# mythos-bio/mythos

Hardware: AMD Instinct MI355X
Metric: MD steps/sec (and ns/day) per GPU, oxDNA2 12 kbp duplex (higher is better)
Workload: dtype f32; 1 GPU; oxDNA2 12000 bp duplex (24000 nt), Debye-Hueckel salt 0.5, Langevin dt 0.005, free space, 1 replica/GPU; half_charged_ends=True, replicas=1, repeats=1, warmup_steps_done=10205, precision=headline f32 (north_star: fp32 at 1e-3); the other precision: --full, full=False

## Files before the change

include/mythos_hip.h:

```cpp
#ifndef MYTHOS_HIP_H
#define MYTHOS_HIP_H

#include <stdint.h>

#ifdef __cplusplus
extern "C" {
#endif

typedef struct mythos_system mythos_system_t;
typedef struct mythos_sim mythos_sim_t;
typedef struct mythos_martini mythos_martini_t;
typedef struct mythos_martini_sim mythos_martini_sim_t;
typedef struct mythos_obs mythos_obs_t;
typedef void* mythos_stream_t;

enum mythos_status {
  MYTHOS_OK = 0,
  MYTHOS_ERR_INVALID_ARGUMENT = -1,
  MYTHOS_ERR_HIP = -2,
  MYTHOS_ERR_NO_DEVICE = -3,
  MYTHOS_ERR_NOT_READY = -4,
  MYTHOS_ERR_OVERFLOW = -5,
  MYTHOS_ERR_NUMERIC = -6
};

enum mythos_dtype { MYTHOS_F32 = 0, MYTHOS_F64 = 1 };

#define MYTHOS_OXDNA_N_TERMS 8

const char* mythos_version(void);
const char* mythos_last_error(void);
int mythos_device_count(void);

int mythos_oxdna_param_count(void);
const char* mythos_oxdna_param_name(int index);

mythos_system_t* mythos_oxdna_create(int model, int n, const int32_t* seq, const uint8_t* is_end, int n_bonded,
                                     const int32_t* bonded, const double* box, int dtype, int device);
void mythos_oxdna_destroy(mythos_system_t* sys);

int mythos_oxdna_set_params(mythos_system_t* sys, const double* flat_params, int n_params);

int mythos_oxdna_set_nucleotide_types(mythos_system_t* sys, const uint8_t* is_rna);

int mythos_oxdna_set_pseq(mythos_system_t* sys, const double* marginals, const int32_t* unit, int n_bp,
                          const double* bp_probs, int terms);

int mythos_oxdna_energy_dpseq(mythos_system_t* sys, const void* center, const void* quat, int n_frames, double* e_terms,
                              void* dU_dcenter, void* dU_dquat, double* dU_dparams, double* dU_dmarginals, double* dU_dbp,
                              mythos_stream_t stream);

int mythos_oxdna_set_neighbors(mythos_system_t* sys, const int32_t* pairs, int n_pairs);

int mythos_oxdna_build_neighbors(mythos_system_t* sys, const void* center, double r_cut, double skin,
                                 mythos_stream_t stream);
int mythos_oxdna_neighbor_stats(mythos_system_t* sys, int* max_row, double* mean_row);

int mythos_oxdna_energy(mythos_system_t* sys, const void* center, const void* quat, int n_frames, double* e_terms,
                        void* dU_dcenter, void* dU_dquat, double* dU_dparams, mythos_stream_t stream);

#define MYTHOS_DEBYE_SWEEP_CONSTS 5
int mythos_oxdna_debye_sweep(mythos_system_t* sys, const void* center, const void* quat, int n_frames, int n_kt,
                             const double* dh_consts, double* e_dh, double* de_dconsts, mythos_stream_t stream);

#define MYTHOS_OP_BOND 0
#define MYTHOS_OP_MINDISTANCE 1
int mythos_oxdna_order_params(mythos_system_t* sys, const void* center, const void* quat, int n_frames, int n_ops,
                              const int32_t* op_kind, const int32_t* op_first, const int32_t* pairs, int n_pairs,
                              double hb_cutoff, double* op_out, double* hb_out, double* dist_out, mythos_stream_t stream);

mythos_obs_t* mythos_observables_create(int model, int n, const double* geometry, const double* box, int n_bp,
                                        const int32_t* base_pairs, int n_quartets, const int32_t* quartets, int skip_ends,
                                        int dtype, int device);
void mythos_observables_destroy(mythos_obs_t* obs);
int mythos_observables_width(const mythos_obs_t* obs);
int mythos_observables_eval(mythos_obs_t* obs, const void* center, const void* quat, int n_frames, double* out,
                            mythos_stream_t stream);
int mythos_oxdna_energy_obs(mythos_system_t* sys, const void* center, const void* quat, int n_frames, double* e_terms,
                            void* dU_dcenter, void* dU_dquat, double* dU_dparams, mythos_obs_t* obs, double* obs_out,
                            mythos_stream_t stream);

mythos_sim_t* mythos_langevin_create(mythos_system_t* sys, double dt, double kT, double gamma_t, double gamma_r,
                                     double mass, const double* inertia, uint64_t seed);
void mythos_langevin_destroy(mythos_sim_t* sim);

int mythos_langevin_set_neighbor_policy(mythos_sim_t* sim, double r_cut, double skin, int every);

int mythos_langevin_init_momenta(mythos_sim_t* sim, void* p_lin, void* p_ang, mythos_stream_t stream);

int mythos_langevin_run(mythos_sim_t* sim, void* center, void* quat, void* p_lin, void* p_ang, int n_steps,
                        int save_every, void* traj_center, void* traj_quat, double* e_trace,
                        mythos_stream_t stream);
int mythos_langevin_load(mythos_sim_t* sim, const void* center, const void* quat, const void* p_lin, const void* p_ang,
                         mythos_stream_t stream);
int mythos_langevin_advance(mythos_sim_t* sim, int n_steps, int save_every, void* traj_center, void* traj_quat,
                            double* e_trace, mythos_stream_t stream);
int mythos_langevin_store(mythos_sim_t* sim, void* center, void* quat, void* p_lin, void* p_ang, mythos_stream_t stream);

int64_t mythos_langevin_get_step(const mythos_sim_t* sim);
int mythos_langevin_set_step(mythos_sim_t* sim, int64_t step);
int mythos_langevin_set_seed(mythos_sim_t* sim, uint64_t seed);

int mythos_langevin_set_external_forces(mythos_sim_t* sim, int count, const int32_t* index, const double* force);

enum mythos_langevin_option { MYTHOS_LANGEVIN_UNFUSED = 0 };
int mythos_langevin_set_option(mythos_sim_t* sim, int option, int64_t value);

int mythos_langevin_set_timing(mythos_sim_t* sim, int samples);
int mythos_langevin_last_kernel_ms(const mythos_sim_t* sim, double* kernel_ms, double* loop_ms_per_launch,
                                   int* launches, int* samples);

int mythos_langevin_last_recoveries(const mythos_sim_t* sim, int* recoveries);
int mythos_langevin_last_rebuilds(const mythos_sim_t* sim, int* scheduled);

int mythos_oxdna_read_trajectory(const char* path, int n, int max_frames, double* times, double* box, double* energies,
                                 double* frames, int* n_frames);

int mythos_oxdna_write_trajectory(const char* path, int n, int n_frames, const double* times, const double* box,
                                  const double* energies, const double* frames, int append);

enum mythos_debug_key {
  MYTHOS_DEBUG_CELL_BUCKET_CAP = 0,
  MYTHOS_DEBUG_ENERGY_LIST_CAP = 1,
  MYTHOS_DEBUG_MD_SEGMENT = 2,
  MYTHOS_DEBUG_MD_OVERFLOW_AT = 3,
  MYTHOS_DEBUG_MD_DENSE = 4,
  MYTHOS_DEBUG_MD_ITEMS_BIG = 5,
  MYTHOS_DEBUG_MD_LANES = 6,
  MYTHOS_DEBUG_KEYS = 7
};
int mythos_debug_set(int key, int64_t value);
int64_t mythos_debug_get(int key);

#define MYTHOS_MARTINI_N_TERMS 3
mythos_martini_t* mythos_martini_create(int n, const int32_t* types, int n_types, const double* sigma,
                                        const double* eps, int n_bonds, const int32_t* bonds, const double* bond_k,
                                        const double* bond_r0, int n_angles, const int32_t* angles,
                                        const double* angle_k, const double* angle_t0, int angle_kind, double r_cut,
                                        int dtype, int device);
void mythos_martini_destroy(mythos_martini_t* m);
int mythos_martini_energy(mythos_martini_t* m, const void* pos, const void* box, int n_frames, double* e_terms,
                          void* dU_dpos, mythos_stream_t stream);

int mythos_martini_param_grads(mythos_martini_t* m, const void* pos, const void* box, int n_frames, double* d_sigma,
                               double* d_eps, double* d_bond_k, double* d_bond_r0, double* d_angle_k,
                               double* d_angle_t0, mythos_stream_t stream);

mythos_martini_sim_t* mythos_martini_langevin_create(mythos_martini_t* sys, double dt, double kT, double gamma,
                                                     const double* mass, uint64_t seed);
void mythos_martini_langevin_destroy(mythos_martini_sim_t* sim);
int mythos_martini_langevin_set_neighbor_policy(mythos_martini_sim_t* sim, double skin, int rebuild_every);
int mythos_martini_langevin_set_inner_list(mythos_martini_sim_t* sim, double margin, int every);
int mythos_martini_langevin_init_velocities(mythos_martini_sim_t* sim, void* vel, mythos_stream_t stream);
int mythos_martini_langevin_run(mythos_martini_sim_t* sim, void* pos, void* vel, const double* box, int n_steps,
                                int save_every, void* traj_pos, double* e_trace, mythos_stream_t stream);
int mythos_martini_langevin_load(mythos_martini_sim_t* sim, const void* pos, const void* vel, const double* box,
                                 mythos_stream_t stream);
int mythos_martini_langevin_advance(mythos_martini_sim_t* sim, int n_steps, int save_every, void* traj_pos, double* e_trace,
                                    mythos_stream_t stream);
int mythos_martini_langevin_store(mythos_martini_sim_t* sim, void* pos, void* vel, mythos_stream_t stream);
int64_t mythos_martini_langevin_get_step(const mythos_martini_sim_t* sim);
int mythos_martini_langevin_last_rebuilds(const mythos_martini_sim_t* sim, int* scheduled);
int mythos_martini_langevin_last_kernel_ms(const mythos_martini_sim_t* sim, double* kernel_ms,
                                           double* loop_ms_per_launch, int* launches, int* samples);
int mythos_martini_langevin_set_timing(mythos_martini_sim_t* sim, int samples);
int mythos_martini_langevin_last_recoveries(const mythos_martini_sim_t* sim, int* recoveries);
int mythos_martini_langevin_neighbor_stats(const mythos_martini_sim_t* sim, int* max_row, double* mean_row);
int mythos_martini_langevin_get_rows(const mythos_martini_sim_t* sim, int which, int32_t* rows, int32_t* row_len, int* stride);

int mythos_martini_langevin_set_barostat(mythos_martini_sim_t* sim, int kind, int coupling, const double ref_p[2],
                                         const double compressibility[2], double tau_p, int every);
int mythos_martini_langevin_pressure(mythos_martini_sim_t* sim, double out[10], mythos_stream_t stream);
int mythos_martini_langevin_get_box(const mythos_martini_sim_t* sim, double box[3]);
int mythos_martini_langevin_last_boxes(const mythos_martini_sim_t* sim, double* boxes, int* n_rows);

typedef struct mythos_martini_obs mythos_martini_obs_t;
mythos_martini_obs_t* mythos_martini_obs_create(int n, int n_groups, const int32_t* beads_per_item, const int32_t* members,
                                                const int32_t* index, int device);
void mythos_martini_obs_destroy(mythos_martini_obs_t* obs);
int64_t mythos_martini_obs_count(const mythos_martini_obs_t* obs);
int mythos_martini_obs_eval(mythos_martini_obs_t* obs, const void* pos, const void* box, int dtype, int n_frames, double* out,
                            mythos_stream_t stream);

typedef struct mythos_w1_plan mythos_w1_plan_t;
mythos_w1_plan_t* mythos_w1_plan_create(int n_groups, const int32_t* n_frames, const int32_t* members, const double* samples,
                                        const int64_t* n_ref, const double* ref, const double* ref_weights,
                                        const uint8_t* has_ref_weights, const int64_t* order, int device,
                                        mythos_stream_t stream);
void mythos_w1_plan_destroy(mythos_w1_plan_t* plan);
int mythos_w1_eval(mythos_w1_plan_t* plan, const double* weights, double* w1, double* dw1_dweights, mythos_stream_t stream);

#define MYTHOS_MEMBRANE_ROW 7
typedef struct mythos_membrane mythos_membrane_t;
mythos_membrane_t* mythos_membrane_create(int n, int n_lipids, const int32_t* lipid_start, const int32_t* lipid_beads, int n_thick,
                                          const int32_t* thick_beads, const int32_t* thick_lipid, int device);
void mythos_membrane_destroy(mythos_membrane_t* mem);
int mythos_membrane_n_lipids(const mythos_membrane_t* mem);
int mythos_membrane_eval(mythos_membrane_t* mem, const void* pos, const void* box, int dtype, int n_frames, double* out,
                         int8_t* leaflets, mythos_stream_t stream);

#define MYTHOS_DUPLEX_ROW 4
typedef struct mythos_duplex_obs mythos_duplex_obs_t;
mythos_duplex_obs_t* mythos_duplex_obs_create(int model, int n, const double* geometry, const double* box, int n_bp,
                                              const int32_t* base_pairs, int n_quartets, const int32_t* quartets,
                                              const int32_t* end_pairs, const double* target_center, int device);
void mythos_duplex_obs_destroy(mythos_duplex_obs_t* obs);
int mythos_duplex_obs_eval(mythos_duplex_obs_t* obs, const void* center, const void* quat, int dtype, int n_frames, double* out,
                           mythos_stream_t stream);

#ifdef __cplusplus
}
#endif
#endif
```

mythos_amd/_lib.py:

```python

from __future__ import annotations

import ctypes as C
import os
from pathlib import Path

import torch

_LIB_PATH = Path(__file__).resolve().parent / "lib" / "libmythos_hip.so"

c_int_p = C.POINTER(C.c_int32)
c_double_p = C.POINTER(C.c_double)
c_uint8_p = C.POINTER(C.c_uint8)


class MythosHipError(RuntimeError):
    """An error reported by libmythos_hip.so."""


_lib = None

V = C.c_void_p
_SIGS = {
    "mythos_version": (C.c_char_p, []),
    "mythos_last_error": (C.c_char_p, []),
    "mythos_device_count": (C.c_int, []),
    "mythos_debug_set": (C.c_int, [C.c_int, C.c_int64]),
    "mythos_debug_get": (C.c_int64, [C.c_int]),
    "mythos_oxdna_param_count": (C.c_int, []),
    "mythos_oxdna_param_name": (C.c_char_p, [C.c_int]),
    "mythos_oxdna_create": (V, [C.c_int, C.c_int, c_int_p, c_uint8_p, C.c_int, c_int_p, c_double_p, C.c_int, C.c_int]),
    "mythos_oxdna_destroy": (None, [V]),
    "mythos_oxdna_set_params": (C.c_int, [V, c_double_p, C.c_int]),
    "mythos_oxdna_set_pseq": (C.c_int, [V, c_double_p, c_int_p, C.c_int, c_double_p, C.c_int]),
    "mythos_oxdna_set_nucleotide_types": (C.c_int, [V, c_uint8_p]),
    "mythos_oxdna_set_neighbors": (C.c_int, [V, c_int_p, C.c_int]),
    "mythos_oxdna_build_neighbors": (C.c_int, [V, V, C.c_double, C.c_double, V]),
    "mythos_oxdna_neighbor_stats": (C.c_int, [V, C.POINTER(C.c_int), c_double_p]),
    "mythos_oxdna_energy": (C.c_int, [V, V, V, C.c_int, V, V, V, V, V]),
    "mythos_oxdna_energy_obs": (C.c_int, [V, V, V, C.c_int, V, V, V, V, V, V, V]),
    "mythos_oxdna_energy_dpseq": (C.c_int, [V, V, V, C.c_int, V, V, V, V, V, V, V]),
    "mythos_oxdna_debye_sweep": (C.c_int, [V, V, V, C.c_int, C.c_int, c_double_p, V, V, V]),
    "mythos_oxdna_order_params": (C.c_int, [V, V, V, C.c_int, C.c_int, c_int_p, c_int_p, c_int_p, C.c_int, C.c_double, V, V, V, V]),
    "mythos_observables_create": (V, [C.c_int, C.c_int, c_double_p, c_double_p, C.c_int, c_int_p, C.c_int, c_int_p, C.c_int, C.c_int, C.c_int]),
    "mythos_observables_destroy": (None, [V]),
    "mythos_observables_width": (C.c_int, [V]),
    "mythos_observables_eval": (C.c_int, [V, V, V, C.c_int, V, V]),
    "mythos_langevin_create": (V, [V, C.c_double, C.c_double, C.c_double, C.c_double, C.c_double, c_double_p, C.c_uint64]),
    "mythos_langevin_destroy": (None, [V]),
    "mythos_langevin_set_neighbor_policy": (C.c_int, [V, C.c_double, C.c_double, C.c_int]),
    "mythos_langevin_init_momenta": (C.c_int, [V, V, V, V]),
    "mythos_langevin_run": (C.c_int, [V, V, V, V, V, C.c_int, C.c_int, V, V, V, V]),
    "mythos_langevin_load": (C.c_int, [V, V, V, V, V, V]),
    "mythos_langevin_advance": (C.c_int, [V, C.c_int, C.c_int, V, V, V, V]),
    "mythos_langevin_store": (C.c_int, [V, V, V, V, V, V]),
    "mythos_langevin_get_step": (C.c_int64, [V]),
    "mythos_langevin_set_step": (C.c_int, [V, C.c_int64]),
    "mythos_langevin_set_seed": (C.c_int, [V, C.c_uint64]),
    "mythos_langevin_set_external_forces": (C.c_int, [V, C.c_int, c_int_p, c_double_p]),
    "mythos_langevin_last_kernel_ms": (C.c_int, [V, c_double_p, c_double_p, C.POINTER(C.c_int), C.POINTER(C.c_int)]),
    "mythos_langevin_set_option": (C.c_int, [V, C.c_int, C.c_int64]),
    "mythos_langevin_set_timing": (C.c_int, [V, C.c_int]),
    "mythos_martini_langevin_set_timing": (C.c_int, [V, C.c_int]),
    "mythos_langevin_last_recoveries": (C.c_int, [V, C.POINTER(C.c_int)]),
    "mythos_langevin_last_rebuilds": (C.c_int, [V, C.POINTER(C.c_int)]),
    "mythos_oxdna_read_trajectory": (C.c_int, [C.c_char_p, C.c_int, C.c_int, c_double_p, c_double_p, c_double_p, c_double_p, C.POINTER(C.c_int)]),
    "mythos_oxdna_write_trajectory": (C.c_int, [C.c_char_p, C.c_int, C.c_int, c_double_p, c_double_p, c_double_p, c_double_p, C.c_int]),
    "mythos_martini_create": (
        V,
        [C.c_int, c_int_p, C.c_int, c_double_p, c_double_p, C.c_int, c_int_p, c_double_p, c_double_p, C.c_int,
         c_int_p, c_double_p, c_double_p, C.c_int, C.c_double, C.c_int, C.c_int],
    ),
    "mythos_martini_destroy": (None, [V]),
    "mythos_martini_energy": (C.c_int, [V, V, V, C.c_int, V, V, V]),
    "mythos_martini_param_grads": (C.c_int, [V, V, V, C.c_int, V, V, V, V, V, V, V]),
    "mythos_martini_langevin_create": (V, [V, C.c_double, C.c_double, C.c_double, c_double_p, C.c_uint64]),
    "mythos_martini_langevin_destroy": (None, [V]),
    "mythos_martini_langevin_set_neighbor_policy": (C.c_int, [V, C.c_double, C.c_int]),
    "mythos_martini_langevin_set_inner_list": (C.c_int, [V, C.c_double, C.c_int]),
    "mythos_martini_langevin_init_velocities": (C.c_int, [V, V, V]),
    "mythos_martini_langevin_run": (C.c_int, [V, V, V, c_double_p, C.c_int, C.c_int, V, V, V]),
    "mythos_martini_langevin_load": (C.c_int, [V, V, V, c_double_p, V]),
    "mythos_martini_langevin_advance": (C.c_int, [V, C.c_int, C.c_int, V, V, V]),
    "mythos_martini_langevin_store": (C.c_int, [V, V, V, V]),
    "mythos_martini_langevin_get_step": (C.c_int64, [V]),
    "mythos_martini_langevin_last_rebuilds": (C.c_int, [V, C.POINTER(C.c_int)]),
    "mythos_martini_langevin_last_kernel_ms": (C.c_int, [V, c_double_p, c_double_p, C.POINTER(C.c_int), C.POINTER(C.c_int)]),
    "mythos_martini_langevin_last_recoveries": (C.c_int, [V, C.POINTER(C.c_int)]),
    "mythos_martini_langevin_neighbor_stats": (C.c_int, [V, C.POINTER(C.c_int), c_double_p]),
    "mythos_martini_langevin_get_rows": (C.c_int, [V, C.c_int, C.POINTER(C.c_int32), C.POINTER(C.c_int32), C.POINTER(C.c_int)]),
    "mythos_martini_langevin_set_barostat": (C.c_int, [V, C.c_int, C.c_int, c_double_p, c_double_p, C.c_double, C.c_int]),
    "mythos_martini_langevin_pressure": (C.c_int, [V, c_double_p, V]),
    "mythos_martini_langevin_get_box": (C.c_int, [V, c_double_p]),
    "mythos_martini_langevin_last_boxes": (C.c_int, [V, c_double_p, C.POINTER(C.c_int)]),
    "mythos_martini_obs_create": (V, [C.c_int, C.c_int, c_int_p, c_int_p, c_int_p, C.c_int]),
    "mythos_martini_obs_destroy": (None, [V]),
    "mythos_martini_obs_count": (C.c_int64, [V]),
    "mythos_martini_obs_eval": (C.c_int, [V, V, V, C.c_int, C.c_int, V, V]),
    "mythos_w1_plan_create": (V, [C.c_int, c_int_p, c_int_p, V, C.POINTER(C.c_int64), V, V, c_uint8_p, V, C.c_int, V]),
    "mythos_w1_plan_destroy": (None, [V]),
    "mythos_w1_eval": (C.c_int, [V, V, V, V, V]),
    "mythos_membrane_create": (V, [C.c_int, C.c_int, c_int_p, c_int_p, C.c_int, c_int_p, c_int_p, C.c_int]),
    "mythos_membrane_destroy": (None, [V]),
    "mythos_membrane_n_lipids": (C.c_int, [V]),
    "mythos_membrane_eval": (C.c_int, [V, V, V, C.c_int, C.c_int, V, V, V]),
    "mythos_duplex_obs_create": (V, [C.c_int, C.c_int, c_double_p, c_double_p, C.c_int, c_int_p, C.c_int, c_int_p, c_int_p, c_double_p, C.c_int]),
    "mythos_duplex_obs_destroy": (None, [V]),
    "mythos_duplex_obs_eval": (C.c_int, [V, V, V, C.c_int, C.c_int, V, V]),
}


def lib_path() -> Path:
    return Path(os.environ.get("MYTHOS_HIP_LIB", _LIB_PATH))


def load() -> C.CDLL:
    global _lib
    if _lib is not None:
        return _lib
    path = lib_path()
    if not path.exists():
        raise MythosHipError(
            f"{path} not found: the HIP extension is not built (run __graft_entry__.build()). "
            "mythos_amd has no CPU fallback."
        )
    lib = C.CDLL(str(path))
    for name, (res, args) in _SIGS.items():
        fn = getattr(lib, name)
        fn.restype = res
        fn.argtypes = args
    _lib = lib
    return lib


DECLARED_SYMBOLS = tuple(_SIGS)


MEMBRANE_ROW = 7


def last_error() -> str:
    return load().mythos_last_error().decode()


def check(rc: int, what: str = "") -> None:
    if rc == 0:
        return
    msg = f"{what}: {last_error()} (status {rc})"
    if rc == -1:
        raise ValueError(msg)
    if rc == -6:
        raise FloatingPointError(msg)
    raise MythosHipError(msg)


DEBUG_KEYS = {"cell_bucket_cap": 0, "energy_list_cap": 1, "md_segment": 2, "md_overflow_at": 3, "md_dense": 4, "md_items_big": 5, "md_lanes": 6}


def debug_set(key: str, value: int) -> None:
    check(load().mythos_debug_set(DEBUG_KEYS[key], int(value)), f"debug_set({key})")


def debug_get(key: str) -> int:
    return int(load().mythos_debug_get(DEBUG_KEYS[key]))


_PARAM_NAMES: list[str] = []


def param_names() -> list[str]:
    if not _PARAM_NAMES:
        lib = load()
        _PARAM_NAMES.extend(lib.mythos_oxdna_param_name(i).decode() for i in range(lib.mythos_oxdna_param_count()))
    return list(_PARAM_NAMES)


def device_count() -> int:
    return int(load().mythos_device_count())


def ptr(t):
    if t is None:
        return None
    if hasattr(t, "data_ptr"):
        return C.c_void_p(t.data_ptr())
    return C.c_void_p(t.ctypes.data)


def stream(device) -> C.c_void_p:
    return C.c_void_p(torch.cuda.current_stream(device).cuda_stream)


def dtype_code(dtype: torch.dtype) -> int:
    if dtype == torch.float32:
        return 0
    if dtype == torch.float64:
        return 1
    raise ValueError(f"unsupported dtype {dtype}: use torch.float32 or torch.float64")


class Handle:

    _destroy = ""
    _h = None

    def __init__(self, create: str, *args):
        self._lib = load()
        self._h = getattr(self._lib, create)(*args)
        if not self._h:
            raise MythosHipError(f"{create}: {last_error()}")

    def close(self) -> None:
        h, self._h = self._h, None
        if h:
            getattr(self._lib, self._destroy)(h)

    def __del__(self):
        try:
            self.close()
        except Exception:
            pass


def per_device(owner, key, make):
    sets = owner.__dict__.setdefault("_sets", {})
    key = str(key)
    if key not in sets:
        sets[key] = make()
    return sets[key]
```

mythos_amd/csrc/langevin.hip:

```cpp
#include <memory>
#include <vector>

#include "langevin_core.inc"

namespace {
MdEntries md_entries_of(const mythos_sim* s) { return s->sys->dtype == MYTHOS_F32 ? md_entries<float>() : md_entries_f64(); }
}

extern "C" {

mythos_sim_t* mythos_langevin_create(mythos_system_t* sys, double dt, double kT, double gamma_t, double gamma_r,
                                     double mass, const double* inertia, uint64_t seed) {
  if (!sys || !(dt > 0) || !(kT >= 0) || gamma_t < 0 || gamma_r < 0 || !(mass > 0)) {
    set_error("mythos_langevin_create: invalid argument");
    return nullptr;
  }
  if (select_device(sys->device, "mythos_langevin_create")) return nullptr;
  auto s = std::make_unique<mythos_sim>();
  s->sys = sys;
  s->device = sys->device;
  s->dt = dt;
  s->kT = kT;
  s->gamma_t = gamma_t;
  s->gamma_r = gamma_r;
  s->mass = mass;
  for (int k = 0; k < 3; ++k) s->inertia[k] = inertia ? inertia[k] : 1.0;
  s->seed = seed;
  const size_t v4 = (sys->dtype == MYTHOS_F32 ? sizeof(float4) : sizeof(double4)) * (size_t)sys->n;
  bool ok = md_run_create(*s);
  for (int k = 0; k < 2; ++k)
    for (int a = 0; a < mythos_sim::kFrameArrays; ++a) ok = ok && s->frame[k][a].alloc(v4) == 0;
  ok = ok && s->keep_hi.alloc(v4) == 0 && s->keep_lo.alloc(v4) == 0 &&
       s->d_epart.alloc((size_t)((sys->n + 15) / 16) * kTraceWidth) == 0 && sys->reserve_refs() == 0;
  if (!ok) {
    set_error("mythos_langevin_create: device allocation failed");
    return nullptr;
  }
  return s.release();
}

void mythos_langevin_destroy(mythos_sim_t* s) { delete s; }

int mythos_langevin_set_neighbor_policy(mythos_sim_t* s, double r_cut, double skin, int every) {
  if (!s || (every > 0 && (!(r_cut > 0) || !(skin > 0)))) {
    set_error("mythos_langevin_set_neighbor_policy: invalid argument");
    return MYTHOS_ERR_INVALID_ARGUMENT;
  }
  s->r_cut = r_cut;
  s->skin = skin;
  s->rebuild_every = every;
  s->list_fitted = false;
  s->list_valid = false;
  return MYTHOS_OK;
}

int mythos_langevin_init_momenta(mythos_sim_t* s, void* p_lin, void* p_ang, mythos_stream_t stream) {
  if (!s || !p_lin || !p_ang) {
    set_error("mythos_langevin_init_momenta: invalid argument");
    return MYTHOS_ERR_INVALID_ARGUMENT;
  }
  MYTHOS_HIP_TRY(hipSetDevice(s->device));
  return md_entries_of(s).init_momenta(s, p_lin, p_ang, (hipStream_t)stream);
}

namespace {

int md_ready_state(mythos_sim_t* s, const char* who) {
  mythos_system* sys = s->sys;
  if (!sys->params_set) {
    set_error(std::string(who) + ": parameters must be set first");
    return MYTHOS_ERR_NOT_READY;
  }
  if (sys->model == 4 && !sys->types_set) {
    set_error(std::string(who) + ": an oxNA system needs its nucleotide types (mythos_oxdna_set_nucleotide_types)");
    return MYTHOS_ERR_NOT_READY;
  }
  MYTHOS_HIP_TRY(hipSetDevice(sys->device));
  return MYTHOS_OK;
}

int md_ready(mythos_sim_t* s, const char* who) {
  mythos_system* sys = s->sys;
  if (int rc = md_ready_state(s, who)) return rc;
  if (!sys->nbrs_set && s->rebuild_every <= 0) {
    set_error(std::string(who) + ": parameters and neighbours (or a neighbour policy) must be set first");
    return MYTHOS_ERR_NOT_READY;
  }
  if (s->rebuild_every > 0 && sys->list.stride == 0)
    if (int rc = rows_reserve(sys->list, sys->n, 64)) return rc;
  if (s->list_epoch != sys->list_epoch) {
    s->list_valid = false;
    s->list_epoch = sys->list_epoch;
  }
  return MYTHOS_OK;
}


int md_load(mythos_sim_t* s, void* c, void* q, void* p, void* l, hipStream_t st) {
  s->unfused.active = s->unfused.want && s->sys->model == 4;
  return md_entries_of(s).load(s, c, q, p, l, st);
}

int md_advance(mythos_sim_t* s, int n_steps, int save_every, bool close, void* tc, void* tq, double* e_trace, hipStream_t st) {
  if (s->ext_count > 0 && s->unfused.active) {
    set_error("mythos_langevin_run / advance: external forces are not applied on the unfused oxNA path "
              "(MYTHOS_LANGEVIN_UNFUSED); clear them or step through the fused kernel");
    return MYTHOS_ERR_INVALID_ARGUMENT;
  }
  const size_t q_align = s->sys->dtype == MYTHOS_F32 ? sizeof(float4) : sizeof(double4);
  if (save_every > 0 && tq && (reinterpret_cast<uintptr_t>(tq) % q_align) != 0) {
    set_error("mythos_langevin_run / advance: traj_quat must be aligned to 4 elements (" + std::to_string(q_align) + " bytes)");
    return MYTHOS_ERR_INVALID_ARGUMENT;
  }
  return md_entries_of(s).advance(s, n_steps, save_every, close, tc, tq, e_trace, st);
}

int md_store(mythos_sim_t* s, void* c, void* q, void* p, void* l, hipStream_t st) {
  return md_entries_of(s).store(s, c, q, p, l, st);
}

}

int mythos_langevin_run(mythos_sim_t* s, void* center, void* quat, void* p_lin, void* p_ang, int n_steps,
                        int save_every, void* traj_center, void* traj_quat, double* e_trace,
                        mythos_stream_t stream) {
  if (!s || !center || !quat || !p_lin || !p_ang || n_steps < 0 || save_every < 0) {
    set_error("mythos_langevin_run: invalid argument");
    return MYTHOS_ERR_INVALID_ARGUMENT;
  }
  if (int rc = md_ready(s, "mythos_langevin_run")) return rc;
  hipStream_t st = (hipStream_t)stream;
  if (int rc = md_load(s, center, quat, p_lin, p_ang, st)) return rc;
  const int rc = md_advance(s, n_steps, save_every, true, traj_center, traj_quat, e_trace, st);
  if (int rs = md_store(s, center, quat, p_lin, p_ang, st)) return rc ? rc : rs;
  return rc;
}

int mythos_langevin_load(mythos_sim_t* s, const void* center, const void* quat, const void* p_lin, const void* p_ang,
                         mythos_stream_t stream) {
  if (!s || !center || !quat || !p_lin || !p_ang) {
    set_error("mythos_langevin_load: invalid argument");
    return MYTHOS_ERR_INVALID_ARGUMENT;
  }
  if (int rc = md_ready_state(s, "mythos_langevin_load")) return rc;
  return md_load(s, (void*)center, (void*)quat, (void*)p_lin, (void*)p_ang, (hipStream_t)stream);
}

int mythos_langevin_advance(mythos_sim_t* s, int n_steps, int save_every, void* traj_center, void* traj_quat,
                            double* e_trace, mythos_stream_t stream) {
  if (!s || n_steps < 0 || save_every < 0) {
    set_error("mythos_langevin_advance: invalid argument");
    return MYTHOS_ERR_INVALID_ARGUMENT;
  }
  if (!s->resident) {
    set_error("mythos_langevin_advance: no resident state (call mythos_langevin_load first; a run that ended in a numeric "
              "error drops its state)");
    return MYTHOS_ERR_NOT_READY;
  }
  if (int rc = md_ready(s, "mythos_langevin_advance")) return rc;
  return md_advance(s, n_steps, save_every, false, traj_center, traj_quat, e_trace, (hipStream_t)stream);
}

int mythos_langevin_store(mythos_sim_t* s, void* center, void* quat, void* p_lin, void* p_ang, mythos_stream_t stream) {
  if (!s || !center || !quat || !p_lin || !p_ang) {
    set_error("mythos_langevin_store: invalid argument");
    return MYTHOS_ERR_INVALID_ARGUMENT;
  }
  if (!s->resident) {
    set_error("mythos_langevin_store: no resident state");
    return MYTHOS_ERR_NOT_READY;
  }
  if (s->open) {
    if (int rc = md_ready(s, "mythos_langevin_store")) return rc;
  } else {
    MYTHOS_HIP_TRY(hipSetDevice(s->device));
  }
  return md_store(s, center, quat, p_lin, p_ang, (hipStream_t)stream);
}

int64_t mythos_langevin_get_step(const mythos_sim_t* s) { return md_get_step(s); }

int mythos_langevin_set_step(mythos_sim_t* s, int64_t step) {
  if (!s || step < 0) {
    set_error("mythos_langevin_set_step: invalid argument");
    return MYTHOS_ERR_INVALID_ARGUMENT;
  }
  s->step = step;
  s->ext_stamp_stale = true;
  return MYTHOS_OK;
}

int mythos_langevin_set_external_forces(mythos_sim_t* s, int count, const int32_t* index, const double* force) {
  const char* who = "mythos_langevin_set_external_forces";
  if (!s || count < 0 || (count > 0 && (!index || !force))) {
    set_error(std::string(who) + ": invalid argument");
    return MYTHOS_ERR_INVALID_ARGUMENT;
  }
  if (s->resident && s->open) {
    set_error(std::string(who) + ": the resident frame is open (its pending closing half kick would mix two forces); call "
              "mythos_langevin_store first");
    return MYTHOS_ERR_INVALID_ARGUMENT;
  }
  const int n = s->sys->n;
  std::vector<char> seen((size_t)n, 0);
  for (int e = 0; e < count; ++e) {
    if (index[e] < 0 || index[e] >= n) {
      set_error(std::string(who) + ": nucleotide index " + std::to_string(index[e]) + " out of range [0, " + std::to_string(n) + ")");
      return MYTHOS_ERR_INVALID_ARGUMENT;
    }
    if (seen[index[e]]) {
      set_error(std::string(who) + ": nucleotide " + std::to_string(index[e]) + " is listed twice (sum its forces first)");
      return MYTHOS_ERR_INVALID_ARGUMENT;
    }
    seen[index[e]] = 1;
    for (int k = 0; k < 3; ++k)
      if (!std::isfinite(force[3 * (size_t)e + k])) {
        set_error(std::string(who) + ": a force component is not finite");
        return MYTHOS_ERR_INVALID_ARGUMENT;
      }
  }
  MYTHOS_HIP_TRY(hipSetDevice(s->device));
  s->ext_stamp_stale = true;
  if (count == 0) {
    s->ext_count = 0;
    return MYTHOS_OK;
  }
  MYTHOS_HIP_TRY(hipDeviceSynchronize());
  std::vector<double> f4((size_t)count * 4, 0.0);
  for (int e = 0; e < count; ++e)
    for (int k = 0; k < 3; ++k) f4[4 * (size_t)e + k] = force[3 * (size_t)e + k];
  s->ext_count = 0;
  if (int rc = s->d_ext_index.upload(index, (size_t)count)) return rc;
  if (int rc = s->d_ext_force.upload_real(s->sys->dtype, f4.data(), f4.size())) return rc;
  if (!s->d_ext_stamp)
    if (int rc = s->d_ext_stamp.alloc(1)) return rc;
  s->ext_count = count;
  return MYTHOS_OK;
}

int mythos_langevin_set_seed(mythos_sim_t* s, uint64_t seed) {
  if (!s) {
    set_error("mythos_langevin_set_seed: invalid argument");
    return MYTHOS_ERR_INVALID_ARGUMENT;
  }
  s->seed = seed;
  return MYTHOS_OK;
}

int mythos_langevin_last_kernel_ms(const mythos_sim_t* s, double* kernel_ms, double* loop_ms_per_launch,
                                   int* launches, int* samples) {
  return md_last_kernel_ms(s, kernel_ms, loop_ms_per_launch, launches, samples, "mythos_langevin_last_kernel_ms");
}

int mythos_langevin_last_recoveries(const mythos_sim_t* s, int* recoveries) {
  return md_last_count(s, &MdRun::last_recoveries, recoveries, "mythos_langevin_last_recoveries");
}

int mythos_langevin_last_rebuilds(const mythos_sim_t* s, int* scheduled) {
  return md_last_count(s, &MdRun::last_rebuilds, scheduled, "mythos_langevin_last_rebuilds");
}

int mythos_langevin_set_option(mythos_sim_t* s, int option, int64_t value) {
  if (!s || option != MYTHOS_LANGEVIN_UNFUSED || (value != 0 && value != 1)) {
    set_error("mythos_langevin_set_option: invalid argument");
    return MYTHOS_ERR_INVALID_ARGUMENT;
  }
  if (value == 1 && s->sys->model != 4) {
    set_error("mythos_langevin_set_option: the unfused path exists for oxNA systems (model 4) only");
    return MYTHOS_ERR_INVALID_ARGUMENT;
  }
  s->unfused.want = value == 1;
  return MYTHOS_OK;
}

int mythos_langevin_set_timing(mythos_sim_t* s, int samples) { return md_set_timing(s, samples, "mythos_langevin_set_timing"); }

}
```

mythos_amd/csrc/langevin_core.inc:

```
#include <algorithm>
#include <cmath>
#include <type_traits>

#include <hip/hip_ext.h>

#ifndef MYTHOS_LEAN_MATH
#define MYTHOS_LEAN_MATH 1
#endif

#include "cell_list.h"
#include "chunk_order.h"
#include "md_driver.h"
#include "md_plan.h"
#include "oxdna_gather.h"
#include "philox.h"

#include "langevin_step.h"
#include "langevin_frame.h"
#include "langevin_unfused.inc"

using namespace mythos;

namespace mythos {

static_assert(kMdPlanBlock == kMdBlock, "md_plan.h plans for the step kernel's workgroup");

inline int device_cus(const mythos_system* sys) {
  int cus = 256;
  (void)hipDeviceGetAttribute(&cus, hipDeviceAttributeMultiprocessorCount, sys->device);
  return cus;
}

template <typename R>
static int update_chunk_order(mythos_sim* sim, const typename Vec4T<R>::type* p0, int blocks, hipStream_t st) {
  if (blocks < 64) {
    sim->d_chunk_order.reset(), sim->d_chunk_keys.reset();
    return 0;
  }
  if (int rc = sim->d_chunk_keys.grow((size_t)blocks)) return rc;
  if (int rc = sim->d_chunk_order.grow((size_t)blocks)) return rc;
  MYTHOS_HIP_TRY(chunk_order_device(p0, blocks, kMdBlock / sim->lanes, std::max(1.0, sim->r_cut > 0 ? sim->r_cut : 4.0), sim->d_chunk_keys.get(),
                                    sim->d_chunk_order.get(), st));
  return 0;
}

template <typename R, int MODEL>
static int load_typed(mythos_sim* sim, const R* center, const R* quat, const R* p_lin, const R* p_ang, hipStream_t st) {
  mythos_system* sys = sim->sys;
  const int n = sys->n;
  const int tb = (n + 255) / 256;
  const OxParams<R>& P = params_of<R>(sys);
  const R g_k1 = P[GEO_BACK_A1], g_k2 = (MODEL >= 2) ? P[GEO_BACK_A2] : R(0);
  sim->cur = 0;
  const Frame<R> f0 = frame_of<R>(sim, 0);
  const double* Prna = oxdna_param_set(sys, sys->param_sets() == 1 ? 0 : 1);
  hipLaunchKernelGGL((pack_state_kernel<R, (MODEL == 4 ? 0 : back_axis<MODEL>())>), dim3(tb), dim3(256), 0, st, n, g_k1, g_k2,
                     R(Prna[GEO_BACK_A1]), R(Prna[GEO_BACK_A2]), center, quat, p_lin, p_ang,
                     sys->d_meta.get(), f0, sim->keep_valid ? (const R*)sim->keep_hi.get() : nullptr,
                     (const R*)sim->keep_lo.get());
  MYTHOS_HIP_TRY(hipGetLastError());
  sim->resident = true;
  sim->list_valid = false;
  sim->since_build = 0;
  sim->items_big = false;
  sim->open = false;
  sim->ext_stamp_stale = true;
  sim->param_epoch = sys->param_epoch;
  const int cus = device_cus(sys);
  sim->lanes = md_lanes_for(n, cus, debug_value(MYTHOS_DEBUG_MD_LANES));
  return update_chunk_order<R>(sim, f0.p0, md_plan_for(n, sim->lanes, cus, sizeof(R), 0).blocks, st);
}

template <typename R>
static int unpack_typed(mythos_sim* sim, R* center, R* quat, R* p_lin, R* p_ang, hipStream_t st) {
  const int n = sim->sys->n;
  hipLaunchKernelGGL(unpack_state_kernel<R>, dim3((n + 255) / 256), dim3(256), 0, st, n, frame_of<R>(sim, sim->cur),
                     center, quat, p_lin, p_ang, (R*)sim->keep_hi.get(), (R*)sim->keep_lo.get());
  MYTHOS_HIP_TRY(hipGetLastError());
  sim->keep_valid = true;
  return 0;
}

template <typename R, int MODEL>
static int advance_typed(mythos_sim* sim, int n_steps, int save_every, bool close, R* traj_center, R* traj_quat, double* e_trace,
                         hipStream_t st) {
  using V4 = typename Vec4T<R>::type;
  mythos_system* sys = sim->sys;
  const int n = sys->n;
  const MdPlan plan = md_plan_for(n, sim->lanes, device_cus(sys), sizeof(R), debug_value(MYTHOS_DEBUG_MD_DENSE));
  const int blocks = plan.blocks;
  const R* Pdev = device_params_of<R>(sys);
  const BoxT<R> box = make_box<R>(sys);
  const LangevinConst<R> K = make_const<R>(sim);
  const MdCut<R> cut = make_cut<R>(sys);
  const Frame<R> fr[2] = {frame_of<R>(sim, 0), frame_of<R>(sim, 1)};
  if (sim->param_epoch != sys->param_epoch) {
    const OxParams<R>& Ph = params_of<R>(sys);
    const double* Prna = oxdna_param_set(sys, sys->param_sets() == 1 ? 0 : 1);
    hipLaunchKernelGGL((rederive_frame_kernel<R, (MODEL == 4 ? 0 : back_axis<MODEL>())>), dim3((n + 255) / 256), dim3(256), 0, st, n,
                       Ph[GEO_BACK_A1], (MODEL >= 2) ? Ph[GEO_BACK_A2] : R(0), R(Prna[GEO_BACK_A1]), R(Prna[GEO_BACK_A2]),
                       (const int*)sys->d_meta.get(), fr[sim->cur]);
    MYTHOS_HIP_TRY(hipGetLastError());
    sim->param_epoch = sys->param_epoch;
  }
  const bool dynamic_list = sim->rebuild_every > 0;
  PseqView<R> pseq;
  const bool use_pseq = sys->pseq_terms != 0;
  if (debug_value(MYTHOS_DEBUG_MD_ITEMS_BIG) == 1) sim->items_big = true;
  if (use_pseq) pseq.marg = (const R*)sys->d_ps_marg.get(), pseq.unit = sys->d_ps_unit.get(), pseq.bp = (const R*)sys->d_ps_bp.get(), pseq.terms = sys->pseq_terms;
  int* halt_words = dynamic_list ? sys->list.d_overflow.get() : nullptr;
  auto launch_step = [&](int k, const LaunchRow& row) {
    const int cur = row.cur;
    const bool save = row.save;
    const R kick_close = R(row.kick_close);
    R* tc = ((save || row.save_next) && traj_center) ? traj_center + (size_t)row.sidx * n * 3 : nullptr;
    R* tq = ((save || row.save_next) && traj_quat) ? traj_quat + (size_t)row.sidx * n * 4 : nullptr;
    const V4* ref = (const V4*)sys->d_ref_pos.get();
    const V4* ref_off = (const V4*)sys->d_ref_off.get();
    const V4* ref_a1 = (const V4*)sys->d_ref_a1.get();
    if (sim->ext_count > 0) {
      if (sim->ext_stamp_stale) {
        (void)hipMemsetAsync(sim->d_ext_stamp.get(), 0, sizeof(unsigned long long), st);
        sim->ext_stamp_stale = false;
      }
      const double c = double(row.kick_close) + 0.5 * row.do_step;
      const unsigned long long stamp = 2ull * (unsigned long long)(sim->step + k) + (row.kick_close != 0.0f ? 1ull : 0ull) + 1ull;
      hipLaunchKernelGGL(ext_kick_kernel<R>, dim3(1), dim3(256), 0, st, sim->ext_count, (const int*)sim->d_ext_index.get(),
                         (const V4*)sim->d_ext_force.get(), R(c * sim->dt), fr[cur].mom, (const int*)sim->d_flags.get(),
                         (const int*)halt_words, k, stamp, sim->d_ext_stamp.get());
    }
    auto launch = [&](auto save_tag, auto items_tag, auto pseq_tag, auto dense_tag, auto lanes_tag) {
      hipExtLaunchKernelGGL((md_step_kernel<R, MODEL, decltype(save_tag)::value, decltype(items_tag)::value, decltype(pseq_tag)::value,
                                            decltype(dense_tag)::value, decltype(lanes_tag)::value>),
                            dim3(plan.grid), dim3(kMdBlock), 0, st, row.ea, row.eb, 0,
                            Pdev, box, K, cut, n, fr[cur], fr[cur ^ 1], sys->list.d_rows.get(), sys->d_row_len.get(), row_close_of(sys),
                            sys->list.stride, sys->extra_bonds ? 1 : 0, kick_close, row.do_step, sim->seed, (uint64_t)(sim->step + k), ref,
                            ref_off, ref_a1, sim->d_flags.get(), tc, tq, sim->d_epart.get(), sim->d_chunk_order.get(), halt_words, k, 0,
                            plan.prio_on, pseq);
    };
    with_bool(save, [&](auto save_tag) {
      with_bool(sim->items_big, [&](auto big_tag) {
        constexpr bool SV = decltype(save_tag)::value;
        using Items = std::integral_constant<int, decltype(big_tag)::value ? md_items_big<R, SV>() : kMdItems>;
        with_bool(use_pseq, [&](auto pseq_tag) {
          using L8 = std::integral_constant<int, 8>;
          using L16 = std::integral_constant<int, 16>;
          constexpr bool dense_exists = sizeof(R) == 4 && !SV && !decltype(pseq_tag)::value && Items::value == kMdItems && MODEL <= 2;
          if (sim->lanes == 16) {
            launch(save_tag, Items{}, pseq_tag, std::false_type{}, L16{});
          } else if constexpr (dense_exists) {
            with_bool(plan.dense_grid, [&](auto dense_tag) { launch(save_tag, Items{}, pseq_tag, dense_tag, L8{}); });
          } else {
            launch(save_tag, Items{}, pseq_tag, std::false_type{}, L8{});
          }
        });
      });
    });
    if (save)
      hipLaunchKernelGGL(reduce_trace_kernel<kTraceWidth>, dim3(1), dim3(256), 0, st, sim->d_epart.get(), blocks,
                         e_trace + (size_t)row.sidx * kTraceWidth);
  };
  auto rebuild = [&](int buf) -> int {
    if ((++sim->builds & 63) == 0)
      if (int rc = update_chunk_order<R>(sim, fr[buf].p0, blocks, st)) return rc;
    return rows_build_device(sys, fr[buf].p0, true, sim->r_cut, sim->skin, fr[buf].p3, fr[buf].p1, true, st);
  };
  auto rebuild_until_fit = [&](int buf) -> int {
    return rows_build_until_fit(sys, fr[buf].p0, true, sim->r_cut, sim->skin, fr[buf].p3, fr[buf].p1, true, true, st);
  };
  auto on_abort = [&]() -> int {
    if (!sim->items_big) {
      sim->items_big = true;
      return 0;
    }
    set_error("mythos_langevin_run: more than " + std::to_string(md_items_big<R, false>()) + " (" + std::to_string(md_items_big<R, true>()) +
              " on steps that save energies)"
              " neighbours of one nucleotide are inside the range of an angular term (overlapping bases?)");
    return MYTHOS_ERR_OVERFLOW;
  };
  MdDrive d;
  d.who = "mythos_langevin_run";
  d.n_steps = n_steps, d.save_every = save_every, d.close = close;
  d.energy_rows = save_every > 0 && e_trace != nullptr;
  d.plain_rows = save_every > 0 && e_trace == nullptr && (traj_center != nullptr || traj_quat != nullptr);
  d.dynamic_list = dynamic_list;
  d.halt_words = halt_words;
  d.row_stride = &sys->list.stride;
  d.skin = sim->skin;
  d.st = st;
  return md_drive(*sim, d, launch_step, rebuild, rebuild_until_fit, on_abort);
}

template <typename R>
static int entry_load(mythos_sim* s, void* c, void* q, void* p, void* l, hipStream_t st) {
  if (s->unfused.active) return unfused_load<R>(s, (R*)c, (R*)q, (R*)p, (R*)l, st);
  return with_model(s->sys->model, [&](auto m) { return load_typed<R, decltype(m)::value>(s, (R*)c, (R*)q, (R*)p, (R*)l, st); });
}

template <typename R>
static int entry_advance(mythos_sim* s, int n_steps, int save_every, bool close, void* tc, void* tq, double* e_trace, hipStream_t st) {
  if (s->unfused.active) return unfused_advance<R>(s, n_steps, save_every, (R*)tc, (R*)tq, e_trace, st);
  return with_model(s->sys->model, [&](auto m) {
    return advance_typed<R, decltype(m)::value>(s, n_steps, save_every, close, (R*)tc, (R*)tq, e_trace, st);
  });
}

template <typename R>
static int entry_store(mythos_sim* s, void* c, void* q, void* p, void* l, hipStream_t st) {
  if (s->unfused.active) return unfused_store<R>(s, (R*)c, (R*)q, (R*)p, (R*)l, st);
  const int rc = s->open ? entry_advance<R>(s, 0, 0, true, nullptr, nullptr, nullptr, st) : MYTHOS_OK;
  const int ru = unpack_typed<R>(s, (R*)c, (R*)q, (R*)p, (R*)l, st);
  return rc ? rc : ru;
}

template <typename R>
static int entry_init_momenta(mythos_sim* s, void* p_lin, void* p_ang, hipStream_t st) {
  const double sd_t = std::sqrt(s->mass * s->kT);
  double sd_r[3];
  for (int k = 0; k < 3; ++k) sd_r[k] = std::sqrt(s->inertia[k] * s->kT);
  hipLaunchKernelGGL(init_momenta_kernel<R>, dim3(1), dim3(256), 0, st, s->sys->n, R(sd_t), R(sd_r[0]), R(sd_r[1]), R(sd_r[2]), s->seed,
                     (R*)p_lin, (R*)p_ang);
  MYTHOS_HIP_TRY(hipGetLastError());
  return MYTHOS_OK;
}

struct MdEntries {
  int (*load)(mythos_sim*, void*, void*, void*, void*, hipStream_t);
  int (*advance)(mythos_sim*, int, int, bool, void*, void*, double*, hipStream_t);
  int (*store)(mythos_sim*, void*, void*, void*, void*, hipStream_t);
  int (*init_momenta)(mythos_sim*, void*, void*, hipStream_t);
};
template <typename R>
constexpr MdEntries md_entries() {
  return {entry_load<R>, entry_advance<R>, entry_store<R>, entry_init_momenta<R>};
}
MdEntries md_entries_f64();

}
```

mythos_amd/csrc/langevin_sim.h:

```cpp
#pragma once
#ifndef MYTHOS_UNFUSED_STATE_DEFINED
#error "langevin_sim.h needs UnfusedState: include langevin_unfused.inc (or langevin_core.inc), which defines it and then includes this file"
#endif
#include <cmath>

#include "langevin_step.h"
#include "md_driver.h"

struct mythos_sim : mythos::MdRun {
  mythos_system* sys = nullptr;
  int device = 0;
  double dt = 0, kT = 0, gamma_t = 0, gamma_r = 0, mass = 1, inertia[3] = {1, 1, 1};
  double r_cut = 0, skin = 0;
  static constexpr int kFrameArrays = 8;
  mythos::DeviceBytes frame[2][kFrameArrays];
  int builds = 0;
  int list_epoch = 0;
  mythos::DeviceBytes keep_hi, keep_lo;
  bool keep_valid = false;
  bool items_big = false;
  int param_epoch = 0;
  int lanes = mythos::kMdG;
  mythos::DeviceBuf<int> d_chunk_order;
  mythos::DeviceBuf<unsigned long long> d_chunk_keys;
  mythos::DeviceBuf<double> d_epart;
  mythos::UnfusedState unfused;
  int ext_count = 0;
  mythos::DeviceBuf<int> d_ext_index;
  mythos::DeviceBytes d_ext_force;
  mythos::DeviceBuf<unsigned long long> d_ext_stamp;
  bool ext_stamp_stale = true;
  ~mythos_sim() { (void)hipSetDevice(device); }
};

namespace mythos {

template <typename R>
static LangevinConst<R> make_const(const mythos_sim* s) {
  LangevinConst<R> K;
  K.dt = R(s->dt);
  K.half_dt = R(0.5 * s->dt);
  K.inv_mass = R(1.0 / s->mass);
  const double c1t = std::exp(-s->gamma_t * s->dt), c1r = std::exp(-s->gamma_r * s->dt);
  K.c1_t = R(c1t);
  K.c2_t = R(std::sqrt(s->kT * (1.0 - c1t * c1t) * s->mass));
  K.c1_r = R(c1r);
  for (int k = 0; k < 3; ++k) {
    K.inv_inertia[k] = R(1.0 / s->inertia[k]);
    K.c2_r[k] = R(std::sqrt(s->kT * (1.0 - c1r * c1r) * s->inertia[k]));
  }
  K.skin_half_sq = R(s->rebuild_every > 0 ? 0.25 * s->skin * s->skin : -1.0);
  return K;
}

template <typename R>
static MdCut<R> make_cut(const mythos_system* sys) {
  const OxParams<double>& P = sys->pd;
  double rbb = oxdna_param_max(sys, NEXC_BACKBONE_RC);
  if (sys->model >= 2) rbb = std::max(rbb, oxdna_param_max(sys, DH_RCUT));
  const double rcom = oxdna_close_range(sys);
  MdCut<R> c;
  c.rbb2 = R(rbb * rbb);
  c.rcom2 = R(rcom * rcom);
  auto sq = [](double v) { return R(v * v); };
  c.hb_lo2 = sq(P[HYDR_RCLOW]), c.hb_hi2 = sq(P[HYDR_RCHIGH]);
  c.cr_lo2 = sq(P[CRST_RCLOW]), c.cr_hi2 = sq(P[CRST_RCHIGH]);
  c.cx_lo2 = sq(P[CXST_RCLOW]), c.cx_hi2 = sq(P[CXST_RCHIGH]);
  c.hb_mask = 0;
  for (int k = 0; k < 16; ++k)
    if (P[HYDR_EPS_00 + k] != 0.0) c.hb_mask |= 1u << k;
  return c;
}

template <typename R>
static Frame<R> frame_of(const mythos_sim* sim, int k) {
  using V4 = typename Vec4T<R>::type;
  auto a = [&](int i) { return (V4*)sim->frame[k][i].get(); };
  return Frame<R>{a(0), a(1), a(2), a(3), a(4), a(5), a(6), a(7)};
}

}
```

mythos_amd/csrc/langevin_step.h:

```cpp
#pragma once
#include <hip/hip_runtime.h>

#include <cstdint>

#include "oxdna_gather.h"
#include "philox.h"

namespace mythos {

template <typename R>
struct LangevinConst {
  R dt, half_dt;
  R inv_mass;
  R inv_inertia[3];
  R c1_t, c2_t;
  R c1_r, c2_r[3];
  R skin_half_sq;
};

template <int K, typename R>
__device__ __forceinline__ void free_rotor(R* q, R* L, R h, const R* inv_I) {
  const R phi = h * L[K] * inv_I[K];
  R s, c;
  if constexpr (sizeof(R) == 4) {
    s = __sinf(R(0.5) * phi);
    c = __cosf(R(0.5) * phi);
  } else {
    R x = R(0.5) * phi;
    int halvings = 0;
    const bool large = __ballot(fabs(x) >= R(0.03125)) != 0ull;
    if (large)
      while (fabs(x) >= R(0.03125) && halvings < 64) x *= R(0.5), ++halvings;
    const R x2 = x * x;
    s = x * (R(1) + x2 * (R(-1.0 / 6) + x2 * (R(1.0 / 120) + x2 * R(-1.0 / 5040))));
    c = R(1) + x2 * (R(-0.5) + x2 * (R(1.0 / 24) + x2 * R(-1.0 / 720)));
    if (large)
      for (; halvings > 0; --halvings) {
        const R s2 = R(2) * s * c;
        c = c * c - s * s;
        s = s2;
      }
  }
  const R q0 = q[0], q1 = q[1], q2 = q[2], q3 = q[3];
  if constexpr (K == 0) {
    q[0] = c * q0 - s * q1;
    q[1] = c * q1 + s * q0;
    q[2] = c * q2 + s * q3;
    q[3] = c * q3 - s * q2;
  } else if constexpr (K == 1) {
    q[0] = c * q0 - s * q2;
    q[1] = c * q1 - s * q3;
    q[2] = c * q2 + s * q0;
    q[3] = c * q3 + s * q1;
  } else {
    q[0] = c * q0 - s * q3;
    q[1] = c * q1 + s * q2;
    q[2] = c * q2 - s * q1;
    q[3] = c * q3 + s * q0;
  }
  const R cf = c * c - s * s, sf = R(2) * s * c;
  constexpr int A = (K + 1) % 3, B = (K + 2) % 3;
  const R la = L[A], lb = L[B];
  L[A] = cf * la + sf * lb;
  L[B] = -sf * la + cf * lb;
}

template <typename R>
__device__ __forceinline__ void drift(R* x, R* q, const R* p, R* L, R h, const LangevinConst<R>& K) {
  x[0] += h * p[0] * K.inv_mass;
  x[1] += h * p[1] * K.inv_mass;
  x[2] += h * p[2] * K.inv_mass;
  free_rotor<2>(q, L, R(0.5) * h, K.inv_inertia);
  free_rotor<1>(q, L, R(0.5) * h, K.inv_inertia);
  free_rotor<0>(q, L, h, K.inv_inertia);
  free_rotor<1>(q, L, R(0.5) * h, K.inv_inertia);
  free_rotor<2>(q, L, R(0.5) * h, K.inv_inertia);
}

constexpr int kMdBlock = 256;
constexpr int kMdG = 8;
constexpr int kMdPPB = kMdBlock / kMdG;
#ifndef MYTHOS_MD_ITEMS
#define MYTHOS_MD_ITEMS 16
#endif
#ifndef MYTHOS_MD_F64_BLOCKS
#define MYTHOS_MD_F64_BLOCKS 3
#endif
#ifndef MYTHOS_MD_F64S_BLOCKS
#define MYTHOS_MD_F64S_BLOCKS 2
#endif
#ifndef MYTHOS_MD_F32_BLOCKS
#define MYTHOS_MD_F32_BLOCKS 3
#endif
#ifndef MYTHOS_MD_F32S_BLOCKS
#define MYTHOS_MD_F32S_BLOCKS 2
#endif
constexpr int kMdItems = MYTHOS_MD_ITEMS;
template <typename R, bool SAVE>
constexpr int md_items_big() {
  return (sizeof(R) == 8 && SAVE) ? 22 : 32;
}
#ifndef MYTHOS_MD_POOL
#define MYTHOS_MD_POOL 320
#endif
constexpr int kMdPool = MYTHOS_MD_POOL;
constexpr int kTraceWidth = T_COUNT + 2;

template <typename R>
struct Frame {
  typename Vec4T<R>::type *p0, *p1, *p2, *p3, *q, *pl, *mom, *ang;
};

template <typename R>
constexpr bool kHiLo = sizeof(R) == 4;

template <typename R>
__device__ __forceinline__ V3<R> centre_diff(const typename Vec4T<R>::type& o_hi, const typename Vec4T<R>::type& o_lo,
                                             const V3<R>& s_hi, const V3<R>& s_lo) {
  V3<R> d{o_hi.x - s_hi.x, o_hi.y - s_hi.y, o_hi.z - s_hi.z};
  if constexpr (kHiLo<R>) {
    d.x += o_lo.x - s_lo.x;
    d.y += o_lo.y - s_lo.y;
    d.z += o_lo.z - s_lo.z;
  }
  return d;
}

template <typename R>
struct MdCut {
  R rbb2;
  R rcom2;
  R hb_lo2, hb_hi2, cr_lo2, cr_hi2, cx_lo2, cx_hi2;
  unsigned int hb_mask;
};

template <typename R>
__device__ __forceinline__ V3<R> xyz(const typename Vec4T<R>::type& v) {
  return V3<R>{v.x, v.y, v.z};
}

template <typename R>
__device__ __forceinline__ R f3_coef(R eps, R tw, const F3P<R>& fp, R r2, R& coef) {
  coef = R(0);
  if (r2 >= fp.rc * fp.rc) return R(0);
  const R r = m_sqrt(r2);
  const FD<R> v = f3_eval(r, eps, fp);
  coef = tw * v.d / r;
  return v.f;
}

template <typename R>
__device__ __forceinline__ R f3_radial(R eps, R tw, const F3P<R>& fp, V3<R> d, R r2, V3<R>& g) {
  if (r2 >= fp.rc * fp.rc) return R(0);
  const R r = m_sqrt(r2);
  const FD<R> v = f3_eval(r, eps, fp);
  axpy(g, tw * v.d / r, d);
  return v.f;
}

#ifndef MYTHOS_MD_PRIO_MAP
#define MYTHOS_MD_PRIO_MAP 33210
#endif
#if MYTHOS_MD_PRIO_MAP != 0
constexpr int md_prio_digit(int phase) {
  int v = MYTHOS_MD_PRIO_MAP;
  for (int k = 4; k > phase; --k) v /= 10;
  return v % 10;
}
#define MD_PRIO(phase)                                                     \
  do {                                                                     \
    if (prio_on) __builtin_amdgcn_s_setprio(md_prio_digit(phase));        \
  } while (0)
#else
#define MD_PRIO(phase) do { } while (0)
#endif

template <typename R, bool SAVE, int ITEMS, bool DENSE = false, int MODEL = 2, bool PSEQ = false>
constexpr int md_blocks_per_cu() {
  if (DENSE) return 5;
  if (ITEMS > kMdItems) return sizeof(R) == 4 ? (SAVE ? 1 : 2) : 1;
  return sizeof(R) == 4 ? (SAVE ? MYTHOS_MD_F32S_BLOCKS : MYTHOS_MD_F32_BLOCKS) : (SAVE ? MYTHOS_MD_F64S_BLOCKS : MYTHOS_MD_F64_BLOCKS);
}

template <typename R>
struct RadSet {
  F3P<R> f_bb, f_base, f_bkba, f_babk;
  R eps_n, tw_n, tw_dh;
  DebyeP<R> dhp;
  bool half_ends;
  R rbb2, hb_lo2, hb_hi2, cr_lo2, cr_hi2, cx_lo2, cx_hi2;
  unsigned int hb_mask;
};
template <typename R, int MODEL, class PT>
__device__ __forceinline__ RadSet<R> radset_from(const PT& P, const MdCut<R>& cut) {
  RadSet<R> s;
  s.f_bb = f3_params<R>(P, NEXC_BACKBONE_RSTAR), s.f_base = f3_params<R>(P, NEXC_BASE_RSTAR);
  s.f_bkba = f3_params<R>(P, NEXC_BACK_BASE_RSTAR), s.f_babk = f3_params<R>(P, NEXC_BASE_BACK_RSTAR);
  s.eps_n = P[NEXC_EPS];
  s.tw_n = P[TW_NEXC], s.tw_dh = (MODEL >= 2) ? P[TW_DH] : R(0);
  s.half_ends = (MODEL >= 2) && (P[DH_HALF_CHARGED_ENDS] != R(0));
  s.dhp = (MODEL >= 2) ? debye_params<R>(P) : DebyeP<R>{};
  s.rbb2 = cut.rbb2, s.hb_lo2 = cut.hb_lo2, s.hb_hi2 = cut.hb_hi2, s.cr_lo2 = cut.cr_lo2, s.cr_hi2 = cut.cr_hi2;
  s.cx_lo2 = cut.cx_lo2, s.cx_hi2 = cut.cx_hi2, s.hb_mask = cut.hb_mask;
  return s;
}
template <typename R, class PT>
__device__ __forceinline__ MdCut<R> cut_from(const PT& P, R rcom2) {
  MdCut<R> c;
  const R rbb = fmax(P[NEXC_BACKBONE_RC], P[DH_RCUT]);
  c.rbb2 = rbb * rbb, c.rcom2 = rcom2;
  c.hb_lo2 = P[HYDR_RCLOW] * P[HYDR_RCLOW], c.hb_hi2 = P[HYDR_RCHIGH] * P[HYDR_RCHIGH];
  c.cr_lo2 = P[CRST_RCLOW] * P[CRST_RCLOW], c.cr_hi2 = P[CRST_RCHIGH] * P[CRST_RCHIGH];
  c.cx_lo2 = P[CXST_RCLOW] * P[CXST_RCLOW], c.cx_hi2 = P[CXST_RCHIGH] * P[CXST_RCHIGH];
  c.hb_mask = 0u;
#pragma unroll
  for (int k = 0; k < 16; ++k) c.hb_mask |= (P[HYDR_EPS_00 + k] != R(0)) ? (1u << k) : 0u;
  return c;
}
template <typename R>
__device__ __forceinline__ F3P<R> pick3(const F3P<R>& a, const F3P<R>& b, const F3P<R>& c, int k) {
  return {k == 0 ? a.rstar : (k == 1 ? b.rstar : c.rstar), k == 0 ? a.sigma : (k == 1 ? b.sigma : c.sigma),
          k == 0 ? a.b : (k == 1 ? b.b : c.b), k == 0 ? a.rc : (k == 1 ? b.rc : c.rc), a.base};
}
#define MD_PICK3(f) (k == 0 ? a.f : (k == 1 ? b.f : c.f))
template <typename R>
__device__ __forceinline__ RadSet<R> pick3(const RadSet<R>& a, const RadSet<R>& b, const RadSet<R>& c, int k) {
  RadSet<R> s;
  s.f_bb = pick3(a.f_bb, b.f_bb, c.f_bb, k), s.f_base = pick3(a.f_base, b.f_base, c.f_base, k);
  s.f_bkba = pick3(a.f_bkba, b.f_bkba, c.f_bkba, k), s.f_babk = pick3(a.f_babk, b.f_babk, c.f_babk, k);
  s.eps_n = MD_PICK3(eps_n), s.tw_n = MD_PICK3(tw_n), s.tw_dh = MD_PICK3(tw_dh);
  s.dhp = {MD_PICK3(dhp.rcut), MD_PICK3(dhp.rhigh), MD_PICK3(dhp.kappa), MD_PICK3(dhp.prefactor), MD_PICK3(dhp.bsmooth)};
  s.half_ends = a.half_ends;
  s.rbb2 = MD_PICK3(rbb2), s.hb_lo2 = MD_PICK3(hb_lo2), s.hb_hi2 = MD_PICK3(hb_hi2), s.cr_lo2 = MD_PICK3(cr_lo2);
  s.cr_hi2 = MD_PICK3(cr_hi2), s.cx_lo2 = MD_PICK3(cx_lo2), s.cx_hi2 = MD_PICK3(cx_hi2), s.hb_mask = MD_PICK3(hb_mask);
  return s;
}
#undef MD_PICK3

#define MD_RADSET_OF_ENTRY                                                                                         \
  const int md_kind = (MODEL == 4) ? na1_kind(self.rna, ((int)o0.w >> 3) & 1) : 0;                                 \
  const RadSet<R> rs_picked = (MODEL == 4) ? pick3(rs0, rs1, rs2, md_kind) : rs0;                                  \
  const RadSet<R>& rs = (MODEL == 4) ? rs_picked : rs0;
__device__ __forceinline__ int na1_kind(int self_rna, int other_rna) { return (self_rna && other_rna) ? 1 : ((self_rna || other_rna) ? 2 : 0); }

template <typename R, int MODEL, bool SAVE, int ITEMS, bool PSEQ = false, bool DENSE = false, int GL = kMdG>
__global__ __launch_bounds__(kMdBlock, (md_blocks_per_cu<R, SAVE, ITEMS, DENSE, MODEL, PSEQ>())) void md_step_kernel(
    const R* __restrict__ Pg, const BoxT<R> box, const LangevinConst<R> K, const MdCut<R> cut, int n, const Frame<R> in,
    const Frame<R> out,
    const int* __restrict__ rows, const int* __restrict__ row_len, const int* __restrict__ row_close, int row_stride,
    int extra_bonds, R kick_close, int do_step, uint64_t seed, uint64_t step, const typename Vec4T<R>::type* __restrict__ ref_pos,
    const typename Vec4T<R>::type* __restrict__ ref_off, const typename Vec4T<R>::type* __restrict__ ref_a1,
    int* __restrict__ flags,
    R* __restrict__ traj_c, R* __restrict__ traj_q, double* __restrict__ e_part, const int* __restrict__ chunk_order,
    const int* __restrict__ list_overflow, int k_index, int , int prio_on, const PseqView<R> pseq) {
  using V4 = typename Vec4T<R>::type;
  constexpr int G = GL, PPB = kMdBlock / GL;
  static_assert(GL == 8 || GL == 16, "lanes per nucleotide");
  static_assert(!DENSE || GL == kMdG, "DENSE serves large grids");
  constexpr int RW = (SAVE ? 12 + T_COUNT : 12) + 1;
  constexpr int kSlots = 2 + ITEMS;
  __shared__ int items[2][PPB][ITEMS];
  __shared__ int item_cnt[2][PPB];
  __shared__ int item_pre[4][PPB + 1];
  __shared__ R self_lds[PPB][13];
  __shared__ R rad_lds[PPB][7];
  static_assert(!DENSE || (sizeof(R) == 4 && !SAVE && !PSEQ && ITEMS == kMdItems && MODEL <= 2), "DENSE: see md_blocks_per_cu");
  constexpr bool kPooled = sizeof(R) == 8 || DENSE;
  constexpr int kPool = (ITEMS > kMdItems || !kPooled) ? PPB * kSlots : kMdPool * PPB / kMdPPB;
  static_assert(kPool >= PPB * ROW_BONDED_SLOTS, "the pool holds at least the bonded rows");
  static_assert(ITEMS > ROW_BONDED_SLOTS, "room for the second-bond slots of circular strands");
  __shared__ R res_flat[kPool * RW + (kPooled ? 0 : PPB)];
  __shared__ int row_base[kPooled ? 4 : 1][PPB + 1];
  constexpr int kFixedStride = (kSlots * RW) | 1;
  auto pool_row = [&](int row) -> R* { return res_flat + row * RW; };
  auto fixed_row = [&](int pp, int slot) -> R* { return res_flat + pp * kFixedStride + slot * RW; };
  __shared__ double e_lds[SAVE ? PPB : 1][kTraceWidth];
  using CP = ConstParams<R, PSEQ>;
  const auto make_cp = [&](const R* g) {
    if constexpr (PSEQ) return CP(g, pseq); else return CP(g);
  };
  const CP P = make_cp(Pg);
  const int grp = threadIdx.x / G;
  const int lane = threadIdx.x % G;
  const int n_blocks = (n + PPB - 1) / PPB;
  const int vb = (int)(blockIdx.x & 7) * ((n_blocks + 7) >> 3) + (int)(blockIdx.x >> 3);
  if (vb >= n_blocks) return;
  __shared__ int s_halt;
  int halt_word = 0;
  if (threadIdx.x == 0) {
    const int hw = flags[1], aw = flags[3];
    halt_word = ((hw != 0 && hw <= k_index) ? 1 : 0) | ((aw != 0 && aw <= k_index) ? 1 : 0) |
                (list_overflow ? (list_overflow[0] | list_overflow[1]) : 0);
  }
  const int bid = chunk_order ? chunk_order[vb] : vb;
  const int i = bid * PPB + grp;
  const bool valid = i < n;
  const int ii = valid ? i : n - 1;

  const R g_ba = P[GEO_BASE], g_st = P[GEO_STACK];
  const CP Prna = make_cp(Pg + ((MODEL == 4) ? OXP_COUNT : 0)), Pdrh = make_cp(Pg + ((MODEL == 4) ? 2 * OXP_COUNT : 0));
  const Na1Params<CP> P4{P, Prna, Pdrh};

  Nuc<R> self;
  V3<R> offb_s, self_lo{R(0), R(0), R(0)};
  {
    const V4 s0 = in.p0[ii], s1 = in.p1[ii], s2 = in.p2[ii], s3 = in.p3[ii];
    if constexpr (kHiLo<R>) self_lo = xyz<R>(in.pl[ii]);
    self.c = xyz<R>(s0);
    self.a1 = xyz<R>(s1);
    self.a3 = xyz<R>(s2);
    self.a2 = cross(self.a3, self.a1);
    offb_s = xyz<R>(s3);
    const int m = (int)s0.w;
    self.seq = m & 3;
    self.is_end = (m >> 2) & 1;
    self.rna = (m >> 3) & 1;
    if (lane == 0) {
      R* sl = self_lds[grp];
      sl[0] = s0.x, sl[1] = s0.y, sl[2] = s0.z, sl[3] = s1.x, sl[4] = s1.y, sl[5] = s1.z;
      sl[6] = s2.x, sl[7] = s2.y, sl[8] = s2.z, sl[9] = s0.w;
      sl[10] = self_lo.x, sl[11] = self_lo.y, sl[12] = self_lo.z;
    }
  }
  const int* __restrict__ row = rows + (size_t)ii * row_stride;
  const int len = valid ? row_len[ii] : 0;
  const int close_end = min(len, row_close[ii]);

  R e[T_COUNT];
#pragma unroll
  for (int k = 0; k < T_COUNT; ++k) e[k] = R(0);
  V3<R> gbk{R(0), R(0), R(0)}, gba{R(0), R(0), R(0)};

  MD_PRIO(0);
  const RadSet<R> rs0 = (MODEL == 4) ? radset_from<R, 2>(P, cut_from<R>(P, cut.rcom2)) : radset_from<R, MODEL>(P, cut);
  const RadSet<R> rs1 = (MODEL == 4) ? radset_from<R, 2>(Prna, cut_from<R>(Prna, cut.rcom2)) : rs0;
  const RadSet<R> rs2 = (MODEL == 4) ? radset_from<R, 2>(Pdrh, cut_from<R>(Pdrh, cut.rcom2)) : rs0;
  int n_items[2] = {0, 0};
  const int row_room = ITEMS - (extra_bonds ? ROW_BONDED_SLOTS - 2 : 0);
  const int lane64 = threadIdx.x & 63;
  const int gshift = lane64 & ~(G - 1);
  auto row_at = [&](int s, int end) -> int {
    const int v = row[max(min(s, end - 1), 0)];
    return s < end ? v : -1;
  };
  auto slot_of_entry = [&](int e) -> int { return e >= 0 ? (e & ROW_INDEX_MASK) : ii; };
  {
    int e_cur = -1, e_nxt = -1;
    V4 n0{}, n3{}, n1{}, nl{};
    {
      const int s = ROW_BONDED_SLOTS + lane;
      e_cur = row_at(s, close_end);
      e_nxt = row_at(s + G, close_end);
      const int j = slot_of_entry(e_cur);
      n0 = in.p0[j];
      n3 = in.p3[j];
      n1 = in.p1[j];
      if constexpr (kHiLo<R>) nl = in.pl[j];
    }
#pragma unroll 1
    for (int s0 = ROW_BONDED_SLOTS; s0 < close_end; s0 += G) {
      const int s = s0 + lane;
      const int entry = e_cur;
      const V4 o0 = n0, o3 = n3, o1 = n1, ol = nl;
      e_cur = e_nxt;
      e_nxt = row_at(s + 2 * G, close_end);
      {
        const int jn = slot_of_entry(e_cur);
        n0 = in.p0[jn];
        n3 = in.p3[jn];
        n1 = in.p1[jn];
        if constexpr (kHiLo<R>) nl = in.pl[jn];
      }
      bool flag[2] = {false, false};
      if (entry >= 0) {
        const bool role_p = (entry & ROW_ROLE_Q) == 0;
        MD_RADSET_OF_ENTRY
        const bool o_rna = (MODEL == 4) && ((((int)o0.w) >> 3) & 1);
        const R gba_s = (MODEL == 4 && self.rna) ? Prna[GEO_BASE] : g_ba, gba_o = o_rna ? Prna[GEO_BASE] : g_ba;
        const R gst_s = (MODEL == 4 && self.rna) ? Prna[GEO_STACK] : g_st, gst_o = o_rna ? Prna[GEO_STACK] : g_st;
        (void)gst_s, (void)gst_o;
        const V3<R> dco = min_image(centre_diff<R>(o0, ol, self.c, self_lo), box);
        const V3<R> offb_o = xyz<R>(o3);
        const bool close = dot(dco, dco) < cut.rcom2;
        {
          const V3<R> d = dco + offb_o - offb_s;
          const R r2 = dot(d, d);
          if (r2 < rs.rbb2) {
            const R r = m_sqrt(r2);
            const FD<R> v = f3_eval(r, rs.eps_n, rs.f_bb);
            R dVdr = rs.tw_n * v.d;
            R en = v.f;
            if constexpr (MODEL >= 2) {
              const FD<R> dh = debye_eval(r, rs.dhp);
              R mult = R(1);
              if (rs.half_ends) {
                const int mo = (int)o0.w;
                mult = (self.is_end ? R(0.5) : R(1)) * (((mo >> 2) & 1) ? R(0.5) : R(1));
              }
              dVdr += rs.tw_dh * mult * dh.d;
              if constexpr (SAVE) e[T_DH] += R(0.5) * mult * dh.f;
            }
            if constexpr (SAVE) e[T_NEXC] += R(0.5) * en;
            axpy(gbk, dVdr / r, d);
          }
        }
        if (close) {
          const V3<R> a1o = xyz<R>(o1);
          R en = R(0);
          {
            V3<R> dA = dco - offb_s;
            axpy(dA, gba_o, a1o);
            V3<R> dB = dco + offb_o;
            axpy(dB, -gba_s, self.a1);
            const R ra2 = dot(dA, dA), rb2 = dot(dB, dB);
            R c1, c2;
            en += f3_coef(rs.eps_n, rs.tw_n, rs.f_bkba, role_p ? ra2 : rb2, c1);
            en += f3_coef(rs.eps_n, rs.tw_n, rs.f_babk, role_p ? rb2 : ra2, c2);
            axpy(gbk, role_p ? c1 : c2, dA);
            axpy(gba, role_p ? c2 : c1, dB);
          }
          const V3<R> da = a1o - self.a1;
          {
            V3<R> d = dco;
            if constexpr (MODEL == 4) {
              axpy(d, gba_o, a1o);
              axpy(d, -gba_s, self.a1);
            } else {
              axpy(d, g_ba, da);
            }
            const R r2 = dot(d, d);
            en += f3_radial(rs.eps_n, rs.tw_n, rs.f_base, d, r2, gba);
            flag[0] = rs.cr_lo2 < r2 && r2 < rs.cr_hi2;
            if (!flag[0] && rs.hb_lo2 < r2 && r2 < rs.hb_hi2) {
              const int so = (int)o0.w & 3;
              if (PSEQ && (pseq.terms & 2) != 0)
                flag[0] = rs.hb_mask != 0u;
              else
                flag[0] = (rs.hb_mask >> (role_p ? (self.seq * 4 + so) : (so * 4 + self.seq))) & 1u;
            }
          }
          {
            V3<R> d = dco;
            if constexpr (MODEL == 4) {
              axpy(d, gst_o, a1o);
              axpy(d, -gst_s, self.a1);
            } else {
              axpy(d, g_st, da);
            }
            const R r2 = dot(d, d);
            flag[1] = rs.cx_lo2 < r2 && r2 < rs.cx_hi2;
          }
          if constexpr (SAVE) e[T_NEXC] += R(0.5) * en;
        }
      }
#pragma unroll
      for (int t = 0; t < 2; ++t) {
        const unsigned long long bal = __ballot(flag[t]);
        const unsigned int gm = (unsigned int)(bal >> gshift) & ((1u << G) - 1u);
        if (flag[t]) {
          const int pos = n_items[t] + __popc(gm & ((1u << lane) - 1u));
          if (pos < ITEMS) items[t][grp][pos] = entry;
        }
        n_items[t] += __popc(gm);
      }
    }
  }
  MD_PRIO(1);
  {
    int e_cur = -1, e_nxt = -1;
    V4 n0{}, n3{}, nl{};
    {
      const int s = close_end + lane;
      e_cur = row_at(s, len);
      e_nxt = row_at(s + G, len);
      const int j = slot_of_entry(e_cur);
      n0 = in.p0[j];
      n3 = in.p3[j];
      if constexpr (kHiLo<R>) nl = in.pl[j];
    }
#pragma unroll 1
    for (int s0 = close_end; s0 < len; s0 += G) {
      const int s = s0 + lane;
      const int entry = e_cur;
      const V4 o0 = n0, o3 = n3, ol = nl;
      e_cur = e_nxt;
      e_nxt = row_at(s + 2 * G, len);
      {
        const int jn = slot_of_entry(e_cur);
        n0 = in.p0[jn];
        n3 = in.p3[jn];
        if constexpr (kHiLo<R>) nl = in.pl[jn];
      }
      if (entry >= 0) {
        MD_RADSET_OF_ENTRY
        const V3<R> dco = min_image(centre_diff<R>(o0, ol, self.c, self_lo), box);
        const V3<R> d = dco + xyz<R>(o3) - offb_s;
        const R r2 = dot(d, d);
        if (r2 < rs.rbb2) {
          const R r = m_sqrt(r2);
          const FD<R> v = f3_eval(r, rs.eps_n, rs.f_bb);
          R dVdr = rs.tw_n * v.d;
          if constexpr (MODEL >= 2) {
            const FD<R> dh = debye_eval(r, rs.dhp);
            R mult = R(1);
            if (rs.half_ends) {
              const int mo = (int)o0.w;
              mult = (self.is_end ? R(0.5) : R(1)) * (((mo >> 2) & 1) ? R(0.5) : R(1));
            }
            dVdr += rs.tw_dh * mult * dh.d;
            if constexpr (SAVE) e[T_DH] += R(0.5) * mult * dh.f;
          }
          if constexpr (SAVE) e[T_NEXC] += R(0.5) * v.f;
          axpy(gbk, dVdr / r, d);
        }
      }
    }
  }
  if (n_items[0] + n_items[1] > row_room) {
    if (lane == 0) atomicMax(flags + 3, k_index + 1);
    n_items[0] = n_items[1] = 0;
  }
  group_reduce_v3<G>(gbk);
  group_reduce_v3<G>(gba);
  if (lane == 0) {
    R* rl = rad_lds[grp];
    rl[0] = gbk.x, rl[1] = gbk.y, rl[2] = gbk.z, rl[3] = gba.x, rl[4] = gba.y, rl[5] = gba.z;
#pragma unroll
    for (int t = 0; t < 2; ++t) item_cnt[t][grp] = valid ? n_items[t] : 0;
  }
  if (threadIdx.x == 0) s_halt = halt_word;
  __syncthreads();
  MD_PRIO(2);
  if (s_halt != 0) return;
  if (vb == 0 && threadIdx.x == 0) flags[2] = k_index + 1;

  {
    NoPG pg;
    const int wave = ((threadIdx.x >> 6) + bid) & 3;
    const bool bonded_wave = wave == 0;
    const int lst = wave == 3 ? 1 : 0;
    const int pw = threadIdx.x >> 6;
    const int n_bonded_rows = extra_bonds ? ROW_BONDED_SLOTS : 2;
    {
      const int l = threadIdx.x & 63;
      int inc = (l < PPB) ? item_cnt[lst][l] : 0;
      int rows_inc = (kPooled && l < PPB) ? n_bonded_rows + item_cnt[0][l] + item_cnt[1][l] : 0;
#pragma unroll
      for (int o = 1; o < PPB; o <<= 1) {
        const int u = __shfl_up(inc, o, 64);
        if (l >= o) inc += u;
        if constexpr (kPooled) {
          const int v = __shfl_up(rows_inc, o, 64);
          if (l >= o) rows_inc += v;
        }
      }
      if (l < PPB) item_pre[pw][l + 1] = inc;
      if (l == 0) item_pre[pw][0] = 0;
      if constexpr (kPooled) {
        if (l < PPB) row_base[pw][l + 1] = rows_inc;
        if (l == 0) row_base[pw][0] = 0;
      }
      __builtin_amdgcn_wave_barrier();
      __builtin_amdgcn_fence(__ATOMIC_ACQ_REL, "wavefront");
    }
    const bool pool_over = kPooled && row_base[kPooled ? pw : 0][PPB] > kPool;
    if (pool_over && threadIdx.x == 0) atomicMax(flags + 3, k_index + 1);
    const int n_list = pool_over ? 0 : item_pre[pw][PPB];
    const int half = (n_list + 1) >> 1;
    const int q_lo = wave == 2 ? half : 0;
    const int q_hi = wave == 1 ? half : n_list;
    const int n_total = q_hi - q_lo;
    const int n_sweeps = (n_total + 63) / 64;
    const int my_sweeps = bonded_wave ? (pool_over ? 0 : (extra_bonds ? 2 : 1)) : n_sweeps;
    for (int sweep = 0; sweep < my_sweeps; ++sweep) {
      int p, idx, sl;
      bool active;
      if (bonded_wave) {
        p = (threadIdx.x & 63) >> 1;
        idx = (threadIdx.x & 1) + 2 * sweep;
        sl = idx;
        active = p < PPB;
      } else {
        const int q = q_lo + sweep * 64 + (threadIdx.x & 63);
        active = q < q_hi;
        int lo = 0, hi = PPB;
        while (hi - lo > 1) {
          const int mid = (lo + hi) >> 1;
          if (item_pre[pw][mid] <= q) lo = mid; else hi = mid;
        }
        p = lo;
        const int k = q - item_pre[pw][lo];
        sl = active ? items[lst][p][k] : -1;
        idx = n_bonded_rows + k + (lst >= 1 ? item_cnt[0][p] : 0);
      }
      const int ip = bid * PPB + p;
      if (!active || ip >= n) continue;
      const int entry = bonded_wave ? rows[(size_t)ip * row_stride + sl] : sl;
      R* out_r = kPooled ? pool_row(row_base[kPooled ? pw : 0][p] + idx) : fixed_row(p, idx);
      SelfGrad<R> g;
      g.dc = g.g1 = g.g2 = g.g3 = V3<R>{R(0), R(0), R(0)};
      R ee[T_COUNT];
#pragma unroll
      for (int k = 0; k < T_COUNT; ++k) ee[k] = R(0);
      if (entry >= 0) {
        const int j = entry & ROW_INDEX_MASK;
        const bool role_p = bonded_wave ? ((sl & 1) == 1) : ((entry & ROW_ROLE_Q) == 0);
        Nuc<R> me, o;
        const R* ms = self_lds[p];
        me.c = V3<R>{ms[0], ms[1], ms[2]};
        me.a1 = V3<R>{ms[3], ms[4], ms[5]};
        me.a3 = V3<R>{ms[6], ms[7], ms[8]};
        me.a2 = cross(me.a3, me.a1);
        const int mm = (int)ms[9];
        me.seq = mm & 3;
        me.is_end = (mm >> 2) & 1;
        me.rna = (mm >> 3) & 1;
        me.idx = ip, o.idx = j;
        const V4 o0 = in.p0[j], o1 = in.p1[j], o2 = in.p2[j];
        V4 ol{};
        if constexpr (kHiLo<R>) ol = in.pl[j];
        o.c = xyz<R>(o0);
        o.a1 = xyz<R>(o1);
        o.a3 = xyz<R>(o2);
        o.a2 = cross(o.a3, o.a1);
        const int mo = (int)o0.w;
        o.seq = mo & 3;
        o.is_end = (mo >> 2) & 1;
        o.rna = (mo >> 3) & 1;
        const V3<R> dco = min_image(centre_diff<R>(o0, ol, me.c, V3<R>{ms[10], ms[11], ms[12]}), box);
        const auto& PP = [&]() -> const auto& {
          if constexpr (MODEL == 4) return P4; else return P;
        }();
        if (wave == 0) {
          bonded_pair<R, MODEL, true, NoPG>(PP, me, o, dco, role_p, R(0.5), ee, g, pg);
        } else if (wave != 3) {
          unbonded_angular<R, MODEL, true, NoPG, 3>(PP, me, o, dco, role_p, R(0.5), ee, g, pg);
        } else {
          unbonded_angular<R, MODEL, true, NoPG, 4>(PP, me, o, dco, role_p, R(0.5), ee, g, pg);
        }
      }
      out_r[0] = g.dc.x, out_r[1] = g.dc.y, out_r[2] = g.dc.z;
      out_r[3] = g.g1.x, out_r[4] = g.g1.y, out_r[5] = g.g1.z;
      out_r[6] = g.g2.x, out_r[7] = g.g2.y, out_r[8] = g.g2.z;
      out_r[9] = g.g3.x, out_r[10] = g.g3.y, out_r[11] = g.g3.z;
      if constexpr (SAVE) {
#pragma unroll
        for (int k = 0; k < T_COUNT; ++k) out_r[12 + k] = ee[k];
      }
    }
  }
  const int int_wave = (3 - bid) & 3;
  const int il = threadIdx.x & 63;
  const int i_int = bid * PPB + il;
  const bool integrates = (int)(threadIdx.x >> 6) == int_wave && il < PPB && i_int < n;
  R z[6] = {R(0), R(0), R(0), R(0), R(0), R(0)};
  V4 pm{}, lm{}, qv{}, r0{}, f0{}, a0{};
  if (integrates) {
    pm = in.mom[i_int], lm = in.ang[i_int], qv = in.q[i_int];
    if (do_step && K.skin_half_sq > R(0)) r0 = ref_pos[i_int], f0 = ref_off[i_int], a0 = ref_a1[i_int];
    if (do_step) normals6(seed, (uint32_t)i_int, step, 0u, z);
#pragma unroll
    for (int k = 0; k < 6; ++k) pin_vgpr(z[k]);
    pin_vgpr(pm.x), pin_vgpr(pm.y), pin_vgpr(pm.z);
    pin_vgpr(lm.x), pin_vgpr(lm.y), pin_vgpr(lm.z);
    pin_vgpr(qv.x), pin_vgpr(qv.y), pin_vgpr(qv.z), pin_vgpr(qv.w);
  }
  __syncthreads();
  MD_PRIO(3);

  SelfGrad<R> sg;
  sg.dc = sg.g1 = sg.g2 = sg.g3 = V3<R>{R(0), R(0), R(0)};
  const int fw = kPooled ? (int)(threadIdx.x >> 6) : 0;
  const int rb = kPooled ? row_base[fw][grp] : 0;
  const bool pool_ok = !kPooled || row_base[fw][PPB] <= kPool;
  const int n_bonded_fold = extra_bonds ? ROW_BONDED_SLOTS : 2;
  if (valid && pool_ok) {
    const int total = kPooled ? row_base[fw][grp + 1] - rb : n_bonded_fold + item_cnt[0][grp] + item_cnt[1][grp];
    for (int u = lane; u < total; u += G) {
      const R* rr = kPooled ? pool_row(rb + u) : fixed_row(grp, u);
      sg.dc = sg.dc + V3<R>{rr[0], rr[1], rr[2]};
      sg.g1 = sg.g1 + V3<R>{rr[3], rr[4], rr[5]};
      sg.g2 = sg.g2 + V3<R>{rr[6], rr[7], rr[8]};
      sg.g3 = sg.g3 + V3<R>{rr[9], rr[10], rr[11]};
      if constexpr (SAVE) {
#pragma unroll
        for (int k = 0; k < T_COUNT; ++k) e[k] += rr[12 + k];
      }
    }
  }
  if (lane == 0) {
    const R* rl = rad_lds[grp];
    const V3<R> rbk{rl[0], rl[1], rl[2]}, rba{rl[3], rl[4], rl[5]};
    sg.dc = sg.dc - (rbk + rba);
    if constexpr (MODEL == 4) {
      const bool r = self.rna != 0;
      axpy(sg.g1, -(r ? Prna[GEO_BACK_A1] : P[GEO_BACK_A1]), rbk);
      axpy(sg.g1, -(r ? Prna[GEO_BASE] : P[GEO_BASE]), rba);
      axpy(sg.g2, r ? R(0) : -P[GEO_BACK_A2], rbk);
      axpy(sg.g3, r ? -Prna[GEO_BACK_A2] : R(0), rbk);
    } else {
    axpy(sg.g1, -P[GEO_BACK_A1], rbk);
    axpy(sg.g1, -P[GEO_BASE], rba);
    if constexpr (MODEL == 2) axpy(sg.g2, -P[GEO_BACK_A2], rbk);
    if constexpr (MODEL == 3) axpy(sg.g3, -P[GEO_BACK_A2], rbk);
    }
  }
  if constexpr (SAVE) {
    group_reduce<G, R, true>(e, sg);
  } else {
    group_reduce_v3<G>(sg.dc);
    group_reduce_v3<G>(sg.g1);
    group_reduce_v3<G>(sg.g2);
    group_reduce_v3<G>(sg.g3);
  }

  if (lane == 0) {
    Nuc<R> own;
    const R* ms = self_lds[grp];
    own.a1 = V3<R>{ms[3], ms[4], ms[5]};
    own.a3 = V3<R>{ms[6], ms[7], ms[8]};
    own.a2 = cross(own.a3, own.a1);
    const V3<R> tl = axes_grad_to_torque(own, sg);
    R* fr = kPooled ? pool_row(pool_ok ? rb : grp * 2) : fixed_row(grp, 0);
    fr[0] = -sg.dc.x, fr[1] = -sg.dc.y, fr[2] = -sg.dc.z;
    fr[3] = dot(own.a1, tl), fr[4] = dot(own.a2, tl), fr[5] = dot(own.a3, tl);
  }
  __syncthreads();
  MD_PRIO(4);
  double ke_t = 0.0, ke_r = 0.0;
  if (integrates) {
    const int i = i_int;
    Nuc<R> self;
    {
      const R* ms = self_lds[il];
      self.c = V3<R>{ms[0], ms[1], ms[2]};
      self.a1 = V3<R>{ms[3], ms[4], ms[5]};
      self.a3 = V3<R>{ms[6], ms[7], ms[8]};
      self.a2 = cross(self.a3, self.a1);
    }
    const R* fr = kPooled ? pool_row(row_base[fw][PPB] <= kPool ? row_base[fw][il] : il * 2) : fixed_row(il, 0);
    const V3<R> F{fr[0], fr[1], fr[2]};
    const R tb[3] = {fr[3], fr[4], fr[5]};
    const bool int_rna = (MODEL == 4) && ((((int)self_lds[il][9]) >> 3) & 1);
    const R g_k1 = int_rna ? Prna[GEO_BACK_A1] : P[GEO_BACK_A1];
    const R g_k2 = (MODEL >= 2) ? (int_rna ? Prna[GEO_BACK_A2] : P[GEO_BACK_A2]) : R(0);
    R p[3] = {pm.x, pm.y, pm.z}, L[3] = {lm.x, lm.y, lm.z};
    R qs[4] = {qv.x, qv.y, qv.z, qv.w};
    const R kc = kick_close * K.dt;
    p[0] += kc * F.x;
    p[1] += kc * F.y;
    p[2] += kc * F.z;
    L[0] += kc * tb[0];
    L[1] += kc * tb[1];
    L[2] += kc * tb[2];
    if constexpr (SAVE) {
      ke_t = 0.5 * double(K.inv_mass) * (double(p[0]) * p[0] + double(p[1]) * p[1] + double(p[2]) * p[2]);
      ke_r = 0.5 * (double(K.inv_inertia[0]) * L[0] * L[0] + double(K.inv_inertia[1]) * L[1] * L[1] +
                    double(K.inv_inertia[2]) * L[2] * L[2]);
      if (traj_c) {
        traj_c[3 * i + 0] = self.c.x;
        traj_c[3 * i + 1] = self.c.y;
        traj_c[3 * i + 2] = self.c.z;
      }
      if (traj_q) {
        traj_q[4 * i + 0] = qs[0];
        traj_q[4 * i + 1] = qs[1];
        traj_q[4 * i + 2] = qs[2];
        traj_q[4 * i + 3] = qs[3];
      }
    }
    R x[3] = {self.c.x, self.c.y, self.c.z};
    R xl[3] = {self_lds[il][10], self_lds[il][11], self_lds[il][12]};
    R dxa[3] = {R(0), R(0), R(0)};
    R* const xd = kHiLo<R> ? dxa : x;
    V3<R> n1 = self.a1, n2 = self.a2, n3 = self.a3;
    const bool bk3 = MODEL == 3 || int_rna;
    V3<R> nbk{bk3 ? n3.x : n2.x, bk3 ? n3.y : n2.y, bk3 ? n3.z : n2.z};
    if (do_step) {
      p[0] += K.half_dt * F.x;
      p[1] += K.half_dt * F.y;
      p[2] += K.half_dt * F.z;
      L[0] += K.half_dt * tb[0];
      L[1] += K.half_dt * tb[1];
      L[2] += K.half_dt * tb[2];
      drift(xd, qs, p, L, K.half_dt, K);
      p[0] = K.c1_t * p[0] + K.c2_t * z[0];
      p[1] = K.c1_t * p[1] + K.c2_t * z[1];
      p[2] = K.c1_t * p[2] + K.c2_t * z[2];
      L[0] = K.c1_r * L[0] + K.c2_r[0] * z[3];
      L[1] = K.c1_r * L[1] + K.c2_r[1] * z[4];
      L[2] = K.c1_r * L[2] + K.c2_r[2] * z[5];
      drift(xd, qs, p, L, K.half_dt, K);
      if constexpr (kHiLo<R>) {
#pragma unroll
        for (int k = 0; k < 3; ++k) {
          const R sdl = xl[k] + dxa[k];
          const R t = x[k] + sdl;
          xl[k] = sdl - (t - x[k]);
          x[k] = t;
        }
      }
      const R inv = m_rsqrt(qs[0] * qs[0] + qs[1] * qs[1] + qs[2] * qs[2] + qs[3] * qs[3]);
      qs[0] *= inv;
      qs[1] *= inv;
      qs[2] *= inv;
      qs[3] *= inv;
      if (!(x[0] == x[0]) || !(qs[0] == qs[0])) atomicOr(flags, 2);
      quat_axes(qs[0], qs[1], qs[2], qs[3], n1, n2, n3);
      nbk = V3<R>{bk3 ? n3.x : n2.x, bk3 ? n3.y : n2.y, bk3 ? n3.z : n2.z};
      if (K.skin_half_sq > R(0)) {
        const R dx = x[0] - r0.x, dy = x[1] - r0.y, dz = x[2] - r0.z;
        const R bx = dx + (g_k1 * n1.x + g_k2 * nbk.x - f0.x), by = dy + (g_k1 * n1.y + g_k2 * nbk.y - f0.y),
                bz = dz + (g_k1 * n1.z + g_k2 * nbk.z - f0.z);
        const R gb = int_rna ? Prna[GEO_BASE] : P[GEO_BASE];
        const R sx = dx + gb * (n1.x - a0.x), sy = dy + gb * (n1.y - a0.y), sz = dz + gb * (n1.z - a0.z);
        if (dx * dx + dy * dy + dz * dz > K.skin_half_sq || bx * bx + by * by + bz * bz > K.skin_half_sq ||
            sx * sx + sy * sy + sz * sz > K.skin_half_sq)
          atomicMax(flags + 1, k_index + 1);
      }
    }
    if constexpr (!SAVE) {
      if (traj_c) {
        traj_c[3 * i + 0] = x[0];
        traj_c[3 * i + 1] = x[1];
        traj_c[3 * i + 2] = x[2];
      }
      if (traj_q) reinterpret_cast<V4*>(traj_q)[i] = V4{qs[0], qs[1], qs[2], qs[3]};
    }
    out.p0[i] = V4{x[0], x[1], x[2], self_lds[il][9]};
    if constexpr (kHiLo<R>) out.pl[i] = V4{xl[0], xl[1], xl[2], R(0)};
    out.p1[i] = V4{n1.x, n1.y, n1.z, R(0)};
    out.p2[i] = V4{n3.x, n3.y, n3.z, R(0)};
    out.p3[i] = do_step ? V4{g_k1 * n1.x + g_k2 * nbk.x, g_k1 * n1.y + g_k2 * nbk.y, g_k1 * n1.z + g_k2 * nbk.z, R(0)} : in.p3[i];
    out.q[i] = V4{qs[0], qs[1], qs[2], qs[3]};
    out.mom[i] = V4{p[0], p[1], p[2], R(0)};
    out.ang[i] = V4{L[0], L[1], L[2], R(0)};
  }
  if constexpr (SAVE) {
    if (lane == 0) {
#pragma unroll
      for (int k = 0; k < T_COUNT; ++k) e_lds[grp][k] = valid ? double(e[k]) : 0.0;
    }
    if ((int)(threadIdx.x >> 6) == int_wave && il < PPB) {
      e_lds[il][T_COUNT] = ke_t;
      e_lds[il][T_COUNT + 1] = ke_r;
    }
    __syncthreads();
    if (threadIdx.x < kTraceWidth) {
      double s = 0.0;
      for (int g = 0; g < PPB; ++g) s += e_lds[g][threadIdx.x];
      e_part[(size_t)bid * kTraceWidth + threadIdx.x] = s;
    }
  }
}

}
```

mythos_amd/csrc/md_driver.h:

```cpp
#ifndef MYTHOS_MD_DRIVER_H
#define MYTHOS_MD_DRIVER_H

#include <algorithm>
#include <string>

#include "mythos_internal.h"

namespace mythos {

struct MdRun {
  static constexpr int kCtlWords = 4;
  static constexpr int kMaxSamples = 16;
  uint64_t seed = 0;
  int64_t step = 0;
  int cur = 0;
  bool open = false;
  bool resident = false;
  bool list_valid = false;
  bool list_fitted = false;
  int since_build = 0;
  int rebuild_every = 0;
  int timing_samples = 0;
  hipEvent_t ev0 = nullptr, ev1 = nullptr;
  hipEvent_t sa[kMaxSamples] = {}, sb[kMaxSamples] = {};
  DeviceBuf<int> d_flags;
  int* h_ctl = nullptr;
  int* d_ctl = nullptr;
  double last_avg_ms = 0;
  double last_kernel_ms = 0;
  int last_launches = 0, last_samples = 0;
  int last_recoveries = 0;
  int last_rebuilds = 0;

  MdRun() = default;
  MdRun(const MdRun&) = delete;
  MdRun& operator=(const MdRun&) = delete;
  ~MdRun() {
    if (h_ctl) (void)hipHostFree(h_ctl);
    for (hipEvent_t e : {ev0, ev1})
      if (e) (void)hipEventDestroy(e);
    for (int k = 0; k < kMaxSamples; ++k) {
      if (sa[k]) (void)hipEventDestroy(sa[k]);
      if (sb[k]) (void)hipEventDestroy(sb[k]);
    }
  }
};

inline bool md_run_create(MdRun& r) {
  bool ok = r.d_flags.alloc(MdRun::kCtlWords) == 0 && hipMemset(r.d_flags.get(), 0, MdRun::kCtlWords * sizeof(int)) == hipSuccess &&
            hipHostMalloc((void**)&r.h_ctl, 8 * sizeof(int), hipHostMallocDefault) == hipSuccess &&
            hipHostGetDevicePointer((void**)&r.d_ctl, r.h_ctl, 0) == hipSuccess &&
            hipEventCreate(&r.ev0) == hipSuccess && hipEventCreate(&r.ev1) == hipSuccess;
  if (ok) std::fill(r.h_ctl, r.h_ctl + 8, 0);
  for (int k = 0; ok && k < MdRun::kMaxSamples; ++k)
    ok = hipEventCreate(&r.sa[k]) == hipSuccess && hipEventCreate(&r.sb[k]) == hipSuccess;
  return ok;
}

static __global__ void publish_ctl_kernel(int* __restrict__ flags, const int* __restrict__ overflow, int* __restrict__ out) {
  if (threadIdx.x != 0 || blockIdx.x != 0) return;
  out[0] = flags[0], out[1] = flags[1], out[2] = flags[2], out[3] = flags[3];
  out[4] = overflow ? overflow[0] : 0, out[5] = overflow ? overflow[1] : 0, out[6] = overflow ? overflow[2] : 0;
  flags[0] = 0, flags[2] = 0;
}

template <int WIDTH>
static __global__ __launch_bounds__(256) void reduce_trace_kernel(const double* __restrict__ part, int n_blocks, double* __restrict__ out) {
  static_assert(WIDTH <= 16, "one column per trace entry");
  __shared__ double acc[16][17];
  const int k = threadIdx.x & 15, g = threadIdx.x >> 4;
  double s = 0.0;
  if (k < WIDTH)
    for (int b = g; b < n_blocks; b += 16) s += part[(size_t)b * WIDTH + k];
  acc[g][k] = s;
  __syncthreads();
  if (g == 0 && k < WIDTH && out) {
    double t = 0.0;
#pragma unroll
    for (int j = 0; j < 16; ++j) t += acc[j][k];
    out[k] = t;
  }
}

struct MdDrive {
  const char* who;
  int n_steps, save_every;
  bool close;
  bool energy_rows;
  bool plain_rows;
  bool dynamic_list;
  int* halt_words;
  const int* row_stride;
  double skin;
  std::string give_up_hint;
  hipStream_t st;
};

struct LaunchRow {
  int cur;
  bool save;
  bool save_next;
  int sidx;
  float kick_close;
  int do_step;
  int built_at;
  hipEvent_t ea, eb;
};

template <class Launch, class Rebuild, class RebuildUntilFit, class OnAbort>
static int md_drive(MdRun& run, const MdDrive& d, Launch&& launch, Rebuild&& rebuild, RebuildUntilFit&& rebuild_until_fit,
                    OnAbort&& on_abort) {
  const bool closes = d.close || (d.energy_rows && d.n_steps > 0 && d.n_steps % d.save_every == 0);
  const int n_launch = closes ? d.n_steps + 1 : d.n_steps;
  if (n_launch == 0) return MYTHOS_OK;
  const hipStream_t st = d.st;
  const bool was_open = run.open;
  const int cur0 = run.cur;
  int built_at = 0;
  if (d.dynamic_list) {
    if (!run.list_fitted) {
      if (int rc = rebuild_until_fit(cur0)) return rc;
      run.list_fitted = true;
    } else if (!run.list_valid) {
      if (int rc = rebuild(cur0)) return rc;
    } else {
      built_at = -run.since_build;
    }
    run.list_valid = true;
  }
  const bool timing = run.timing_samples > 0;
  if (timing) MYTHOS_HIP_TRY(hipEventRecord(run.ev0, st));
  int launches = 0, samples = 0, recoveries = 0, scheduled = 0;
  const int max_samples = std::min(run.timing_samples, MdRun::kMaxSamples);
  const int sample_stride = std::max(1, n_launch / std::max(1, max_samples));
  auto drop_list = [&]() {
    run.list_valid = false;
    run.since_build = 0;
    run.last_recoveries = recoveries;
    run.last_rebuilds = scheduled;
    (void)hipMemsetAsync(run.d_flags.get() + 1, 0, 3 * sizeof(int), st);
    if (d.halt_words) (void)hipMemsetAsync(d.halt_words, 0, kOverflowWords * sizeof(int), st);
  };
  auto fail = [&](int ran, int rc) -> int {
    run.cur = cur0 ^ (ran & 1);
    run.step += ran;
    run.open = was_open || ran > 0;
    drop_list();
    return rc;
  };
  constexpr int kMaxRecoveries = 64;
  const long long dbg_seg = debug_value(MYTHOS_DEBUG_MD_SEGMENT);
  const int kSegment = dbg_seg > 0 ? (int)std::min<long long>(dbg_seg, 1 << 20) : 8192;
  int k = 0, seg_len = kSegment;
  int cur = cur0;
  while (k < n_launch) {
    const int seg_start = k, seg_end = std::min(n_launch - 1, k + seg_len - 1);
    for (; k <= seg_end; ++k) {
      const bool last = (k == d.n_steps);
      LaunchRow row;
      row.cur = cur;
      row.save = d.energy_rows && k > 0 && (k % d.save_every == 0);
      row.save_next = d.plain_rows && !last && ((k + 1) % d.save_every == 0);
      row.sidx = row.save ? (k / d.save_every - 1) : (row.save_next ? ((k + 1) / d.save_every - 1) : 0);
      if (d.dynamic_list && k - built_at >= run.rebuild_every) {
        if (int rc = rebuild(cur)) return fail(k, rc);
        built_at = k;
        ++scheduled;
        if (debug_value(MYTHOS_DEBUG_MD_OVERFLOW_AT) == k + 1) {
          debug_clear(MYTHOS_DEBUG_MD_OVERFLOW_AT);
          MYTHOS_HIP_TRY(hipMemsetD32Async((hipDeviceptr_t)d.halt_words, *d.row_stride + 1, 1, st));
        }
      }
      row.kick_close = (k == 0 && !was_open) ? 0.0f : 0.5f;
      row.do_step = last ? 0 : 1;
      row.built_at = built_at;
      row.ea = row.eb = nullptr;
      if (!row.save && (k % sample_stride == sample_stride / 2) && samples < max_samples)
        row.ea = run.sa[samples], row.eb = run.sb[samples], ++samples;
      launch(k, row);
      ++launches;
      cur ^= 1;
    }
    if (timing && k >= n_launch) MYTHOS_HIP_TRY(hipEventRecord(run.ev1, st));
    hipLaunchKernelGGL(publish_ctl_kernel, dim3(1), dim3(1), 0, st, run.d_flags.get(), (const int*)d.halt_words, run.d_ctl);
    MYTHOS_HIP_TRY(hipGetLastError());
    MYTHOS_HIP_TRY(hipStreamSynchronize(st));
    const int* ctl = run.h_ctl;
    if (ctl[0] & 2) {
      drop_list();
      run.resident = false;
      run.step += d.n_steps;
      run.last_avg_ms = run.last_kernel_ms = 0.0;
      run.last_launches = launches;
      run.last_samples = samples;
      set_error(std::string(d.who) + ": NaN in the state (time step too large or overlapping start configuration)");
      return MYTHOS_ERR_NUMERIC;
    }
    const int aborted = ctl[3];
    if (ctl[1] == 0 && ctl[4] == 0 && ctl[5] == 0 && aborted == 0) continue;
    if (aborted != 0) {
      if (int rc = on_abort()) return fail(aborted - 1, rc);
    } else if (!d.dynamic_list) {
      break;
    }
    const int progressed = std::max(ctl[2], seg_start);
    const int ran = aborted != 0 ? std::min(progressed, aborted - 1) : progressed;
    if (++recoveries > kMaxRecoveries) {
      set_error(std::string(d.who) + ": the neighbour list had to be rebuilt out of turn more than " + std::to_string(kMaxRecoveries) +
                " times in one run: the skin (" + std::to_string(d.skin) + ") is too small for a rebuild every " +
                std::to_string(run.rebuild_every) + " steps" + d.give_up_hint);
      return fail(ran, MYTHOS_ERR_OVERFLOW);
    }
    cur = cur0 ^ (ran & 1);
    k = ran;
    seg_len = std::max(std::min(256, kSegment), seg_len / 4);
    MYTHOS_HIP_TRY(hipMemsetAsync(run.d_flags.get() + 1, 0, 3 * sizeof(int), st));
    if (d.dynamic_list) {
      if (int rc = rebuild_until_fit(cur)) return fail(ran, rc);
      built_at = k;
    }
  }
  run.last_recoveries = recoveries;
  run.last_rebuilds = scheduled;
  run.cur = cur;
  run.open = !closes;
  run.since_build = d.n_steps - built_at;
  if (timing) {
    float ms = 0;
    MYTHOS_HIP_TRY(hipEventElapsedTime(&ms, run.ev0, run.ev1));
    run.last_avg_ms = launches ? double(ms) / launches : 0.0;
    double acc = 0;
    for (int s = 0; s < samples; ++s) {
      float t = 0;
      MYTHOS_HIP_TRY(hipEventElapsedTime(&t, run.sa[s], run.sb[s]));
      acc += t;
    }
    run.last_kernel_ms = samples ? acc / samples : 0.0;
  } else {
    run.last_avg_ms = run.last_kernel_ms = 0.0;
  }
  run.last_launches = launches;
  run.last_samples = samples;
  run.step += d.n_steps;
  return MYTHOS_OK;
}

inline int md_set_timing(MdRun* r, int samples, const char* who) {
  if (!r || samples < 0) {
    set_error(std::string(who) + ": invalid argument");
    return MYTHOS_ERR_INVALID_ARGUMENT;
  }
  r->timing_samples = std::min(samples, MdRun::kMaxSamples);
  return MYTHOS_OK;
}

inline int md_last_kernel_ms(const MdRun* r, double* kernel_ms, double* loop_ms_per_launch, int* launches, int* samples,
                             const char* who) {
  if (!r) {
    set_error(std::string(who) + ": invalid argument");
    return MYTHOS_ERR_INVALID_ARGUMENT;
  }
  if (kernel_ms) *kernel_ms = r->last_kernel_ms;
  if (loop_ms_per_launch) *loop_ms_per_launch = r->last_avg_ms;
  if (launches) *launches = r->last_launches;
  if (samples) *samples = r->last_samples;
  return MYTHOS_OK;
}

inline int md_last_count(const MdRun* r, int MdRun::*field, int* out, const char* who) {
  if (!r || !out) {
    set_error(std::string(who) + ": invalid argument");
    return MYTHOS_ERR_INVALID_ARGUMENT;
  }
  *out = r->*field;
  return MYTHOS_OK;
}

inline int64_t md_get_step(const MdRun* r) { return r ? r->step : -1; }

}

#endif
```

mythos_amd/csrc/md_plan.h:

```cpp
#pragma once
#include <cstddef>

namespace mythos {

constexpr int kMdPlanBlock = 256;

inline int md_lanes_for(int n, int cus, long long debug_lanes) {
  if (debug_lanes == 8 || debug_lanes == 16) return (int)debug_lanes;
  const int grid16 = (n + 15) / 16;
  return 2 * grid16 <= 3 * cus ? 16 : 8;
}

struct MdPlan {
  int ppb;
  int blocks;
  int grid;
  bool dense_grid;
  int prio_on;
};

inline MdPlan md_plan_for(int n, int lanes, int cus, std::size_t real_bytes, long long debug_dense) {
  MdPlan p;
  p.ppb = kMdPlanBlock / lanes;
  p.blocks = (n + p.ppb - 1) / p.ppb;
  p.grid = 8 * ((p.blocks + 7) / 8);
  p.dense_grid = real_bytes == 4 && lanes == 8 && (debug_dense == 1 || (debug_dense != 2 && p.grid > 4 * cus));
  p.prio_on = (real_bytes == 8 && p.grid > 3 * cus) ? 0 : 1;
  return p;
}

}
```

mythos_amd/csrc/neighbors.hip:

```cpp
#include <algorithm>
#include <cmath>

#include "cell_list.h"
#include "oxdna_gather.h"

namespace mythos {

int rows_from_pairs(mythos_system* sys, const int32_t* pairs, int n_pairs) {
  const int n = sys->n;
  std::vector<int> count(n, 0);
  for (int k = 0; k < n_pairs; ++k) {
    const int i = pairs[2 * k], j = pairs[2 * k + 1];
    if (i < 0 || j < 0 || i >= n || j >= n || i == j) {
      set_error("set_neighbors: pair index out of range or i == j");
      return MYTHOS_ERR_INVALID_ARGUMENT;
    }
    ++count[i];
    ++count[j];
  }
  int mx = 0;
  for (int c : count) mx = std::max(mx, c);
  const int stride = ((mx + ROW_BONDED_SLOTS + 15) / 16) * 16;
  std::vector<int> rows((size_t)n * stride, -1), len(n, ROW_BONDED_SLOTS);
  for (int i = 0; i < n; ++i) {
    for (int k = 0; k < ROW_BONDED_SLOTS; ++k) rows[(size_t)i * stride + k] = sys->h_partners[(size_t)ROW_BONDED_SLOTS * i + k];
  }
  for (int k = 0; k < n_pairs; ++k) {
    const int i = pairs[2 * k], j = pairs[2 * k + 1];
    rows[(size_t)i * stride + len[i]++] = j;
    rows[(size_t)j * stride + len[j]++] = i | ROW_ROLE_Q;
  }
  if (int rc = rows_reserve(sys->list, n, stride)) return rc;
  MYTHOS_HIP_TRY(hipMemcpy(sys->list.d_rows.get(), rows.data(), rows.size() * sizeof(int), hipMemcpyHostToDevice));
  MYTHOS_HIP_TRY(hipMemcpy(sys->d_row_len.get(), len.data(), n * sizeof(int), hipMemcpyHostToDevice));
  MYTHOS_HIP_TRY(hipMemcpy(row_close_of(sys), len.data(), n * sizeof(int), hipMemcpyHostToDevice));
  sys->nbrs_set = true;
  return 0;
}

template <typename R>
struct SiteCrit {
  const R* off;
  const R* a1;
  R rbb2;
  R rbase2, rstack2, rkb2;
  R g_ba, g_st;
};

template <typename R, class A>
__device__ __forceinline__ bool far_in_range_v(const SiteCrit<R>& sc, const A& oi, const A& oj, const V3<R>& d) {
  const V3<R> e{d.x + oj[0] - oi[0], d.y + oj[1] - oi[1], d.z + oj[2] - oi[2]};
  return dot(e, e) < sc.rbb2;
}
template <typename R>
__device__ __forceinline__ bool far_in_range(const SiteCrit<R>& sc, int i, int j, const V3<R>& d) {
  if (!sc.off) return true;
  return far_in_range_v(sc, sc.off + 4 * i, sc.off + 4 * j, d);
}

template <typename R, class A>
__device__ __forceinline__ bool site_close_v(const SiteCrit<R>& sc, const A& ai, const A& oi, const A& aj, const A& oj, const V3<R>& d) {
  const V3<R> da{aj[0] - ai[0], aj[1] - ai[1], aj[2] - ai[2]};
  V3<R> e = d;
  axpy(e, sc.g_ba, da);
  if (dot(e, e) < sc.rbase2) return true;
  e = d;
  axpy(e, sc.g_st, da);
  if (dot(e, e) < sc.rstack2) return true;
  e = V3<R>{d.x + sc.g_ba * aj[0] - oi[0], d.y + sc.g_ba * aj[1] - oi[1], d.z + sc.g_ba * aj[2] - oi[2]};
  if (dot(e, e) < sc.rkb2) return true;
  e = V3<R>{d.x + oj[0] - sc.g_ba * ai[0], d.y + oj[1] - sc.g_ba * ai[1], d.z + oj[2] - sc.g_ba * ai[2]};
  return dot(e, e) < sc.rkb2;
}
template <typename R>
__device__ __forceinline__ bool site_close(const SiteCrit<R>& sc, int i, int j, const V3<R>& d) {
  if (!sc.off) return true;
  return site_close_v(sc, sc.a1 + 4 * i, sc.off + 4 * i, sc.a1 + 4 * j, sc.off + 4 * j, d);
}

template <typename R, bool VEC4>
__global__ __launch_bounds__(256) void build_rows_allpairs_kernel(int n, const R* __restrict__ pos,
                                                                   const BoxT<R> box, R rc2, R rcl2,
                                                                   const SiteCrit<R> sc,
                                                                   const int* __restrict__ partners_rows_in,
                                                                   int* __restrict__ rows, int* __restrict__ row_len,
                                                                   int* __restrict__ row_close, int row_stride,
                                                                   int* __restrict__ overflow) {
  const int wave = (blockIdx.x * blockDim.x + threadIdx.x) >> 6;
  const int lane = threadIdx.x & 63;
  if (wave >= n) return;
  const int i = wave;
  constexpr int S = VEC4 ? 4 : 3;
  const V3<R> ci{pos[S * i], pos[S * i + 1], pos[S * i + 2]};
  int* row = rows + (size_t)i * row_stride;
  const int* bq = partners_rows_in + (size_t)ROW_BONDED_SLOTS * i;
  const int4 bp = make_int4(bq[0], bq[1], bq[2], bq[3]);
  int cnt = ROW_BONDED_SLOTS, n_close = 0;
  for (int pass = 0; pass < 2; ++pass) {
    for (int j0 = 0; j0 < n; j0 += 64) {
      const int j = j0 + lane;
      bool hit = false;
      if (j < n && j != i && j != bp.x && j != bp.y && j != bp.z && j != bp.w) {
        V3<R> d{pos[S * j] - ci.x, pos[S * j + 1] - ci.y, pos[S * j + 2] - ci.z};
        d = min_image(d, box);
        const R r2 = dot(d, d);
        if (r2 < rc2) {
          const bool cl = r2 < rcl2 && site_close(sc, i, j, d);
          hit = (pass == 0) ? cl : (!cl && far_in_range(sc, i, j, d));
        }
      }
      const unsigned long long m = __ballot(hit);
      if (hit) {
        const int slot = cnt + __popcll(m & ((1ull << lane) - 1ull));
        if (slot < row_stride) row[slot] = (j < i) ? (j | ROW_ROLE_Q) : j;
      }
      cnt += __popcll(m);
    }
    if (pass == 0) n_close = cnt;
  }
  if (lane == 0) {
    row[0] = bp.x, row[1] = bp.y, row[2] = bp.z, row[3] = bp.w;
    if (cnt > row_stride) {
      atomicMax(overflow, cnt);
      cnt = row_stride;
    }
    row_len[i] = cnt;
    row_close[i] = min(n_close, cnt);
  }
}

template <int G>
__device__ __forceinline__ void group_sort_to_row(const int* buf, int cnt, int* __restrict__ dst, int room, int l) {
  for (int b = 0; b < cnt; b += G) {
    const int k = b + l;
    const int e = (k < cnt) ? buf[k] : 0;
    const int key = e & ROW_INDEX_MASK;
    int rank = 0;
    for (int q = 0; q < cnt; ++q) rank += ((buf[q] & ROW_INDEX_MASK) < key) ? 1 : 0;
    if (k < cnt && rank < room) dst[rank] = e;
  }
}

#ifndef MYTHOS_ROW_G
#define MYTHOS_ROW_G 16
#endif
constexpr int kRowG = MYTHOS_ROW_G;

template <typename R, bool VEC4, int G>
__global__ __launch_bounds__(256) void build_rows_cells_kernel(int n, const R* __restrict__ pos, const BoxT<R> box,
                                                                const CellGrid<R> g, R rc2, R rcl2,
                                                                const SiteCrit<R> sc,
                                                                const int* __restrict__ partners,
                                                                const int* __restrict__ cell_cnt,
                                                                const typename CellPlace<R>::type* __restrict__ place,
                                                                int cell_cap, const int* __restrict__ spill, int cell_H,
                                                                size_t site_stride,
                                                                int* __restrict__ rows,
                                                                int* __restrict__ row_len, int* __restrict__ row_close,
                                                                int row_stride, int* __restrict__ overflow,
                                                                R* __restrict__ ref_pos, R* __restrict__ ref_off,
                                                                R* __restrict__ ref_a1) {
  constexpr int NG = 256 / G;
  __shared__ int s_pre[NG][29], s_st[NG][28], s_c[NG][28][3];
  extern __shared__ int s_seg_all[];
  const int kSegCap = row_stride;
  const int grp = threadIdx.x / G, l = threadIdx.x % G;
  const int gshift = (threadIdx.x & 63) & ~(G - 1);
  const int i = blockIdx.x * NG + grp;
  if (i >= n) return;
  int* s_close = s_seg_all + (size_t)grp * 2 * row_stride;
  int* s_far = s_close + row_stride;
  constexpr int S = VEC4 ? 4 : 3;
  const V3<R> ci{pos[S * i], pos[S * i + 1], pos[S * i + 2]};
  using PL = typename CellPlace<R>::type;
  R oi[3] = {R(0), R(0), R(0)}, ai[3] = {R(0), R(0), R(0)};
  if (sc.off) {
#pragma unroll
    for (int a = 0; a < 3; ++a) oi[a] = sc.off[4 * (size_t)i + a], ai[a] = sc.a1[4 * (size_t)i + a];
  }
  const int total = cell_candidates<R, G>(g, ci.x, ci.y, ci.z, cell_cnt, cell_cap, cell_H, s_pre[grp], s_st[grp], s_c[grp], l);
  int* row = rows + (size_t)i * row_stride;
  const int* bq = partners + (size_t)ROW_BONDED_SLOTS * i;
  const int4 bp = make_int4(bq[0], bq[1], bq[2], bq[3]);
  int out_c = 0, out_f = 0;
  int lo = 0;
  constexpr unsigned int kGroupMask = (G == 32) ? 0xffffffffu : ((1u << G) - 1u);
  for (int t0 = 0; t0 < total; t0 += G) {
    const int t = t0 + l;
    bool hit_c = false, hit_f = false;
    int j = -1;
    if (t < total) {
      while (s_pre[grp][lo + 1] <= t) ++lo;
      R xj, yj, zj;
      R oj[3] = {R(0), R(0), R(0)}, aj[3] = {R(0), R(0), R(0)};
      if (lo < 27) {
        const size_t at = (size_t)s_st[grp][lo] + (t - s_pre[grp][lo]);
        const PL pl = place[at];
        if (site_stride) {
          const PL po = place[site_stride + at], pa = place[2 * site_stride + at];
          oj[0] = po.x, oj[1] = po.y, oj[2] = po.z, aj[0] = pa.x, aj[1] = pa.y, aj[2] = pa.z;
        }
        xj = pl.x, yj = pl.y, zj = pl.z;
        j = cell_index_of(pl.w);
      } else {
        j = spill[t - s_pre[grp][27]];
        xj = pos[S * j], yj = pos[S * j + 1], zj = pos[S * j + 2];
        if (site_stride) {
#pragma unroll
          for (int a = 0; a < 3; ++a) oj[a] = sc.off[4 * (size_t)j + a], aj[a] = sc.a1[4 * (size_t)j + a];
        }
      }
      if (j != i && j != bp.x && j != bp.y && j != bp.z && j != bp.w) {
        bool mine = true;
        if (!g.direct && lo < 27) {
          int jx, jy, jz;
          cell_of(g, xj, yj, zj, jx, jy, jz);
          mine = jx == s_c[grp][lo][0] && jy == s_c[grp][lo][1] && jz == s_c[grp][lo][2];
        }
        if (mine) {
          V3<R> d{xj - ci.x, yj - ci.y, zj - ci.z};
          d = min_image(d, box);
          const R r2 = dot(d, d);
          if (r2 < rc2) {
            if (site_stride) {
              hit_c = r2 < rcl2 && site_close_v(sc, ai, oi, aj, oj, d);
              hit_f = !hit_c && far_in_range_v(sc, oi, oj, d);
            } else {
              hit_c = r2 < rcl2 && site_close(sc, i, j, d);
              hit_f = !hit_c && far_in_range(sc, i, j, d);
            }
          }
        }
      }
    }
    const int e = (j < i) ? (j | ROW_ROLE_Q) : j;
    const unsigned int mc = (unsigned int)(__ballot(hit_c) >> gshift) & kGroupMask;
    const unsigned int mf = (unsigned int)(__ballot(hit_f) >> gshift) & kGroupMask;
    const unsigned int below = (1u << l) - 1u;
    if (hit_c) {
      const int k = out_c + __popc(mc & below);
      if (k < kSegCap) s_close[k] = e;
    }
    if (hit_f) {
      const int k = out_f + __popc(mf & below);
      if (k < kSegCap) s_far[k] = e;
    }
    out_c += __popc(mc);
    out_f += __popc(mf);
  }
  __builtin_amdgcn_wave_barrier();
  __builtin_amdgcn_fence(__ATOMIC_ACQ_REL, "wavefront");
  const int n_close = ROW_BONDED_SLOTS + out_c;
  int out = n_close + out_f;
  group_sort_to_row<G>(s_close, min(out_c, kSegCap), row + ROW_BONDED_SLOTS, row_stride - ROW_BONDED_SLOTS, l);
  if (n_close < row_stride) group_sort_to_row<G>(s_far, min(out_f, kSegCap), row + n_close, row_stride - n_close, l);
  if (l == 0) {
    row[0] = bp.x, row[1] = bp.y, row[2] = bp.z, row[3] = bp.w;
    if (out > row_stride) {
      atomicMax(overflow, out);
      out = row_stride;
    }
    row_len[i] = out;
    row_close[i] = min(n_close, out);
    if (ref_pos) {
      R* rp = ref_pos + 4 * (size_t)i;
      rp[0] = ci.x, rp[1] = ci.y, rp[2] = ci.z, rp[3] = VEC4 ? pos[S * i + 3] : R(0);
      if (sc.off) {
        R* ro = ref_off + 4 * (size_t)i;
        R* ra = ref_a1 + 4 * (size_t)i;
#pragma unroll
        for (int k = 0; k < 4; ++k) ro[k] = sc.off[4 * (size_t)i + k], ra[k] = sc.a1[4 * (size_t)i + k];
      }
    }
  }
}

template <typename R>
static int build_cells_typed(mythos_system* sys, const R* pos, bool vec4, double rl, double skin, const R* off,
                             const R* a1, bool write_refs, hipStream_t st) {
  R* ref_pos = write_refs ? (R*)sys->d_ref_pos.get() : nullptr;
  R* ref_off = write_refs ? (R*)sys->d_ref_off.get() : nullptr;
  R* ref_a1 = write_refs ? (R*)sys->d_ref_a1.get() : nullptr;
  const int n = sys->n;
  const double rcl = sys->params_set ? std::min(rl, oxdna_close_range(sys) + skin) : rl;
  int* d_close = row_close_of(sys);
  double rbb = rl;
  if (off && sys->params_set) {
    rbb = oxdna_param_max(sys, NEXC_BACKBONE_RC);
    if (sys->model >= 2) rbb = std::max(rbb, oxdna_param_max(sys, DH_RCUT));
    rbb = std::min(rl, rbb + skin);
  }
  if (!sys->params_set || !a1) off = nullptr;
  SiteCrit<R> sc{off, a1, R(rbb * rbb), R(0), R(0), R(0), R(0), R(0)};
  if (off) {
    auto mx = [&](int idx) { return oxdna_param_max(sys, idx); };
    const double* Pd = oxdna_param_set(sys, 0);
    const double* Pr = oxdna_param_set(sys, sys->param_sets() == 1 ? 0 : 1);
    const double slack_ba = std::fabs(Pd[GEO_BASE] - Pr[GEO_BASE]), slack_st = std::fabs(Pd[GEO_STACK] - Pr[GEO_STACK]);
    auto sq = [&](double r) { return R((r + skin) * (r + skin)); };
    sc.rbase2 = sq(std::max({mx(HYDR_RCHIGH), mx(CRST_RCHIGH), mx(NEXC_BASE_RC)}) + slack_ba);
    sc.rstack2 = sq(mx(CXST_RCHIGH) + slack_st);
    sc.rkb2 = sq(std::max(mx(NEXC_BACK_BASE_RC), mx(NEXC_BASE_BACK_RC)) + 0.5 * slack_ba);
    sc.g_ba = R(0.5 * (Pd[GEO_BASE] + Pr[GEO_BASE]));
    sc.g_st = R(0.5 * (Pd[GEO_STACK] + Pr[GEO_STACK]));
  }
  VerletRows& L = sys->list;
  CellGrid<R> g;
  const bool cells = cell_grid(g, n, rl, sys->has_box ? sys->box : nullptr);
  const int blocks_ap = (n * 64 + 255) / 256;
  int* d_partners = sys->d_row_len.get() + n;
  const BoxT<R> box = make_box<R>(sys);
  if (!cells) {
    if (vec4)
      hipLaunchKernelGGL((build_rows_allpairs_kernel<R, true>), dim3(blocks_ap), dim3(256), 0, st, n, pos, box,
                         R(rl * rl), R(rcl * rcl), sc, d_partners, L.d_rows.get(), sys->d_row_len.get(), d_close, L.stride, L.d_overflow.get());
    else
      hipLaunchKernelGGL((build_rows_allpairs_kernel<R, false>), dim3(blocks_ap), dim3(256), 0, st, n, pos, box,
                         R(rl * rl), R(rcl * rcl), sc, d_partners, L.d_rows.get(), sys->d_row_len.get(), d_close, L.stride, L.d_overflow.get());
    if (write_refs && vec4) {
      const size_t bytes = (size_t)n * 4 * sizeof(R);
      MYTHOS_HIP_TRY(hipMemcpyAsync(ref_pos, pos, bytes, hipMemcpyDeviceToDevice, st));
      if (sc.off) {
        MYTHOS_HIP_TRY(hipMemcpyAsync(ref_off, sc.off, bytes, hipMemcpyDeviceToDevice, st));
        MYTHOS_HIP_TRY(hipMemcpyAsync(ref_a1, sc.a1, bytes, hipMemcpyDeviceToDevice, st));
      }
    }
    return 0;
  }
  const bool sites = sc.off != nullptr && vec4;
  CellBins bins;
  if (int rc = cell_table<R>(L, next_pow2(2 * n), sites, st, bins)) return rc;
  const size_t site_stride = sites ? (size_t)bins.H * bins.cap : 0;
  if (vec4)
    cell_bins_build<R, true>(n, pos, g, bins, L.d_overflow.get(), false, st, sc.off, sc.a1);
  else
    cell_bins_build<R, false>(n, pos, g, bins, L.d_overflow.get(), false, st);
  constexpr int kPerBlock = 256 / kRowG;
  const int wb = (n + kPerBlock - 1) / kPerBlock;
  const size_t far_lds = (size_t)kPerBlock * 2 * L.stride * sizeof(int);
  if (vec4)
    hipLaunchKernelGGL((build_rows_cells_kernel<R, true, kRowG>), dim3(wb), dim3(256), far_lds, st, n, pos, box, g, R(rl * rl),
                       R(rcl * rcl), sc, d_partners, bins.cnt_cur, (const typename CellPlace<R>::type*)bins.place, bins.cap, bins.spill, bins.H, site_stride, L.d_rows.get(), sys->d_row_len.get(), d_close, L.stride,
                       L.d_overflow.get(), ref_pos, ref_off, ref_a1);
  else
    hipLaunchKernelGGL((build_rows_cells_kernel<R, false, kRowG>), dim3(wb), dim3(256), far_lds, st, n, pos, box, g, R(rl * rl),
                       R(rcl * rcl), sc, d_partners, bins.cnt_cur, (const typename CellPlace<R>::type*)bins.place, bins.cap, bins.spill, bins.H, site_stride, L.d_rows.get(), sys->d_row_len.get(), d_close, L.stride,
                       L.d_overflow.get(), ref_pos, ref_off, ref_a1);
  return 0;
}

int rows_build_device(mythos_system* sys, const void* center, bool center_is_vec4, double r_cut, double skin,
                      const void* backbone_offsets, const void* base_vectors, bool write_refs, hipStream_t stream) {
  if (sys->list.stride == 0)
    if (int rc = rows_reserve(sys->list, sys->n, 64)) return rc;
  const double rl = r_cut + skin;
  int rc;
  if (sys->dtype == MYTHOS_F32)
    rc = build_cells_typed<float>(sys, (const float*)center, center_is_vec4, rl, skin, (const float*)backbone_offsets, (const float*)base_vectors, write_refs, stream);
  else
    rc = build_cells_typed<double>(sys, (const double*)center, center_is_vec4, rl, skin, (const double*)backbone_offsets, (const double*)base_vectors, write_refs, stream);
  if (rc) return rc;
  MYTHOS_HIP_TRY(hipGetLastError());
  sys->nbrs_set = true;
  return 0;
}

int rows_build_until_fit(mythos_system* sys, const void* center, bool center_is_vec4, double r_cut, double skin,
                         const void* backbone_offsets, const void* base_vectors, bool write_refs, bool headroom,
                         hipStream_t stream) {
  return list_build_until_fit(
      sys->list, sys->n,
      [&] { return rows_build_device(sys, center, center_is_vec4, r_cut, skin, backbone_offsets, base_vectors, write_refs, stream); },
      headroom, "neighbour build", stream);
}

}
```

mythos_amd/hip_system.py:

```python

from __future__ import annotations

import ctypes as C

import numpy as np
import torch

from mythos_amd import _lib

N_TERMS = 8
TRACE_WIDTH = 10
TERM_NAMES = (
    "fene",
    "bonded_excluded_volume",
    "stacking",
    "unbonded_excluded_volume",
    "hydrogen_bonding",
    "cross_stacking",
    "coaxial_stacking",
    "debye",
)


class OxdnaSystem(_lib.Handle):

    _destroy = "mythos_oxdna_destroy"

    def __init__(self, model: int, seq, is_end, bonded, box=None, dtype=torch.float32, device=None, is_rna=None):
        if _lib.device_count() == 0 or not torch.cuda.is_available():
            raise _lib.MythosHipError("no HIP device visible: the mythos_amd HIP path has no CPU fallback")
        self.device = torch.device("cuda", torch.cuda.current_device()) if device is None else torch.device(device)
        if self.device.type != "cuda":
            raise ValueError("OxdnaSystem needs a cuda (HIP) device")
        self.dtype = dtype
        self.model = int(model)
        seq = np.ascontiguousarray(seq, dtype=np.int32)
        self.n = int(seq.shape[0])
        is_end = np.zeros(self.n, np.uint8) if is_end is None else np.ascontiguousarray(is_end, dtype=np.uint8)
        bonded = np.ascontiguousarray(bonded, dtype=np.int32).reshape(-1, 2)
        box_arr = None if box is None else np.ascontiguousarray(np.broadcast_to(np.asarray(box, np.float64), (3,)))
        self.box = box_arr
        super().__init__(
            "mythos_oxdna_create",
            self.model,
            self.n,
            seq.ctypes.data_as(_lib.c_int_p),
            is_end.ctypes.data_as(_lib.c_uint8_p),
            int(bonded.shape[0]),
            bonded.ctypes.data_as(_lib.c_int_p),
            None if box_arr is None else box_arr.ctypes.data_as(_lib.c_double_p),
            _lib.dtype_code(dtype),
            self.device.index or 0,
        )
        self._pseq_n_bp = 0
        self._pseq_terms = 0
        self._op_lists = None
        self.n_params = self._lib.mythos_oxdna_param_count() * (3 if self.model == 4 else 1)
        if self.model == 4:
            if is_rna is None:
                raise ValueError("an oxNA system (model 4) needs is_rna, the type of every nucleotide")
            t = np.ascontiguousarray(is_rna, dtype=np.uint8)
            if t.shape != (self.n,):
                raise ValueError(f"is_rna must have shape ({self.n},)")
            _lib.check(self._lib.mythos_oxdna_set_nucleotide_types(self._h, t.ctypes.data_as(_lib.c_uint8_p)), "set_nucleotide_types")

    def set_params(self, flat) -> None:
        flat = np.ascontiguousarray(torch.as_tensor(flat).detach().cpu().numpy(), dtype=np.float64)
        _lib.check(
            self._lib.mythos_oxdna_set_params(self._h, flat.ctypes.data_as(_lib.c_double_p), int(flat.shape[0])),
            "set_params",
        )

    def set_pseq(self, marginals=None, unit=None, bp_probs=None, terms: int = 0) -> None:
        if not terms:
            _lib.check(self._lib.mythos_oxdna_set_pseq(self._h, None, None, 0, None, 0), "set_pseq")
            self._pseq_terms = 0
            return
        marg = np.ascontiguousarray(marginals, dtype=np.float64)
        unit = np.ascontiguousarray(unit, dtype=np.int32)
        bp = np.ascontiguousarray(bp_probs, dtype=np.float64).reshape(-1, 4)
        if marg.shape != (self.n, 4) or unit.shape != (self.n,):
            raise ValueError(f"marginals must be ({self.n}, 4) and unit ({self.n},)")
        n_bp = int(bp.shape[0]) if (unit >= 0).any() else 0
        self._pseq_n_bp = n_bp
        if (unit >= 0).any() and int(unit.max()) >= 2 * n_bp:
            raise ValueError("bp_probs has fewer rows than the base pairs named in unit")
        _lib.check(self._lib.mythos_oxdna_set_pseq(self._h, marg.ctypes.data_as(_lib.c_double_p), unit.ctypes.data_as(_lib.c_int_p),
                                                   n_bp, bp.ctypes.data_as(_lib.c_double_p), int(terms)), "set_pseq")
        self._pseq_terms = int(terms)

    def set_neighbors(self, pairs) -> None:
        pairs = np.ascontiguousarray(pairs, dtype=np.int32)
        if pairs.ndim != 2 or (pairs.size and pairs.shape[1] != 2):
            raise ValueError("pairs must have shape (P, 2)")
        _lib.check(
            self._lib.mythos_oxdna_set_neighbors(self._h, pairs.ctypes.data_as(_lib.c_int_p), int(pairs.shape[0])),
            "set_neighbors",
        )

    def build_neighbors(self, center: torch.Tensor, r_cut: float, skin: float) -> None:
        c = self._check(center, (self.n, 3), "center")
        _lib.check(
            self._lib.mythos_oxdna_build_neighbors(self._h, _lib.ptr(c), float(r_cut), float(skin), _lib.stream(self.device)),
            "build_neighbors",
        )

    def neighbor_stats(self) -> tuple[int, float]:
        mx, mean = C.c_int(0), C.c_double(0.0)
        _lib.check(self._lib.mythos_oxdna_neighbor_stats(self._h, C.byref(mx), C.byref(mean)), "neighbor_stats")
        return mx.value, mean.value

    def _check(self, t: torch.Tensor, tail: tuple, name: str) -> torch.Tensor:
        if not isinstance(t, torch.Tensor) or t.device != self.device:
            raise ValueError(f"{name} must be a torch tensor on {self.device}")
        if t.dtype != self.dtype:
            raise ValueError(f"{name} must have dtype {self.dtype}, got {t.dtype}")
        if tuple(t.shape[-len(tail):]) != tail:
            raise ValueError(f"{name} must have trailing shape {tail}, got {tuple(t.shape)}")
        return t.contiguous()

    def _frames(self, center, quat):
        single = center.dim() == 2
        c = self._check(center, (self.n, 3), "center")
        q = self._check(quat, (self.n, 4), "quat")
        if single:
            c, q = c[None], q[None]
        if q.shape[0] != c.shape[0]:
            raise ValueError("center and quat disagree on the number of frames")
        return c, q, int(c.shape[0]), single

    def energy(self, center, quat, *, grads=False, param_grads=False, observables=None, pseq_grads=False):
        c, q, nf, single = self._frames(center, quat)
        e = torch.empty((nf, N_TERMS), dtype=torch.float64, device=self.device)
        gc = torch.empty_like(c) if grads else None
        gq = torch.empty_like(q) if grads else None
        gp = torch.empty((nf, self.n_params), dtype=torch.float64, device=self.device) if param_grads else None
        if pseq_grads:
            if not param_grads or observables is not None:
                raise ValueError("pseq_grads comes with param_grads and without fused observables")
            gm = torch.empty((nf, self.n, 4), dtype=torch.float64, device=self.device)
            gb = torch.empty((nf, max(self._pseq_n_bp, 1), 4), dtype=torch.float64, device=self.device)
            _lib.check(
                self._lib.mythos_oxdna_energy_dpseq(
                    self._h, _lib.ptr(c), _lib.ptr(q), nf, _lib.ptr(e), _lib.ptr(gc), _lib.ptr(gq), _lib.ptr(gp), _lib.ptr(gm),
                    _lib.ptr(gb), _lib.stream(self.device),
                ),
                "energy_dpseq",
            )
            if single:
                return e[0], (gc[0] if grads else None), (gq[0] if grads else None), gp[0], gm[0], gb[0]
            return e, gc, gq, gp, gm, gb
        if observables is not None and not getattr(observables, "fusable", True):
            raise ValueError(f"{type(observables).__name__} is not evaluated in the energy call (the fused energy + observables "
                             "path takes an ObservableSet of propeller twist / rise / pitch / persistence length)")
        if observables is None:
            _lib.check(
                self._lib.mythos_oxdna_energy(
                    self._h, _lib.ptr(c), _lib.ptr(q), nf, _lib.ptr(e), _lib.ptr(gc), _lib.ptr(gq), _lib.ptr(gp),
                    _lib.stream(self.device),
                ),
                "energy",
            )
            rows = None
        else:
            rows = torch.empty((nf, observables.width), dtype=torch.float64, device=self.device)
            _lib.check(
                self._lib.mythos_oxdna_energy_obs(
                    self._h, _lib.ptr(c), _lib.ptr(q), nf, _lib.ptr(e), _lib.ptr(gc), _lib.ptr(gq), _lib.ptr(gp),
                    observables._h, _lib.ptr(rows), _lib.stream(self.device),
                ),
                "energy_obs",
            )
        if single:
            e = e[0]
            gc = gc[0] if grads else None
            gq = gq[0] if grads else None
            gp = gp[0] if param_grads else None
        if observables is not None:
            return e, gc, gq, gp, rows
        return e, gc, gq, gp


    def debye_sweep(self, center, quat, table, *, const_grads=False):
        c, q, nf, _ = self._frames(center, quat)
        table = np.ascontiguousarray(table, dtype=np.float64)
        if table.ndim != 2 or table.shape[1] != 5:
            raise ValueError("table must have shape (T, 5)")
        nt = int(table.shape[0])
        e = torch.empty((nt, nf), dtype=torch.float64, device=self.device)
        de = torch.empty((nt, nf, 5), dtype=torch.float64, device=self.device) if const_grads else None
        self._sweep_table = table
        _lib.check(
            self._lib.mythos_oxdna_debye_sweep(self._h, _lib.ptr(c), _lib.ptr(q), nf, nt, table.ctypes.data_as(_lib.c_double_p),
                                               _lib.ptr(e), _lib.ptr(de), _lib.stream(self.device)),
            "debye_sweep",
        )
        return e, de

    def order_params(self, center, quat, ops, *, raw=False, hb_cutoff=-0.1):
        from mythos_amd.input.order_parameters import KINDS

        c, q, nf, _ = self._frames(center, quat)
        cached = self._op_lists
        if cached is not None and (cached[0] is ops or cached[0] == ops):
            _, kind, first, pairs = cached
        else:
            ops = tuple(ops)
            kind = np.ascontiguousarray([KINDS.index(o.kind) for o in ops], dtype=np.int32)
            first = np.ascontiguousarray(np.concatenate([[0], np.cumsum([len(o.pairs) for o in ops])]), dtype=np.int32)
            pairs = np.ascontiguousarray([p for o in ops for p in o.pairs], dtype=np.int32).reshape(-1, 2)
            if pairs.size and int(pairs.max()) >= self.n:
                raise ValueError(f"an order parameter names nucleotide {int(pairs.max())}; the system has {self.n}")
            self._op_lists = (ops, kind, first, pairs)
        n_pairs = int(pairs.shape[0])
        out = torch.empty((nf, len(ops)), dtype=torch.float64, device=self.device)
        hb = torch.empty((nf, n_pairs), dtype=torch.float64, device=self.device) if raw else None
        dist = torch.empty((nf, n_pairs), dtype=torch.float64, device=self.device) if raw else None
        _lib.check(
            self._lib.mythos_oxdna_order_params(
                self._h, _lib.ptr(c), _lib.ptr(q), nf, len(ops), kind.ctypes.data_as(_lib.c_int_p), first.ctypes.data_as(_lib.c_int_p),
                pairs.ctypes.data_as(_lib.c_int_p), n_pairs, float(hb_cutoff), _lib.ptr(out), _lib.ptr(hb), _lib.ptr(dist),
                _lib.stream(self.device)),
            "order_params",
        )
        return (out, hb, dist) if raw else out


def _touched(*tensors) -> None:
    for t in tensors:
        if t is not None:
            torch.autograd.graph.increment_version(t)


class _MdIntegrator(_lib.Handle):

    _prefix = ""
    _destroy = property(lambda self: f"{self._prefix}_destroy")

    def __init__(self, system, *args):
        self.system = system
        super().__init__(f"{self._prefix}_create", system._h, *args)

    def _fn(self, name):
        return getattr(self._lib, f"{self._prefix}_{name}")

    @property
    def step(self) -> int:
        return int(self._fn("get_step")(self._h))

    def set_timing(self, samples: int) -> None:
        _lib.check(self._fn("set_timing")(self._h, int(samples)), "set_timing")

    def _count(self, name: str) -> int:
        r = C.c_int(0)
        _lib.check(self._fn(name)(self._h, C.byref(r)), name)
        return int(r.value)

    def last_recoveries(self) -> int:
        return self._count("last_recoveries")

    def last_rebuilds(self) -> int:
        return self._count("last_rebuilds")

    def last_kernel_ms(self) -> dict:
        k, loop, n, ns = C.c_double(0.0), C.c_double(0.0), C.c_int(0), C.c_int(0)
        _lib.check(self._fn("last_kernel_ms")(self._h, C.byref(k), C.byref(loop), C.byref(n), C.byref(ns)), "last_kernel_ms")
        return {"kernel_ms": k.value, "loop_ms_per_launch": loop.value, "launches": n.value, "samples": ns.value}


class LangevinIntegrator(_MdIntegrator):

    _prefix = "mythos_langevin"

    def __init__(self, system: OxdnaSystem, dt, kT, gamma_t, gamma_r, mass=1.0, inertia=(1.0, 1.0, 1.0), seed=0):
        inertia = np.ascontiguousarray(inertia, dtype=np.float64)
        super().__init__(system, float(dt), float(kT), float(gamma_t), float(gamma_r), float(mass),
                         inertia.ctypes.data_as(_lib.c_double_p), C.c_uint64(int(seed) & (2**64 - 1)))
        self.dt, self.kT = float(dt), float(kT)
        self.external_forces = (np.zeros(0, np.int32), np.zeros((0, 3), np.float64))

    def set_neighbor_policy(self, r_cut: float, skin: float, every: int) -> None:
        _lib.check(
            self._lib.mythos_langevin_set_neighbor_policy(self._h, float(r_cut), float(skin), int(every)),
            "set_neighbor_policy",
        )

    def set_unfused(self, on: bool = True) -> None:
        _lib.check(self._lib.mythos_langevin_set_option(self._h, 0, 1 if on else 0), "set_option(unfused)")

    def set_external_forces(self, index=None, force=None) -> None:
        from mythos_amd.input.external_forces import sum_repeated

        if index is None or len(index) == 0:
            idx, f = np.zeros(0, np.int32), np.zeros((0, 3), np.float64)
        else:
            idx, f = sum_repeated(torch.as_tensor(index).detach().cpu().numpy(), torch.as_tensor(force).detach().cpu().numpy())
        idx, f = np.ascontiguousarray(idx, dtype=np.int32), np.ascontiguousarray(f, dtype=np.float64)
        _lib.check(self._lib.mythos_langevin_set_external_forces(self._h, int(idx.shape[0]), idx.ctypes.data_as(_lib.c_int_p),
                                                                 f.ctypes.data_as(_lib.c_double_p)), "set_external_forces")
        self.external_forces = (idx, f)

    def init_momenta(self):
        s = self.system
        p = torch.empty((s.n, 3), dtype=s.dtype, device=s.device)
        ang = torch.empty((s.n, 3), dtype=s.dtype, device=s.device)
        _lib.check(self._lib.mythos_langevin_init_momenta(self._h, _lib.ptr(p), _lib.ptr(ang), _lib.stream(s.device)), "init_momenta")
        return p, ang

    def run(self, center, quat, p_lin, p_ang, n_steps: int, save_every: int = 0, want_energy: bool = True):
        state = self._state_ptrs(center, quat, p_lin, p_ang)
        tc, tq, et = self._rows(n_steps, save_every, want_energy)
        rc = self._lib.mythos_langevin_run(
            self._h, *state, int(n_steps), int(save_every), _lib.ptr(tc), _lib.ptr(tq), _lib.ptr(et), _lib.stream(self.system.device),
        )
        _touched(center, quat, p_lin, p_ang)
        _lib.check(rc, "langevin_run")
        return tc, tq, et

    def _state_ptrs(self, center, quat, p_lin, p_ang):
        s = self.system
        for t, tail, name in ((center, (s.n, 3), "center"), (quat, (s.n, 4), "quat"), (p_lin, (s.n, 3), "p_lin"), (p_ang, (s.n, 3), "p_ang")):
            if s._check(t, tail, name).data_ptr() != t.data_ptr():
                raise ValueError(f"{name} must be contiguous (the library reads and writes it in place)")
        return _lib.ptr(center), _lib.ptr(quat), _lib.ptr(p_lin), _lib.ptr(p_ang)

    def _rows(self, n_steps: int, save_every: int, want_energy: bool, out=None):
        s = self.system
        n_save = n_steps // save_every if save_every > 0 else 0
        if out is not None and n_save:
            tc, tq = out
            for t, w in ((tc, 3), (tq, 4)):
                if t.device != s.device or t.dtype != s.dtype or tuple(t.shape) != (n_save, s.n, w) or not t.is_contiguous():
                    raise ValueError(f"out tensors must be contiguous {s.dtype} of shape ({n_save}, {s.n}, 3) and ({n_save}, {s.n}, 4) on {s.device}")
        else:
            tc = torch.empty((n_save, s.n, 3), dtype=s.dtype, device=s.device) if n_save else None
            tq = torch.empty((n_save, s.n, 4), dtype=s.dtype, device=s.device) if n_save else None
        et = torch.zeros((n_save, TRACE_WIDTH), dtype=torch.float64, device=s.device) if (n_save and want_energy) else None
        return tc, tq, et

    def load(self, center, quat, p_lin, p_ang) -> None:
        _lib.check(self._lib.mythos_langevin_load(self._h, *self._state_ptrs(center, quat, p_lin, p_ang), _lib.stream(self.system.device)), "langevin_load")

    def advance(self, n_steps: int, save_every: int = 0, want_energy: bool = True, out=None):
        s = self.system
        tc, tq, et = self._rows(n_steps, save_every, want_energy, out)
        _lib.check(
            self._lib.mythos_langevin_advance(self._h, int(n_steps), int(save_every), _lib.ptr(tc), _lib.ptr(tq), _lib.ptr(et), _lib.stream(s.device)),
            "langevin_advance",
        )
        if out is not None and tc is not None:
            _touched(tc, tq)
        return tc, tq, et

    def store(self, center, quat, p_lin, p_ang) -> None:
        rc = self._lib.mythos_langevin_store(self._h, *self._state_ptrs(center, quat, p_lin, p_ang), _lib.stream(self.system.device))
        _touched(center, quat, p_lin, p_ang)
        _lib.check(rc, "langevin_store")

    @_MdIntegrator.step.setter
    def step(self, value: int) -> None:
        _lib.check(self._lib.mythos_langevin_set_step(self._h, int(value)), "set_step")

    def set_seed(self, seed: int) -> None:
        _lib.check(self._lib.mythos_langevin_set_seed(self._h, C.c_uint64(int(seed) & (2**64 - 1))), "set_seed")


def martini_frames(pos, box):
    if box is None:
        raise ValueError("MARTINI observables need trajectory.box_size (per-frame periodic box)")
    if not isinstance(pos, torch.Tensor) or pos.device.type != "cuda":
        raise _lib.MythosHipError("observables are evaluated by the HIP library: the trajectory must live on a GPU "
                                  "(mythos_amd has no CPU fallback)")
    if pos.dtype not in (torch.float32, torch.float64):
        raise ValueError(f"unsupported dtype {pos.dtype}")
    if pos.dim() == 2:
        pos = pos[None]
    box = torch.as_tensor(box, dtype=pos.dtype, device=pos.device).reshape(-1, 3)
    if box.shape[0] == 1 and pos.shape[0] > 1:
        box = box.expand(pos.shape[0], 3)
    if box.shape[0] != pos.shape[0]:
        raise ValueError(f"box_size has {box.shape[0]} rows for {pos.shape[0]} frames")
    return pos.contiguous(), box.contiguous()


class MartiniSystem(_lib.Handle):

    N_TERMS = 3
    _destroy = "mythos_martini_destroy"

    def __init__(self, types, sigma, eps, bonds, bond_k, bond_r0, angles, angle_k, angle_t0, angle_kind=0, r_cut=1.1,
                 dtype=torch.float32, device=None):
        if _lib.device_count() == 0 or not torch.cuda.is_available():
            raise _lib.MythosHipError("no HIP device visible: the mythos_amd HIP path has no CPU fallback")
        self.device = torch.device("cuda", torch.cuda.current_device()) if device is None else torch.device(device)
        self.dtype = dtype
        types = np.ascontiguousarray(types, dtype=np.int32)
        self.n = int(types.shape[0])
        sigma = np.ascontiguousarray(sigma, dtype=np.float64)
        eps = np.ascontiguousarray(eps, dtype=np.float64)
        n_types = int(sigma.shape[0])
        bonds = np.ascontiguousarray(bonds, dtype=np.int32).reshape(-1, 2)
        angles = np.ascontiguousarray(angles, dtype=np.int32).reshape(-1, 3)
        self.n_types, self.n_bonds, self.n_angles = n_types, int(bonds.shape[0]), int(angles.shape[0])
        f = lambda a: np.ascontiguousarray(a, dtype=np.float64)
        bond_k, bond_r0, angle_k, angle_t0 = f(bond_k), f(bond_r0), f(angle_k), f(angle_t0)
        dp = lambda a: a.ctypes.data_as(_lib.c_double_p)
        super().__init__(
            "mythos_martini_create", self.n, types.ctypes.data_as(_lib.c_int_p), n_types, dp(sigma), dp(eps), int(bonds.shape[0]),
            bonds.ctypes.data_as(_lib.c_int_p), dp(bond_k), dp(bond_r0), int(angles.shape[0]),
            angles.ctypes.data_as(_lib.c_int_p), dp(angle_k), dp(angle_t0), int(angle_kind), float(r_cut),
            _lib.dtype_code(dtype), self.device.index or 0,
        )

    def _frames(self, pos, box):
        if pos.device != self.device or pos.dtype != self.dtype or tuple(pos.shape[-2:]) != (self.n, 3):
            raise ValueError(f"pos must be a {self.dtype} tensor of shape (F, {self.n}, 3) on {self.device}")
        return martini_frames(pos, box)

    def energy(self, pos: torch.Tensor, box: torch.Tensor, grads: bool = False):
        single = pos.dim() == 2
        pos, box = self._frames(pos, box)
        nf = pos.shape[0]
        e = torch.empty((nf, 3), dtype=torch.float64, device=self.device)
        g = torch.empty_like(pos) if grads else None
        _lib.check(
            self._lib.mythos_martini_energy(self._h, _lib.ptr(pos), _lib.ptr(box), nf, _lib.ptr(e), _lib.ptr(g), _lib.stream(self.device)),
            "martini_energy",
        )
        return (e[0], g[0] if grads else None) if single else (e, g)

    def param_grads(self, pos: torch.Tensor, box: torch.Tensor, lj: bool = True, bonds: bool = True, angles: bool = True):
        pos, box = self._frames(pos, box)
        nf = pos.shape[0]

        def buf(on, *shape):
            return torch.zeros((nf, *shape), dtype=torch.float64, device=self.device) if on else None

        out = {"sigma": buf(lj, self.n_types, self.n_types), "eps": buf(lj, self.n_types, self.n_types),
               "bond_k": buf(bonds, self.n_bonds), "bond_r0": buf(bonds, self.n_bonds),
               "angle_k": buf(angles, self.n_angles), "angle_t0": buf(angles, self.n_angles)}
        _lib.check(
            self._lib.mythos_martini_param_grads(
                self._h, _lib.ptr(pos), _lib.ptr(box), nf, _lib.ptr(out["sigma"]), _lib.ptr(out["eps"]),
                _lib.ptr(out["bond_k"]), _lib.ptr(out["bond_r0"]), _lib.ptr(out["angle_k"]), _lib.ptr(out["angle_t0"]),
                _lib.stream(self.device)),
            "martini_param_grads",
        )
        return out


class MartiniLangevinIntegrator(_MdIntegrator):

    KB = 0.0083144626
    _prefix = "mythos_martini_langevin"

    def __init__(self, system: MartiniSystem, dt, kT, gamma, mass=None, seed=0):
        mptr = None
        if mass is not None:
            mass = np.ascontiguousarray(mass, dtype=np.float64)
            if mass.shape != (system.n,):
                raise ValueError(f"mass must have shape ({system.n},)")
            mptr = mass.ctypes.data_as(_lib.c_double_p)
        super().__init__(system, float(dt), float(kT), float(gamma), mptr, int(seed))

    def set_neighbor_policy(self, skin: float, every: int) -> None:
        _lib.check(self._lib.mythos_martini_langevin_set_neighbor_policy(self._h, float(skin), int(every)), "set_neighbor_policy")

    def set_inner_list(self, margin: float, every: int) -> None:
        _lib.check(self._lib.mythos_martini_langevin_set_inner_list(self._h, float(margin), int(every)), "set_inner_list")

    BAROSTATS = {None: 0, "berendsen": 1, "c-rescale": 2}
    COUPLINGS = {"isotropic": 0, "semiisotropic": 1}

    def set_barostat(self, kind=None, coupling="isotropic", ref_p=1.0, compressibility=4.5e-5, tau_p=1.0, every=10) -> None:
        if kind not in self.BAROSTATS or coupling not in self.COUPLINGS:
            raise ValueError(f"kind must be one of {list(self.BAROSTATS)}, coupling one of {list(self.COUPLINGS)}")
        pair = lambda v: np.ascontiguousarray(np.broadcast_to(np.asarray(v, dtype=np.float64), (2,)))
        p0, beta = pair(ref_p), pair(compressibility)
        _lib.check(self._lib.mythos_martini_langevin_set_barostat(
            self._h, self.BAROSTATS[kind], self.COUPLINGS[coupling], p0.ctypes.data_as(_lib.c_double_p),
            beta.ctypes.data_as(_lib.c_double_p), float(tau_p), int(every)), "set_barostat")

    def pressure(self) -> dict:
        out = np.zeros(10, dtype=np.float64)
        _lib.check(self._lib.mythos_martini_langevin_pressure(self._h, out.ctypes.data_as(_lib.c_double_p), _lib.stream(self.system.device)),
                   "martini_langevin_pressure")
        return {"kinetic": out[0:3].copy(), "virial": out[3:6].copy(), "pressure": out[6:9].copy(), "volume": float(out[9]),
                "p": float(out[6:9].mean())}

    @property
    def box(self) -> np.ndarray:
        b = np.zeros(3, dtype=np.float64)
        _lib.check(self._lib.mythos_martini_langevin_get_box(self._h, b.ctypes.data_as(_lib.c_double_p)), "get_box")
        return b

    @property
    def last_boxes(self) -> torch.Tensor:
        n = C.c_int(0)
        _lib.check(self._lib.mythos_martini_langevin_last_boxes(self._h, None, C.byref(n)), "last_boxes")
        b = np.zeros((n.value, 3), dtype=np.float64)
        if n.value:
            _lib.check(self._lib.mythos_martini_langevin_last_boxes(self._h, b.ctypes.data_as(_lib.c_double_p), C.byref(n)), "last_boxes")
        return torch.as_tensor(b, device=self.system.device)

    def init_velocities(self) -> torch.Tensor:
        v = torch.empty((self.system.n, 3), dtype=self.system.dtype, device=self.system.device)
        _lib.check(self._lib.mythos_martini_langevin_init_velocities(self._h, _lib.ptr(v), _lib.stream(self.system.device)), "init_velocities")
        return v

    def _check_state(self, pos, vel):
        s = self.system
        for t, name in ((pos, "pos"), (vel, "vel")):
            if t.device != s.device or t.dtype != s.dtype or tuple(t.shape) != (s.n, 3) or not t.is_contiguous():
                raise ValueError(f"{name} must be a contiguous {s.dtype} tensor of shape ({s.n}, 3) on {s.device}")

    def _rows(self, n_steps: int, save_every: int, want_energy: bool):
        s = self.system
        ns = n_steps // save_every if save_every > 0 else 0
        traj = torch.empty((ns, s.n, 3), dtype=s.dtype, device=s.device) if ns else None
        et = torch.zeros((ns, 4), dtype=torch.float64, device=s.device) if (ns and want_energy) else None
        return traj, et

    def run(self, pos, vel, box, n_steps: int, save_every: int = 0, want_energy: bool = True):
        s = self.system
        self._check_state(pos, vel)
        box = np.ascontiguousarray(np.asarray(box, dtype=np.float64).reshape(3))
        traj, et = self._rows(n_steps, save_every, want_energy)
        rc = self._lib.mythos_martini_langevin_run(
            self._h, _lib.ptr(pos), _lib.ptr(vel), box.ctypes.data_as(_lib.c_double_p), int(n_steps), int(save_every),
            _lib.ptr(traj), _lib.ptr(et), _lib.stream(s.device))
        _touched(pos, vel)
        _lib.check(rc, "martini_langevin_run")
        return traj, et

    def load(self, pos, vel, box) -> None:
        self._check_state(pos, vel)
        box = np.ascontiguousarray(np.asarray(box, dtype=np.float64).reshape(3))
        _lib.check(self._lib.mythos_martini_langevin_load(self._h, _lib.ptr(pos), _lib.ptr(vel), box.ctypes.data_as(_lib.c_double_p),
                                                          _lib.stream(self.system.device)), "martini_langevin_load")

    def advance(self, n_steps: int, save_every: int = 0, want_energy: bool = True):
        traj, et = self._rows(n_steps, save_every, want_energy)
        _lib.check(self._lib.mythos_martini_langevin_advance(self._h, int(n_steps), int(save_every), _lib.ptr(traj), _lib.ptr(et),
                                                             _lib.stream(self.system.device)), "martini_langevin_advance")
        return traj, et

    def store(self, pos, vel) -> None:
        self._check_state(pos, vel)
        rc = self._lib.mythos_martini_langevin_store(self._h, _lib.ptr(pos), _lib.ptr(vel), _lib.stream(self.system.device))
        _touched(pos, vel)
        _lib.check(rc, "martini_langevin_store")

    def rows(self, pruned: bool = False):
        stride = C.c_int(0)
        which = 1 if pruned else 0
        _lib.check(self._lib.mythos_martini_langevin_get_rows(self._h, which, None, None, C.byref(stride)), "get_rows")
        rows = np.empty((self.system.n, stride.value), dtype=np.int32)
        lens = np.empty(self.system.n, dtype=np.int32)
        _lib.check(self._lib.mythos_martini_langevin_get_rows(self._h, which, rows.ctypes.data_as(C.POINTER(C.c_int32)),
                                                              lens.ctypes.data_as(C.POINTER(C.c_int32)), C.byref(stride)), "get_rows")
        return rows, lens

    def neighbor_stats(self) -> tuple[int, float]:
        mx, mean = C.c_int(0), C.c_double(0.0)
        _lib.check(self._lib.mythos_martini_langevin_neighbor_stats(self._h, C.byref(mx), C.byref(mean)), "neighbor_stats")
        return mx.value, mean.value
```

Measured before the change: 69870 steps/s.

## Add pruned inner neighbor rows refreshed between full Verlet rebuilds

Adds a two-level neighbor list. A prune kernel periodically filters the full Verlet rows into a tighter inner list, using a smaller margin and keeping the close/far split. The MD step kernel then reads these shorter rows and flags when a particle drifts past half the inner margin. The aim is to cut pair work per step in exchange for extra prune launches, memory and displacement checks. The feature is off unless enabled through the new set_inner_list API, or an auto rule when every is negative.

```diff
diff --git a/include/mythos_hip.h b/include/mythos_hip.h
--- a/include/mythos_hip.h
+++ b/include/mythos_hip.h
@@ -85,6 +85,10 @@
 void mythos_langevin_destroy(mythos_sim_t* sim);
 
 int mythos_langevin_set_neighbor_policy(mythos_sim_t* sim, double r_cut, double skin, int every);
+
+int mythos_langevin_set_inner_list(mythos_sim_t* sim, double margin, int every);
+int mythos_langevin_get_inner_list(const mythos_sim_t* sim, double* margin, int* every, int* active);
+int mythos_langevin_get_rows(const mythos_sim_t* sim, int which, int32_t* rows, int32_t* row_len, int32_t* row_close, int* stride);
 
 int mythos_langevin_init_momenta(mythos_sim_t* sim, void* p_lin, void* p_ang, mythos_stream_t stream);
 
diff --git a/mythos_amd/_lib.py b/mythos_amd/_lib.py
--- a/mythos_amd/_lib.py
+++ b/mythos_amd/_lib.py
@@ -49,6 +49,9 @@
     "mythos_langevin_create": (V, [V, C.c_double, C.c_double, C.c_double, C.c_double, C.c_double, c_double_p, C.c_uint64]),
     "mythos_langevin_destroy": (None, [V]),
     "mythos_langevin_set_neighbor_policy": (C.c_int, [V, C.c_double, C.c_double, C.c_int]),
+    "mythos_langevin_set_inner_list": (C.c_int, [V, C.c_double, C.c_int]),
+    "mythos_langevin_get_inner_list": (C.c_int, [V, c_double_p, C.POINTER(C.c_int), C.POINTER(C.c_int)]),
+    "mythos_langevin_get_rows": (C.c_int, [V, C.c_int, c_int_p, c_int_p, c_int_p, C.POINTER(C.c_int)]),
     "mythos_langevin_init_momenta": (C.c_int, [V, V, V, V]),
     "mythos_langevin_run": (C.c_int, [V, V, V, V, V, C.c_int, C.c_int, V, V, V, V]),
     "mythos_langevin_load": (C.c_int, [V, V, V, V, V, V]),
diff --git a/mythos_amd/csrc/inner_rows.h b/mythos_amd/csrc/inner_rows.h
--- /dev/null
+++ b/mythos_amd/csrc/inner_rows.h
@@ -0,0 +1,80 @@
+#pragma once
+#include "langevin_step.h"
+#include "site_crit.h"
+
+namespace mythos {
+
+constexpr int kPruneG = 8;
+constexpr int kPrunePPB = 256 / kPruneG;
+
+template <typename R>
+struct InnerRows {
+  int* rows;
+  int* len;
+  int* close;
+  typename Vec4T<R>::type *ref_pos, *ref_off, *ref_a1;
+};
+
+template <typename R>
+static __global__ __launch_bounds__(256) void prune_rows_kernel(int n, const Frame<R> in, const BoxT<R> box, const SiteCrit<R> sc, R rcl2,
+                                                                 const int* __restrict__ rows, const int* __restrict__ row_len,
+                                                                 const int* __restrict__ row_close, int row_stride,
+                                                                 const InnerRows<R> out, R half_sq) {
+  using V4 = typename Vec4T<R>::type;
+  constexpr int G = kPruneG;
+  extern __shared__ int s_far_all[];
+  const int grp = threadIdx.x / G, l = threadIdx.x % G;
+  const int gshift = (threadIdx.x & 63) & ~(G - 1);
+  const int i = blockIdx.x * kPrunePPB + grp;
+  if (i >= n) return;
+  if (i == 0 && l == 0) out.ref_pos[3 * (size_t)n] = V4{half_sq, R(0), R(0), R(0)};
+  int* s_far = s_far_all + (size_t)grp * row_stride;
+  const V4 s0 = in.p0[i], s1 = in.p1[i], s3 = in.p3[i];
+  V3<R> self_lo{R(0), R(0), R(0)};
+  if constexpr (kHiLo<R>) self_lo = xyz<R>(in.pl[i]);
+  const V3<R> self_c = xyz<R>(s0);
+  const R ai[3] = {s1.x, s1.y, s1.z}, oi[3] = {s3.x, s3.y, s3.z};
+  const int* __restrict__ row = rows + (size_t)i * row_stride;
+  int* __restrict__ orow = out.rows + (size_t)i * row_stride;
+  const int len = min(max(row_len[i], ROW_BONDED_SLOTS), row_stride);
+  (void)row_close;
+  int out_c = 0, out_f = 0;
+  constexpr unsigned int kGroupMask = (1u << G) - 1u;
+  for (int s0i = ROW_BONDED_SLOTS; s0i < len; s0i += G) {
+    const int s = s0i + l;
+    bool hit_c = false, hit_f = false;
+    int e = -1;
+    if (s < len) {
+      e = row[s];
+      const int j = e & ROW_INDEX_MASK;
+      if (e >= 0 && j < n) {
+        const V4 o0 = in.p0[j], o1 = in.p1[j], o3 = in.p3[j];
+        V4 ol{};
+        if constexpr (kHiLo<R>) ol = in.pl[j];
+        const V3<R> d = min_image(centre_diff<R>(o0, ol, self_c, self_lo), box);
+        const R aj[3] = {o1.x, o1.y, o1.z}, oj[3] = {o3.x, o3.y, o3.z};
+        hit_c = dot(d, d) < rcl2 && site_close_v(sc, ai, oi, aj, oj, d);
+        hit_f = !hit_c && far_in_range_v(sc, oi, oj, d);
+      }
+    }
+    const unsigned int mc = (unsigned int)(__ballot(hit_c) >> gshift) & kGroupMask;
+    const unsigned int mf = (unsigned int)(__ballot(hit_f) >> gshift) & kGroupMask;
+    const unsigned int below = (1u << l) - 1u;
+    if (hit_c) orow[ROW_BONDED_SLOTS + out_c + __popc(mc & below)] = e;
+    if (hit_f) s_far[out_f + __popc(mf & below)] = e;
+    out_c += __popc(mc);
+    out_f += __popc(mf);
+  }
+  __builtin_amdgcn_wave_barrier();
+  __builtin_amdgcn_fence(__ATOMIC_ACQ_REL, "wavefront");
+  const int n_close = ROW_BONDED_SLOTS + out_c;
+  for (int k = l; k < out_f; k += G) orow[n_close + k] = s_far[k];
+  if (l < ROW_BONDED_SLOTS) orow[l] = row[l];
+  if (l == 0) {
+    out.len[i] = n_close + out_f;
+    out.close[i] = n_close;
+    out.ref_pos[i] = s0, out.ref_off[i] = s3, out.ref_a1[i] = s1;
+  }
+}
+
+}
diff --git a/mythos_amd/csrc/langevin.hip b/mythos_amd/csrc/langevin.hip
--- a/mythos_amd/csrc/langevin.hip
+++ b/mythos_amd/csrc/langevin.hip
@@ -54,6 +54,58 @@
   return MYTHOS_OK;
 }
 
+int mythos_langevin_set_inner_list(mythos_sim_t* s, double margin, int every) {
+  if (!s || !std::isfinite(margin)) {
+    set_error("mythos_langevin_set_inner_list: invalid argument");
+    return MYTHOS_ERR_INVALID_ARGUMENT;
+  }
+  s->inner_auto = every < 0;
+  const bool on = every >= 2 && margin > 0;
+  s->inner_margin = on ? margin : 0.0;
+  s->inner_every = on ? every : 0;
+  s->list_valid = false;
+  return MYTHOS_OK;
+}
+
+int mythos_langevin_get_inner_list(const mythos_sim_t* s, double* margin, int* every, int* active) {
+  if (!s) {
+    set_error("mythos_langevin_get_inner_list: invalid argument");
+    return MYTHOS_ERR_INVALID_ARGUMENT;
+  }
+  const InnerPolicy p = inner_policy_of(s);
+  if (margin) *margin = p.margin;
+  if (every) *every = p.every;
+  if (active) *active = p.active ? 1 : 0;
+  return MYTHOS_OK;
+}
+
+int mythos_langevin_get_rows(const mythos_sim_t* s, int which, int32_t* rows, int32_t* row_len, int32_t* row_close, int* stride) {
+  const char* who = "mythos_langevin_get_rows";
+  if (!s || (which != 0 && which != 1)) {
+    set_error(std::string(who) + ": invalid argument");
+    return MYTHOS_ERR_INVALID_ARGUMENT;
+  }
+  const mythos_system* sys = s->sys;
+  const size_t n = (size_t)sys->n;
+  const int st = which == 0 ? sys->list.stride : s->inner_stride;
+  if (stride) *stride = st;
+  if (!rows && !row_len && !row_close) return MYTHOS_OK;
+  const int* d_rows = which == 0 ? sys->list.d_rows.get() : s->d_inner_rows.get();
+  const int* d_len = which == 0 ? sys->d_row_len.get() : s->d_inner_len.get();
+  const int* d_close = which == 0 ? row_close_of(sys) : s->d_inner_len.get() + n;
+  const bool have = which == 0 ? (sys->nbrs_set && d_rows && d_len) : (s->list_valid && inner_policy_of(s).active && d_rows && d_len && st > 0);
+  if (!have) {
+    set_error(std::string(who) + (which == 0 ? ": no list has been built" : ": no inner rows (switched off, or no step taken yet)"));
+    return MYTHOS_ERR_INVALID_ARGUMENT;
+  }
+  MYTHOS_HIP_TRY(hipSetDevice(s->device));
+  MYTHOS_HIP_TRY(hipDeviceSynchronize());
+  if (rows) MYTHOS_HIP_TRY(hipMemcpy(rows, d_rows, n * st * sizeof(int), hipMemcpyDeviceToHost));
+  if (row_len) MYTHOS_HIP_TRY(hipMemcpy(row_len, d_len, n * sizeof(int), hipMemcpyDeviceToHost));
+  if (row_close) MYTHOS_HIP_TRY(hipMemcpy(row_close, d_close, n * sizeof(int), hipMemcpyDeviceToHost));
+  return MYTHOS_OK;
+}
+
 int mythos_langevin_init_momenta(mythos_sim_t* s, void* p_lin, void* p_ang, mythos_stream_t stream) {
   if (!s || !p_lin || !p_ang) {
     set_error("mythos_langevin_init_momenta: invalid argument");
diff --git a/mythos_amd/csrc/langevin_core.inc b/mythos_amd/csrc/langevin_core.inc
--- a/mythos_amd/csrc/langevin_core.inc
+++ b/mythos_amd/csrc/langevin_core.inc
@@ -109,6 +109,8 @@
   if (debug_value(MYTHOS_DEBUG_MD_ITEMS_BIG) == 1) sim->items_big = true;
   if (use_pseq) pseq.marg = (const R*)sys->d_ps_marg.get(), pseq.unit = sys->d_ps_unit.get(), pseq.bp = (const R*)sys->d_ps_bp.get(), pseq.terms = sys->pseq_terms;
   int* halt_words = dynamic_list ? sys->list.d_overflow.get() : nullptr;
+  const InnerPolicy inner_pol = inner_policy_of(sim);
+  const bool inner_on = dynamic_list && inner_pol.active && md_inner_supported<R, MODEL>();
   auto launch_step = [&](int k, const LaunchRow& row) {
     const int cur = row.cur;
     const bool save = row.save;
@@ -118,6 +120,10 @@
     const V4* ref = (const V4*)sys->d_ref_pos.get();
     const V4* ref_off = (const V4*)sys->d_ref_off.get();
     const V4* ref_a1 = (const V4*)sys->d_ref_a1.get();
+    const InnerRows<R> ir = inner_rows_of<R>(sim);
+    const int* l_rows = inner_on ? ir.rows : sys->list.d_rows.get();
+    const int* l_len = inner_on ? ir.len : sys->d_row_len.get();
+    const int* l_close = inner_on ? ir.close : row_close_of(sys);
     if (sim->ext_count > 0) {
       if (sim->ext_stamp_stale) {
         (void)hipMemsetAsync(sim->d_ext_stamp.get(), 0, sizeof(unsigned long long), st);
@@ -133,8 +139,8 @@
       hipExtLaunchKernelGGL((md_step_kernel<R, MODEL, decltype(save_tag)::value, decltype(items_tag)::value, decltype(pseq_tag)::value,
                                             decltype(dense_tag)::value, decltype(lanes_tag)::value>),
                             dim3(plan.grid), dim3(kMdBlock), 0, st, row.ea, row.eb, 0,
-                            Pdev, box, K, cut, n, fr[cur], fr[cur ^ 1], sys->list.d_rows.get(), sys->d_row_len.get(), row_close_of(sys),
-                            sys->list.stride, sys->extra_bonds ? 1 : 0, kick_close, row.do_step, sim->seed, (uint64_t)(sim->step + k), ref,
+                            Pdev, box, K, cut, n, fr[cur], fr[cur ^ 1], l_rows, l_len, l_close,
+                            sys->list.stride, (sys->extra_bonds ? kMdRowExtraBonds : 0) | (inner_on ? kMdRowInner : 0), kick_close, row.do_step, sim->seed, (uint64_t)(sim->step + k), ref,
                             ref_off, ref_a1, sim->d_flags.get(), tc, tq, sim->d_epart.get(), sim->d_chunk_order.get(), halt_words, k, 0,
                             plan.prio_on, pseq);
     };
@@ -168,6 +174,26 @@
   auto rebuild_until_fit = [&](int buf) -> int {
     return rows_build_until_fit(sys, fr[buf].p0, true, sim->r_cut, sim->skin, fr[buf].p3, fr[buf].p1, true, true, st);
   };
+  auto prune = [&](int buf) -> int {
+    const int stride = sys->list.stride;
+    if (sim->inner_stride != stride || !sim->d_inner_rows) {
+      static_assert(sizeof(V4) % sizeof(int) == 0, "the reference words are counted in ints");
+      if (stride % 16 != 0) {
+        set_error("mythos_langevin_run: row stride " + std::to_string(stride) + " is not a multiple of 16");
+        return MYTHOS_ERR_INVALID_ARGUMENT;
+      }
+      if (int rc = sim->d_inner_rows.grow((size_t)n * stride + ((size_t)3 * n + 1) * (sizeof(V4) / sizeof(int)))) return rc;
+      if (int rc = sim->d_inner_len.grow((size_t)2 * n)) return rc;
+      sim->inner_stride = stride;
+    }
+    const SiteCrit<R> sc = site_crit_for<R>(sys, (const R*)fr[buf].p3, (const R*)fr[buf].p1, 1e30, inner_pol.margin);
+    const double rcl = oxdna_close_range(sys) + inner_pol.margin;
+    hipLaunchKernelGGL(prune_rows_kernel<R>, dim3((n + kPrunePPB - 1) / kPrunePPB), dim3(256), (size_t)kPrunePPB * stride * sizeof(int), st, n,
+                       fr[buf], box, sc, R(rcl * rcl), (const int*)sys->list.d_rows.get(), (const int*)sys->d_row_len.get(),
+                       (const int*)row_close_of(sys), stride, inner_rows_of<R>(sim), R(0.25 * inner_pol.margin * inner_pol.margin));
+    MYTHOS_HIP_TRY(hipGetLastError());
+    return 0;
+  };
   auto on_abort = [&]() -> int {
     if (!sim->items_big) {
       sim->items_big = true;
@@ -187,8 +213,9 @@
   d.halt_words = halt_words;
   d.row_stride = &sys->list.stride;
   d.skin = sim->skin;
+  d.inner_every = inner_on ? inner_pol.every : 0;
   d.st = st;
-  return md_drive(*sim, d, launch_step, rebuild, rebuild_until_fit, on_abort);
+  return md_drive(*sim, d, launch_step, rebuild, rebuild_until_fit, on_abort, prune);
 }
 
 template <typename R>
diff --git a/mythos_amd/csrc/langevin_sim.h b/mythos_amd/csrc/langevin_sim.h
--- a/mythos_amd/csrc/langevin_sim.h
+++ b/mythos_amd/csrc/langevin_sim.h
@@ -4,8 +4,10 @@
 #endif
 #include <cmath>
 
+#include "inner_rows.h"
 #include "langevin_step.h"
 #include "md_driver.h"
+#include "md_plan.h"
 
 struct mythos_sim : mythos::MdRun {
   mythos_system* sys = nullptr;
@@ -14,6 +16,12 @@
   double r_cut = 0, skin = 0;
   static constexpr int kFrameArrays = 8;
   mythos::DeviceBytes frame[2][kFrameArrays];
+  bool inner_auto = false;
+  double inner_margin = 0;
+  int inner_every = 0;
+  int inner_stride = 0;
+  mythos::DeviceBuf<int> d_inner_rows;
+  mythos::DeviceBuf<int> d_inner_len;
   int builds = 0;
   int list_epoch = 0;
   mythos::DeviceBytes keep_hi, keep_lo;
@@ -53,6 +61,22 @@
   return K;
 }
 
+inline InnerPolicy inner_policy_of(const mythos_sim* s) {
+  InnerPolicy p = s->inner_auto ? md_inner_rule(s->lanes, s->rebuild_every, s->skin)
+                                : InnerPolicy{s->inner_margin, s->inner_every, s->rebuild_every > 0 && s->inner_margin > 0 && s->inner_every >= 2};
+  if (s->sys->model == 4 && s->sys->dtype != MYTHOS_F32) p.active = false;
+  if (s->unfused.active) p.active = false;
+  return p;
+}
+
+template <typename R>
+static InnerRows<R> inner_rows_of(const mythos_sim* s) {
+  using V4 = typename Vec4T<R>::type;
+  const size_t n = (size_t)s->sys->n;
+  V4* ref = s->d_inner_rows ? (V4*)(s->d_inner_rows.get() + n * s->inner_stride) : nullptr;
+  return InnerRows<R>{s->d_inner_rows.get(), s->d_inner_len.get(), s->d_inner_len.get() + n, ref, ref + n, ref + 2 * n};
+}
+
 template <typename R>
 static MdCut<R> make_cut(const mythos_system* sys) {
   const OxParams<double>& P = sys->pd;
diff --git a/mythos_amd/csrc/langevin_step.h b/mythos_amd/csrc/langevin_step.h
--- a/mythos_amd/csrc/langevin_step.h
+++ b/mythos_amd/csrc/langevin_step.h
@@ -78,6 +78,11 @@
 }
 
 constexpr int kMdBlock = 256;
+constexpr int kMdRowExtraBonds = 1, kMdRowInner = 2;
+template <typename R, int MODEL>
+constexpr bool md_inner_supported() {
+  return !(MODEL == 4 && sizeof(R) == 8);
+}
 constexpr int kMdG = 8;
 constexpr int kMdPPB = kMdBlock / kMdG;
 #ifndef MYTHOS_MD_ITEMS
@@ -248,11 +253,14 @@
     const R* __restrict__ Pg, const BoxT<R> box, const LangevinConst<R> K, const MdCut<R> cut, int n, const Frame<R> in,
     const Frame<R> out,
     const int* __restrict__ rows, const int* __restrict__ row_len, const int* __restrict__ row_close, int row_stride,
-    int extra_bonds, R kick_close, int do_step, uint64_t seed, uint64_t step, const typename Vec4T<R>::type* __restrict__ ref_pos,
+    int row_flags, R kick_close, int do_step, uint64_t seed, uint64_t step, const typename Vec4T<R>::type* __restrict__ ref_pos,
     const typename Vec4T<R>::type* __restrict__ ref_off, const typename Vec4T<R>::type* __restrict__ ref_a1,
     int* __restrict__ flags,
     R* __restrict__ traj_c, R* __restrict__ traj_q, double* __restrict__ e_part, const int* __restrict__ chunk_order,
     const int* __restrict__ list_overflow, int k_index, int , int prio_on, const PseqView<R> pseq) {
+  const int extra_bonds = row_flags & kMdRowExtraBonds;
+  const bool inner_rows = md_inner_supported<R, MODEL>() && (row_flags & kMdRowInner) != 0;
+  const typename Vec4T<R>::type* inner_ref = reinterpret_cast<const typename Vec4T<R>::type*>(rows + (size_t)n * row_stride);
   using V4 = typename Vec4T<R>::type;
   constexpr int G = GL, PPB = kMdBlock / GL;
   static_assert(GL == 8 || GL == 16, "lanes per nucleotide");
@@ -654,10 +662,16 @@
   const int i_int = bid * PPB + il;
   const bool integrates = (int)(threadIdx.x >> 6) == int_wave && il < PPB && i_int < n;
   R z[6] = {R(0), R(0), R(0), R(0), R(0), R(0)};
-  V4 pm{}, lm{}, qv{}, r0{}, f0{}, a0{};
+  V4 pm{}, lm{}, qv{}, r0{}, f0{}, a0{}, ri{}, fi{}, ai{};
+  R inner_hs = R(0);
+  constexpr bool kInnerEarly = sizeof(R) == 4;
   if (integrates) {
     pm = in.mom[i_int], lm = in.ang[i_int], qv = in.q[i_int];
-    if (do_step && K.skin_half_sq > R(0)) r0 = ref_pos[i_int], f0 = ref_off[i_int], a0 = ref_a1[i_int];
+    if (do_step && K.skin_half_sq > R(0)) {
+      r0 = ref_pos[i_int], f0 = ref_off[i_int], a0 = ref_a1[i_int];
+      if constexpr (kInnerEarly)
+        if (inner_rows) ri = inner_ref[i_int], fi = inner_ref[n + i_int], ai = inner_ref[2 * n + i_int], inner_hs = inner_ref[3 * n].x;
+    }
     if (do_step) normals6(seed, (uint32_t)i_int, step, 0u, z);
 #pragma unroll
     for (int k = 0; k < 6; ++k) pin_vgpr(z[k]);
@@ -817,6 +831,16 @@
         if (dx * dx + dy * dy + dz * dz > K.skin_half_sq || bx * bx + by * by + bz * bz > K.skin_half_sq ||
             sx * sx + sy * sy + sz * sz > K.skin_half_sq)
           atomicMax(flags + 1, k_index + 1);
+        if (inner_rows) {
+          if constexpr (!kInnerEarly) ri = inner_ref[i], fi = inner_ref[n + i], ai = inner_ref[2 * n + i], inner_hs = inner_ref[3 * n].x;
+          const R ex = x[0] - ri.x, ey = x[1] - ri.y, ez = x[2] - ri.z;
+          const R cx = ex + (g_k1 * n1.x + g_k2 * nbk.x - fi.x), cy = ey + (g_k1 * n1.y + g_k2 * nbk.y - fi.y),
+                  cz = ez + (g_k1 * n1.z + g_k2 * nbk.z - fi.z);
+          const R tx = ex + gb * (n1.x - ai.x), ty = ey + gb * (n1.y - ai.y), tz = ez + gb * (n1.z - ai.z);
+          if (ex * ex + ey * ey + ez * ez > inner_hs || cx * cx + cy * cy + cz * cz > inner_hs ||
+              tx * tx + ty * ty + tz * tz > inner_hs)
+            atomicMax(flags + 1, k_index + 1);
+        }
       }
     }
     if constexpr (!SAVE) {
diff --git a/mythos_amd/csrc/md_driver.h b/mythos_amd/csrc/md_driver.h
--- a/mythos_amd/csrc/md_driver.h
+++ b/mythos_amd/csrc/md_driver.h
@@ -92,6 +92,7 @@
   int* halt_words;
   const int* row_stride;
   double skin;
+  int inner_every = 0;
   std::string give_up_hint;
   hipStream_t st;
 };
@@ -107,9 +108,9 @@
   hipEvent_t ea, eb;
 };
 
-template <class Launch, class Rebuild, class RebuildUntilFit, class OnAbort>
+template <class Launch, class Rebuild, class RebuildUntilFit, class OnAbort, class Prune>
 static int md_drive(MdRun& run, const MdDrive& d, Launch&& launch, Rebuild&& rebuild, RebuildUntilFit&& rebuild_until_fit,
-                    OnAbort&& on_abort) {
+                    OnAbort&& on_abort, Prune&& prune) {
   const bool closes = d.close || (d.energy_rows && d.n_steps > 0 && d.n_steps % d.save_every == 0);
   const int n_launch = closes ? d.n_steps + 1 : d.n_steps;
   if (n_launch == 0) return MYTHOS_OK;
@@ -171,6 +172,8 @@
           MYTHOS_HIP_TRY(hipMemsetD32Async((hipDeviceptr_t)d.halt_words, *d.row_stride + 1, 1, st));
         }
       }
+      if (d.dynamic_list && d.inner_every > 0 && (k - built_at) % d.inner_every == 0)
+        if (int rc = prune(cur)) return fail(k, rc);
       row.kick_close = (k == 0 && !was_open) ? 0.0f : 0.5f;
       row.do_step = last ? 0 : 1;
       row.built_at = built_at;
@@ -245,6 +248,12 @@
   return MYTHOS_OK;
 }
 
+template <class Launch, class Rebuild, class RebuildUntilFit, class OnAbort>
+static int md_drive(MdRun& run, const MdDrive& d, Launch&& launch, Rebuild&& rebuild, RebuildUntilFit&& rebuild_until_fit,
+                    OnAbort&& on_abort) {
+  return md_drive(run, d, launch, rebuild, rebuild_until_fit, on_abort, [](int) { return 0; });
+}
+
 inline int md_set_timing(MdRun* r, int samples, const char* who) {
   if (!r || samples < 0) {
     set_error(std::string(who) + ": invalid argument");
diff --git a/mythos_amd/csrc/md_plan.h b/mythos_amd/csrc/md_plan.h
--- a/mythos_amd/csrc/md_plan.h
+++ b/mythos_amd/csrc/md_plan.h
@@ -29,4 +29,20 @@
   return p;
 }
 
+struct InnerPolicy {
+  double margin;
+  int every;
+  bool active;
+};
+
+constexpr double kInnerMarginOfSkin = 1.0 / 3.0;
+constexpr int kInnerPrunesPerBuild = 4;
+inline InnerPolicy md_inner_rule(int lanes, int rebuild_every, double skin) {
+  InnerPolicy p;
+  p.margin = skin * kInnerMarginOfSkin;
+  p.every = rebuild_every / kInnerPrunesPerBuild;
+  p.active = lanes == 8 && rebuild_every >= 8 && skin >= 0.3;
+  return p;
 }
+
+}
diff --git a/mythos_amd/csrc/neighbors.hip b/mythos_amd/csrc/neighbors.hip
--- a/mythos_amd/csrc/neighbors.hip
+++ b/mythos_amd/csrc/neighbors.hip
@@ -3,6 +3,7 @@
 
 #include "cell_list.h"
 #include "oxdna_gather.h"
+#include "site_crit.h"
 
 namespace mythos {
 
@@ -39,39 +40,11 @@
 }
 
 template <typename R>
-struct SiteCrit {
-  const R* off;
-  const R* a1;
-  R rbb2;
-  R rbase2, rstack2, rkb2;
-  R g_ba, g_st;
-};
-
-template <typename R, class A>
-__device__ __forceinline__ bool far_in_range_v(const SiteCrit<R>& sc, const A& oi, const A& oj, const V3<R>& d) {
-  const V3<R> e{d.x + oj[0] - oi[0], d.y + oj[1] - oi[1], d.z + oj[2] - oi[2]};
-  return dot(e, e) < sc.rbb2;
-}
-template <typename R>
 __device__ __forceinline__ bool far_in_range(const SiteCrit<R>& sc, int i, int j, const V3<R>& d) {
   if (!sc.off) return true;
   return far_in_range_v(sc, sc.off + 4 * i, sc.off + 4 * j, d);
 }
 
-template <typename R, class A>
-__device__ __forceinline__ bool site_close_v(const SiteCrit<R>& sc, const A& ai, const A& oi, const A& aj, const A& oj, const V3<R>& d) {
-  const V3<R> da{aj[0] - ai[0], aj[1] - ai[1], aj[2] - ai[2]};
-  V3<R> e = d;
-  axpy(e, sc.g_ba, da);
-  if (dot(e, e) < sc.rbase2) return true;
-  e = d;
-  axpy(e, sc.g_st, da);
-  if (dot(e, e) < sc.rstack2) return true;
-  e = V3<R>{d.x + sc.g_ba * aj[0] - oi[0], d.y + sc.g_ba * aj[1] - oi[1], d.z + sc.g_ba * aj[2] - oi[2]};
-  if (dot(e, e) < sc.rkb2) return true;
-  e = V3<R>{d.x + oj[0] - sc.g_ba * ai[0], d.y + oj[1] - sc.g_ba * ai[1], d.z + oj[2] - sc.g_ba * ai[2]};
-  return dot(e, e) < sc.rkb2;
-}
 template <typename R>
 __device__ __forceinline__ bool site_close(const SiteCrit<R>& sc, int i, int j, const V3<R>& d) {
   if (!sc.off) return true;
@@ -284,26 +257,7 @@
   const int n = sys->n;
   const double rcl = sys->params_set ? std::min(rl, oxdna_close_range(sys) + skin) : rl;
   int* d_close = row_close_of(sys);
-  double rbb = rl;
-  if (off && sys->params_set) {
-    rbb = oxdna_param_max(sys, NEXC_BACKBONE_RC);
-    if (sys->model >= 2) rbb = std::max(rbb, oxdna_param_max(sys, DH_RCUT));
-    rbb = std::min(rl, rbb + skin);
-  }
-  if (!sys->params_set || !a1) off = nullptr;
-  SiteCrit<R> sc{off, a1, R(rbb * rbb), R(0), R(0), R(0), R(0), R(0)};
-  if (off) {
-    auto mx = [&](int idx) { return oxdna_param_max(sys, idx); };
-    const double* Pd = oxdna_param_set(sys, 0);
-    const double* Pr = oxdna_param_set(sys, sys->param_sets() == 1 ? 0 : 1);
-    const double slack_ba = std::fabs(Pd[GEO_BASE] - Pr[GEO_BASE]), slack_st = std::fabs(Pd[GEO_STACK] - Pr[GEO_STACK]);
-    auto sq = [&](double r) { return R((r + skin) * (r + skin)); };
-    sc.rbase2 = sq(std::max({mx(HYDR_RCHIGH), mx(CRST_RCHIGH), mx(NEXC_BASE_RC)}) + slack_ba);
-    sc.rstack2 = sq(mx(CXST_RCHIGH) + slack_st);
-    sc.rkb2 = sq(std::max(mx(NEXC_BACK_BASE_RC), mx(NEXC_BASE_BACK_RC)) + 0.5 * slack_ba);
-    sc.g_ba = R(0.5 * (Pd[GEO_BASE] + Pr[GEO_BASE]));
-    sc.g_st = R(0.5 * (Pd[GEO_STACK] + Pr[GEO_STACK]));
-  }
+  const SiteCrit<R> sc = site_crit_for<R>(sys, off, a1, rl, skin);
   VerletRows& L = sys->list;
   CellGrid<R> g;
   const bool cells = cell_grid(g, n, rl, sys->has_box ? sys->box : nullptr);
diff --git a/mythos_amd/csrc/site_crit.h b/mythos_amd/csrc/site_crit.h
--- /dev/null
+++ b/mythos_amd/csrc/site_crit.h
@@ -0,0 +1,65 @@
+#pragma once
+#include <algorithm>
+#include <cmath>
+
+#include "mythos_internal.h"
+#include "oxdna_gather.h"
+
+namespace mythos {
+
+template <typename R>
+struct SiteCrit {
+  const R* off;
+  const R* a1;
+  R rbb2;
+  R rbase2, rstack2, rkb2;
+  R g_ba, g_st;
+};
+
+template <typename R, class A>
+__device__ __forceinline__ bool far_in_range_v(const SiteCrit<R>& sc, const A& oi, const A& oj, const V3<R>& d) {
+  const V3<R> e{d.x + oj[0] - oi[0], d.y + oj[1] - oi[1], d.z + oj[2] - oi[2]};
+  return dot(e, e) < sc.rbb2;
+}
+
+template <typename R, class A>
+__device__ __forceinline__ bool site_close_v(const SiteCrit<R>& sc, const A& ai, const A& oi, const A& aj, const A& oj, const V3<R>& d) {
+  const V3<R> da{aj[0] - ai[0], aj[1] - ai[1], aj[2] - ai[2]};
+  V3<R> e = d;
+  axpy(e, sc.g_ba, da);
+  if (dot(e, e) < sc.rbase2) return true;
+  e = d;
+  axpy(e, sc.g_st, da);
+  if (dot(e, e) < sc.rstack2) return true;
+  e = V3<R>{d.x + sc.g_ba * aj[0] - oi[0], d.y + sc.g_ba * aj[1] - oi[1], d.z + sc.g_ba * aj[2] - oi[2]};
+  if (dot(e, e) < sc.rkb2) return true;
+  e = V3<R>{d.x + oj[0] - sc.g_ba * ai[0], d.y + oj[1] - sc.g_ba * ai[1], d.z + oj[2] - sc.g_ba * ai[2]};
+  return dot(e, e) < sc.rkb2;
+}
+
+template <typename R>
+static inline SiteCrit<R> site_crit_for(const mythos_system* sys, const R* off, const R* a1, double rl, double slack) {
+  double rbb = rl;
+  if (off && sys->params_set) {
+    rbb = oxdna_param_max(sys, NEXC_BACKBONE_RC);
+    if (sys->model >= 2) rbb = std::max(rbb, oxdna_param_max(sys, DH_RCUT));
+    rbb = std::min(rl, rbb + slack);
+  }
+  if (!sys->params_set || !a1) off = nullptr;
+  SiteCrit<R> sc{off, a1, R(rbb * rbb), R(0), R(0), R(0), R(0), R(0)};
+  if (off) {
+    auto mx = [&](int idx) { return oxdna_param_max(sys, idx); };
+    const double* Pd = oxdna_param_set(sys, 0);
+    const double* Pr = oxdna_param_set(sys, sys->param_sets() == 1 ? 0 : 1);
+    const double slack_ba = std::fabs(Pd[GEO_BASE] - Pr[GEO_BASE]), slack_st = std::fabs(Pd[GEO_STACK] - Pr[GEO_STACK]);
+    auto sq = [&](double r) { return R((r + slack) * (r + slack)); };
+    sc.rbase2 = sq(std::max({mx(HYDR_RCHIGH), mx(CRST_RCHIGH), mx(NEXC_BASE_RC)}) + slack_ba);
+    sc.rstack2 = sq(mx(CXST_RCHIGH) + slack_st);
+    sc.rkb2 = sq(std::max(mx(NEXC_BACK_BASE_RC), mx(NEXC_BASE_BACK_RC)) + 0.5 * slack_ba);
+    sc.g_ba = R(0.5 * (Pd[GEO_BASE] + Pr[GEO_BASE]));
+    sc.g_st = R(0.5 * (Pd[GEO_STACK] + Pr[GEO_STACK]));
+  }
+  return sc;
+}
+
+}
diff --git a/mythos_amd/hip_system.py b/mythos_amd/hip_system.py
--- a/mythos_amd/hip_system.py
+++ b/mythos_amd/hip_system.py
@@ -285,6 +285,25 @@
             "set_neighbor_policy",
         )
 
+    def set_inner_list(self, margin: float, every: int) -> None:
+        _lib.check(self._lib.mythos_langevin_set_inner_list(self._h, float(margin), int(every)), "set_inner_list")
+
+    def get_inner_list(self) -> tuple[float, int, bool]:
+        m, e, a = C.c_double(0.0), C.c_int(0), C.c_int(0)
+        _lib.check(self._lib.mythos_langevin_get_inner_list(self._h, C.byref(m), C.byref(e), C.byref(a)), "get_inner_list")
+        return m.value, e.value, bool(a.value)
+
+    def rows(self, inner: bool = False):
+        stride = C.c_int(0)
+        which = 1 if inner else 0
+        _lib.check(self._lib.mythos_langevin_get_rows(self._h, which, None, None, None, C.byref(stride)), "get_rows")
+        rows = np.empty((self.system.n, stride.value), dtype=np.int32)
+        lens = np.empty(self.system.n, dtype=np.int32)
+        close = np.empty(self.system.n, dtype=np.int32)
+        p = lambda a: a.ctypes.data_as(_lib.c_int_p)
+        _lib.check(self._lib.mythos_langevin_get_rows(self._h, which, p(rows), p(lens), p(close), C.byref(stride)), "get_rows")
+        return rows, lens, close
+
     def set_unfused(self, on: bool = True) -> None:
         _lib.check(self._lib.mythos_langevin_set_option(self._h, 0, 1 if on else 0), "set_option(unfused)")
 
```

Measured after the change: 69140 steps/s. 0.99x the previous value.
